# castorini/dhr

Hardware: AMD Instinct MI355X
Metric: queries/sec (exact top-1000, brute-force dense-hybrid GIP retrieval) (higher is better)
Workload: dtype i8 (bound GEMM: gated AND ungated columns int8 x int8 -> int32 on the matrix cores, every gated rounding upward, the ungated quantisation error paid by the filter margin) + f64-accumulated f16 x f32 exact rescoring of the survivors -- the returned scores are the exact scores rounded once, identical

## Files before the change

dhr_amd/_build.py:

```python
from __future__ import annotations

import concurrent.futures
import fcntl
import os
import shutil
import subprocess

CSRC = os.path.join(os.path.dirname(os.path.abspath(__file__)), "csrc")
LIB = os.path.join(CSRC, "libdhr_hip.so")
OBJDIR = os.path.join(CSRC, "build")
SOURCES = ["abi.cpp", "kernels.hip", "gemm_w4.hip", "gemm_g8.hip", "index_build.hip", "search_core.hip", "api.hip", "sharded.hip", "pq_adc.hip", "select_global.hip", "host_io.hip", "lexical.hip", "gip_train.hip", "lexical_train.hip", "maxsim.hip", "aggretriever_train.hip", "lexical_proj.hip", "lexical_proj_train.hip", "train_loss.hip", "densify_sparse.hip"]
HEADERS = ["dhr_internal.h", "dhr_state.h", "search_plan.h", "index_layout.h", "sharded_plan.h", "host_stage.h", "op_dispatch.h", "abi_guard.h", "libdhr.map", "gemm_common.h", "gemm_g8.h", "lexical_common.h", "lexical_proj_common.h", "lexical_proj_layout.h", os.path.join("..", "..", "include", "dhr_hip.h")]
FLAGS = ["--offload-arch=gfx950", "-O3", "-std=c++17", "-fPIC", "-Wno-unused-value", "-Wno-unused-result"]
if os.environ.get("DHR_AB_VARIANTS") == "1":
    SOURCES = SOURCES + [os.path.join("..", "..", "tools", "ab", "gemm_g8p.hip")]
    FLAGS = FLAGS + ["-DDHR_AB_VARIANTS", "-I" + CSRC]


def _mtime(path: str) -> float:
    return os.path.getmtime(path) if os.path.exists(path) else 0.0


def _stale() -> bool:
    t = _mtime(LIB)
    return t == 0.0 or any(_mtime(os.path.join(CSRC, f)) > t for f in SOURCES + HEADERS)


def _compile(hipcc: str, src: str, newest_header: float, force: bool, verbose: bool) -> str:
    obj = os.path.join(OBJDIR, os.path.splitext(os.path.basename(src))[0] + ".o")
    if not force and _mtime(obj) > max(_mtime(os.path.join(CSRC, src)), newest_header):
        return obj
    tmp = obj + ".tmp.%d" % os.getpid()
    cmd = [hipcc] + FLAGS + ["-c", src, "-o", tmp]
    if verbose:
        print(" ".join(cmd), flush=True)
    subprocess.run(cmd, cwd=CSRC, check=True)
    os.replace(tmp, obj)
    return obj


def build(force: bool = False, verbose: bool = False) -> str:
    if not force and not _stale():
        return LIB
    os.makedirs(OBJDIR, exist_ok=True)
    with open(os.path.join(OBJDIR, ".lock"), "w") as lock:
        fcntl.flock(lock, fcntl.LOCK_EX)
        try:
            if not force and not _stale():
                return LIB
            hipcc = shutil.which("hipcc") or "/opt/rocm/bin/hipcc"
            newest_header = max(_mtime(os.path.join(CSRC, h)) for h in HEADERS)
            with concurrent.futures.ThreadPoolExecutor(max_workers=min(len(SOURCES), os.cpu_count() or 1, 16)) as ex:
                objs = list(ex.map(lambda s: _compile(hipcc, s, newest_header, force, verbose), SOURCES))
            tmp = LIB + ".tmp.%d" % os.getpid()
            cmd = [hipcc, "--offload-arch=gfx950", "-shared", "-fPIC", "-Wl,--version-script=" + os.path.join(CSRC, "libdhr.map"), "-o", tmp] + objs + ["-L/opt/rocm/lib", "-lrccl"]
            if verbose:
                print(" ".join(cmd), flush=True)
            subprocess.run(cmd, cwd=CSRC, check=True)
            os.replace(tmp, LIB)
        finally:
            fcntl.flock(lock, fcntl.LOCK_UN)
    return LIB


if __name__ == "__main__":
# ... 3 lines not shown
```

dhr_amd/_lib.py:

```python
from __future__ import annotations

import ctypes as C
import os

import numpy as np

from . import _build

DHR_OK = 0
ERR_INVALID, ERR_UNSUPPORTED, ERR_HIP, ERR_INTERNAL, ERR_NOMEM, ERR_PEER = -1, -2, -3, -4, -5, -6
ABI_INDEX_DESC, ABI_QUERY_BATCH, ABI_SEARCH_STATS, ABI_FILE_INFO, ABI_HOST_SHARD = 0, 1, 2, 3, 4
IDX_NONE, IDX_U8, IDX_I8, IDX_I16 = 0, 1, 2, 3
VAL_F16, VAL_F32, VAL_BF16 = 0, 1, 2
MEM_HOST, MEM_DEVICE = 0, 1
LEX_RAW, LEX_DENSIFY, LEX_AGG_FULL, LEX_AGG_SEMI = 0, 1, 2, 3
PARAM_CAND_CAP, PARAM_FIRST_ROWS, PARAM_PROFILE, PARAM_MAX_GROWTH, PARAM_SAMPLE_PERIOD, PARAM_GEMM_VARIANT, PARAM_MAIN_CHUNKS, PARAM_PROGRESSIVE_THR, PARAM_AUX_CUS, PARAM_GEMM_EXCLUSIVE, PARAM_OVERLAP_AUX, PARAM_SAMPLE_SHARE, PARAM_ASYNC_CONTROLLER, PARAM_LIST_STRIDE = 1, 2, 3, 4, 5, 6, 7, 8, 9, 10, 11, 12, 13, 14
OPT_DENSE_I8, OPT_GATED_I8 = 1, 2
COMM_TRANSPORT, COMM_WORLD, COMM_RANK, COMM_DEVICE = 0, 1, 2, 3
INFO_DENSE_I8, INFO_I8_SCALE, INFO_I8_ROW_ERR, INFO_I8_ROW_NORM, INFO_ROW_NORM_MAX, INFO_TILE_BYTES, INFO_GATED_I8, INFO_GEMM_KERNEL = 1, 2, 3, 4, 5, 6, 7, 8

EXPORTS = ["dhr_version", "dhr_abi_sizes", "dhr_abi_size", "dhr_debug_fail_alloc", "dhr_set_option", "dhr_index_get_info", "dhr_last_error", "dhr_index_create", "dhr_index_destroy", "dhr_index_set_param",
           "dhr_index_device_bytes", "dhr_search", "dhr_score_rows", "dhr_merge_topk", "dhr_merge_topk_host", "dhr_merge_topk_lists", "dhr_merge_topk_lists_host",
           "dhr_get_stats", "dhr_debug_bound_scores", "dhr_debug_query_margins", "dhr_debug_gemm_time", "dhr_debug_seq_to_tile", "dhr_debug_sharded_repairs", "dhr_search_sample_rank", "dhr_search_union_rank", "dhr_search_begin",
           "dhr_search_finish", "dhr_search_mid_ranks", "dhr_search_mid", "dhr_search_pre_ranks", "dhr_search_pre", "dhr_search_begin_rest", "dhr_search_rerank", "dhr_comm_unique_id", "dhr_comm_create", "dhr_comm_wrap", "dhr_comm_create_callback", "dhr_comm_destroy", "dhr_comm_info", "dhr_comm_abort", "dhr_search_sharded", "dhr_search_sharded_local", "dhr_search_sharded_host", "dhr_pq_create", "dhr_pq_destroy", "dhr_pq_device_bytes", "dhr_pq_search", "dhr_pq_adc_scores", "dhr_pq_last_scan", "dhr_index_save", "dhr_index_file_info", "dhr_index_load", "dhr_densify", "dhr_pq_train", "dhr_pq_encode", "dhr_pq_decode", "dhr_pq_train_nbits", "dhr_pq_encode_nbits", "dhr_pq_decode_nbits", "dhr_write_trec", "dhr_format_float", "dhr_lexical_head", "dhr_aggregate", "dhr_gip_scores_workspace", "dhr_gip_scores", "dhr_gip_scores_backward", "dhr_densify_backward", "dhr_lexical_head_train_workspace", "dhr_lexical_head_train", "dhr_lexical_head_backward", "dhr_maxsim_scores", "dhr_maxsim_scores_backward", "dhr_aggregate_train", "dhr_aggregate_backward", "dhr_term_weight_head",
           "dhr_term_weight_head_backward", "dhr_lexical_proj_workspace", "dhr_lexical_proj_head", "dhr_lexical_proj_train_workspace",
           "dhr_lexical_proj_train", "dhr_lexical_proj_backward", "dhr_train_loss_workspace", "dhr_train_loss", "dhr_densify_sparse"]


class DhrError(RuntimeError):

    def __init__(self, msg, status=None):
        super().__init__(msg)
        self.status = status


class IndexDesc(C.Structure):
    _fields_ = [("device", C.c_int32), ("mem_kind", C.c_int32), ("n_rows", C.c_int64), ("d_dlr", C.c_int32),
                ("d_cls", C.c_int32), ("value", C.c_void_p), ("ld_value", C.c_int64), ("index", C.c_void_p),
                ("index_dtype", C.c_int32), ("idx_buckets", C.c_int32), ("ld_index", C.c_int64),
                ("row_offset", C.c_int64)]


class QueryBatch(C.Structure):
    _fields_ = [("n_queries", C.c_int32), ("mem_kind", C.c_int32), ("value", C.c_void_p), ("value_dtype", C.c_int32),
                ("index_dtype", C.c_int32), ("ld_value", C.c_int64), ("index", C.c_void_p), ("ld_index", C.c_int64)]


class SearchStats(C.Structure):
    _fields_ = [("n_rows", C.c_int64), ("n_queries", C.c_int64), ("k", C.c_int64), ("phases", C.c_int32),
                ("overflow_retries", C.c_int32), ("candidates_bound", C.c_int64), ("candidates_exact", C.c_int64),
                ("gemm_rows", C.c_int64), ("sample_fallback_queries", C.c_int64), ("gemm_ms", C.c_double), ("refine_ms", C.c_double),
                ("rescore_ms", C.c_double), ("select_ms", C.c_double), ("prep_ms", C.c_double),
                ("total_ms", C.c_double), ("gemm_flops", C.c_double), ("gemm_flops_alg", C.c_double)]

    def as_dict(self):
        return {f: getattr(self, f) for f, _ in self._fields_}


class FileInfo(C.Structure):
    _fields_ = [("n_rows", C.c_int64), ("row_offset", C.c_int64), ("d_dlr", C.c_int32), ("d_cls", C.c_int32),
                ("index_dtype", C.c_int32), ("idx_buckets", C.c_int32), ("file_version", C.c_uint32), ("reserved", C.c_uint32),
                ("payload_bytes", C.c_int64), ("blob_offset", C.c_int64), ("blob_bytes", C.c_int64)]


FILE_MAGIC = b"DHRIDX1\x00"

ALLGATHER_FN = C.CFUNCTYPE(C.c_int, C.c_void_p, C.c_void_p, C.c_void_p, C.c_int64)
HS_SAMPLE_RANK = C.CFUNCTYPE(C.c_int32, C.c_void_p, C.c_int32, C.c_int32)
HS_UNION_RANK = C.CFUNCTYPE(C.c_int32, C.c_void_p, C.c_int32)
HS_BEGIN = C.CFUNCTYPE(C.c_int32, C.c_void_p, C.POINTER(QueryBatch), C.c_int32, C.c_int32, C.c_void_p)
HS_FINISH = C.CFUNCTYPE(C.c_int32, C.c_void_p, C.c_void_p, C.c_void_p, C.c_void_p, C.c_void_p)
HS_SEARCH = C.CFUNCTYPE(C.c_int32, C.c_void_p, C.POINTER(QueryBatch), C.c_int32, C.c_void_p, C.c_void_p)
HS_MID_RANKS = C.CFUNCTYPE(C.c_int32, C.c_void_p, C.c_int32, C.c_int32, C.POINTER(C.c_int32), C.POINTER(C.c_int32))
HS_MID = C.CFUNCTYPE(C.c_int32, C.c_void_p, C.c_void_p, C.c_int32, C.c_void_p)
HS_PRE_RANKS = C.CFUNCTYPE(C.c_int32, C.c_void_p, C.c_int32, C.c_int32, C.POINTER(C.c_int32), C.POINTER(C.c_int32))
HS_PRE = C.CFUNCTYPE(C.c_int32, C.c_void_p, C.POINTER(QueryBatch), C.c_int32, C.c_int32, C.c_int32, C.c_void_p)
# ... 103 lines not shown
    lib.dhr_aggregate_train.argtypes = lib.dhr_aggregate.argtypes[:-1] + [C.c_void_p, C.c_int64, C.c_void_p]
    lib.dhr_aggregate_backward.argtypes = [C.c_int32, C.c_int32, C.c_void_p, C.c_int32, C.c_int64, C.c_void_p, C.c_int64, C.c_int64, C.c_int32, C.c_int32,
                                           C.c_int32, C.c_int32, C.c_void_p, C.c_int64, C.c_void_p]
    ids = [C.c_int32, C.c_int32, C.c_void_p, C.c_int32, C.c_int64]
    lib.dhr_term_weight_head.argtypes = ids + [C.c_void_p, C.c_int32, C.c_int64, C.c_int64, C.c_int32, C.c_int32, C.c_int32, C.c_void_p, C.c_int64,
                                               C.c_void_p, C.c_int64, C.c_void_p]
    lib.dhr_term_weight_head_backward.argtypes = ids + [C.c_int64, C.c_int32, C.c_int32, C.c_int32, C.c_void_p, C.c_int64, C.c_void_p, C.c_int64,
                                                        C.c_void_p, C.c_int32, C.c_int64, C.c_void_p]
    lib.dhr_pq_train.argtypes = [C.c_int32, C.c_int32, C.c_void_p, C.c_int64, C.c_int64, C.c_int32, C.c_int32, C.c_int32, C.c_int64, C.c_void_p,
                                 C.POINTER(C.c_double), C.c_void_p]
    lib.dhr_pq_encode.argtypes = [C.c_int32, C.c_int32, C.c_void_p, C.c_int64, C.c_int64, C.c_int32, C.c_int32, C.c_void_p, C.c_void_p, C.c_void_p]
    lib.dhr_pq_train_nbits.argtypes = [C.c_int32, C.c_int32, C.c_void_p, C.c_int64, C.c_int64, C.c_int32, C.c_int32, C.c_int32, C.c_int32, C.c_int64, C.c_void_p,
                                       C.POINTER(C.c_double), C.c_void_p]
    lib.dhr_pq_encode_nbits.argtypes = [C.c_int32, C.c_int32, C.c_void_p, C.c_int64, C.c_int64, C.c_int32, C.c_int32, C.c_int32, C.c_void_p, C.c_void_p, C.c_void_p]
    lib.dhr_pq_decode_nbits.argtypes = [C.c_int32, C.c_int32, C.c_void_p, C.c_int64, C.c_int32, C.c_int32, C.c_int32, C.c_void_p, C.c_void_p, C.c_int64, C.c_void_p]
    lib.dhr_write_trec.argtypes = [C.c_char_p, C.c_int32, C.c_int64, C.c_int64, C.c_void_p, C.c_void_p, C.c_void_p, C.c_void_p, C.c_int64, C.c_void_p,
                                   C.c_int64, C.c_void_p, C.c_char_p, C.c_int32, C.c_int32, C.POINTER(C.c_int64)]
    lib.dhr_format_float.argtypes = [C.c_double, C.c_char_p, C.c_int32]
    lib.dhr_pq_decode.argtypes = [C.c_int32, C.c_int32, C.c_void_p, C.c_int64, C.c_int32, C.c_int32, C.c_void_p, C.c_void_p, C.c_int64, C.c_void_p]
    lib.dhr_score_rows.argtypes = [C.c_void_p, C.POINTER(QueryBatch), C.c_int32, C.c_void_p, C.c_void_p, C.c_int32, C.c_void_p]
    lib.dhr_merge_topk.argtypes = [C.c_int32, C.c_int32, C.c_int32, C.c_void_p, C.c_void_p, C.c_int32, C.c_void_p,
                                   C.c_void_p, C.c_void_p]
    lib.dhr_merge_topk_host.argtypes = [C.c_int32, C.c_int32, C.c_void_p, C.c_void_p, C.c_int32, C.c_void_p, C.c_void_p]
    lib.dhr_merge_topk_lists.argtypes = [C.c_int32, C.c_int32, C.c_int32, C.c_int32, C.c_void_p, C.c_void_p, C.c_int32,
                                         C.c_void_p, C.c_void_p, C.c_void_p]
    lib.dhr_merge_topk_lists_host.argtypes = [C.c_int32, C.c_int32, C.c_int32, C.c_void_p, C.c_void_p, C.c_int32, C.c_void_p,
                                              C.c_void_p]
    lib.dhr_comm_unique_id.argtypes = [C.c_void_p, C.c_int32]
    lib.dhr_comm_create.argtypes = [C.c_void_p, C.c_int32, C.c_int32, C.c_int32, C.POINTER(C.c_void_p)]
    lib.dhr_comm_wrap.argtypes = [C.c_void_p, C.c_int32, C.c_int32, C.c_int32, C.POINTER(C.c_void_p)]
    lib.dhr_comm_create_callback.argtypes = [C.c_int32, C.c_int32, C.c_int32, ALLGATHER_FN, C.c_void_p, C.POINTER(C.c_void_p)]
    lib.dhr_search_sharded_host.argtypes = [C.POINTER(HostShard), C.c_int32, C.c_int32, ALLGATHER_FN, C.c_void_p, C.POINTER(QueryBatch), C.c_int32,
                                            C.c_void_p, C.c_void_p]
    lib.dhr_comm_destroy.argtypes = [C.c_void_p]
    lib.dhr_comm_destroy.restype = None
    lib.dhr_comm_abort.argtypes = [C.c_void_p]
    lib.dhr_comm_abort.restype = None
    lib.dhr_comm_info.argtypes = [C.c_void_p, C.c_int32]
    lib.dhr_search_sharded.argtypes = [C.c_void_p, C.c_void_p, C.POINTER(QueryBatch), C.c_int32, C.c_void_p, C.c_void_p, C.c_int32, C.c_void_p]
    lib.dhr_search_sharded_local.argtypes = [C.POINTER(C.c_void_p), C.c_int32, C.POINTER(QueryBatch), C.c_int32, C.c_void_p, C.c_void_p, C.c_int32, C.c_void_p]
    lib.dhr_pq_create.argtypes = [C.c_int32, C.c_int32, C.c_int64, C.c_int32, C.c_int32, C.c_int32, C.c_void_p, C.c_void_p, C.c_int64, C.POINTER(C.c_void_p)]
    lib.dhr_pq_destroy.argtypes = [C.c_void_p]
    lib.dhr_pq_destroy.restype = None
    lib.dhr_pq_device_bytes.argtypes = [C.c_void_p]
    lib.dhr_pq_device_bytes.restype = C.c_int64
    lib.dhr_pq_search.argtypes = [C.c_void_p, C.POINTER(QueryBatch), C.c_int32, C.c_void_p, C.c_void_p, C.c_int32, C.c_void_p]
    lib.dhr_pq_adc_scores.argtypes = [C.c_void_p, C.POINTER(QueryBatch), C.c_int64, C.c_int64, C.c_void_p, C.c_void_p]
    lib.dhr_pq_last_scan.argtypes = [C.c_void_p, C.POINTER(C.c_double), C.POINTER(C.c_double)]
    lib.dhr_get_stats.argtypes = [C.c_void_p, C.POINTER(SearchStats)]
    lib.dhr_set_option.argtypes = [C.c_int32, C.c_int64]
    lib.dhr_index_get_info.argtypes = [C.c_void_p, C.c_int32, C.POINTER(C.c_double)]
    lib.dhr_debug_bound_scores.argtypes = [C.c_void_p, C.POINTER(QueryBatch), C.c_int64, C.c_int64, C.c_void_p, C.c_void_p]
    lib.dhr_debug_query_margins.argtypes = [C.c_void_p, C.POINTER(QueryBatch), C.c_void_p, C.c_void_p]
    lib.dhr_debug_gemm_time.argtypes = [C.c_void_p, C.POINTER(QueryBatch), C.c_int32, C.POINTER(C.c_double),
                                        C.POINTER(C.c_double), C.c_void_p]
    if hasattr(lib, "dhr_debug_seq_to_tile"):
        lib.dhr_debug_seq_to_tile.argtypes = [C.c_int64, C.c_int32, C.c_int32, C.c_int64, C.c_int64, C.c_int64, C.POINTER(C.c_int64)]
        lib.dhr_debug_seq_to_tile.restype = None
    lib.dhr_search_sample_rank.argtypes = [C.c_void_p, C.c_int32]
    lib.dhr_search_sample_rank.restype = C.c_int32
    lib.dhr_search_union_rank.argtypes = [C.c_void_p, C.c_int32]
    lib.dhr_search_union_rank.restype = C.c_int32
    lib.dhr_search_begin.argtypes = [C.c_void_p, C.POINTER(QueryBatch), C.c_int32, C.c_void_p, C.c_void_p]
    lib.dhr_search_finish.argtypes = [C.c_void_p, C.c_void_p, C.c_void_p, C.c_void_p, C.c_void_p, C.c_int32, C.c_void_p]
    lib.dhr_search_mid_ranks.argtypes = [C.c_void_p, C.c_int32, C.POINTER(C.c_int32), C.POINTER(C.c_int32)]
    lib.dhr_search_mid_ranks.restype = C.c_int32
    lib.dhr_search_mid.argtypes = [C.c_void_p, C.c_void_p, C.c_int32, C.c_void_p, C.c_void_p]
    lib.dhr_search_pre_ranks.argtypes = [C.c_void_p, C.c_int32, C.POINTER(C.c_int32), C.POINTER(C.c_int32)]
    lib.dhr_search_pre_ranks.restype = C.c_int32
    lib.dhr_search_pre.argtypes = [C.c_void_p, C.POINTER(QueryBatch), C.c_int32, C.c_int32, C.c_void_p, C.c_void_p]
    lib.dhr_search_begin_rest.argtypes = [C.c_void_p, C.c_void_p, C.c_void_p, C.c_void_p]
    _lib = lib
    return lib


def check(rc: int, what: str):
    if rc != DHR_OK:
        raise DhrError(f"{what} failed ({rc}): {load().dhr_last_error().decode()}", status=rc)


_NP_IDX = {np.dtype(np.uint8): IDX_U8, np.dtype(np.int8): IDX_I8, np.dtype(np.int16): IDX_I16}


def idx_code(dtype) -> int:
    name = str(dtype).replace("torch.", "")
    try:
        return _NP_IDX[np.dtype(name)]
    except (KeyError, TypeError):
        raise DhrError(f"unsupported index dtype {dtype} (uint8 / int8 / int16)") from None


def _ptr_ld(a):
    if isinstance(a, np.ndarray):
        if a.ndim != 2 or a.strides[1] != a.itemsize or a.strides[0] % a.itemsize:
            raise DhrError("arrays must be 2-D with a contiguous last dimension")
        return a.ctypes.data, a.strides[0] // a.itemsize, MEM_HOST
    if a.dim() != 2 or a.stride(1) != 1:
        raise DhrError("tensors must be 2-D with a contiguous last dimension")
    return a.data_ptr(), a.stride(0), (MEM_DEVICE if a.is_cuda else MEM_HOST)


def _val_code(a, bf16: bool = False) -> int:
    name = str(a.dtype).replace("torch.", "")
    if name == "float16":
        return VAL_F16
    if name == "float32":
# ... 21 lines not shown
```

dhr_amd/csrc/api.hip:

```cpp
#include "host_stage.h"

namespace {
dhr_search_stats fresh_stats(const dhr_index* ix, int Q, int k) {
  dhr_search_stats st{};
  st.n_rows = ix->n_rows; st.n_queries = Q; st.k = k;
  return st;
}
int emit_results(dhr_index* ix, Workspace& w, int Q, int k, float* out_scores, int64_t* out_rows, int out_mem_kind, hipStream_t s) {
  if (out_mem_kind == DHR_MEM_HOST) {
    const int rc = grow(w.out_stage, w.out_stage_bytes, (size_t)Q * k * 12, w.bytes);
    if (rc != DHR_OK) return rc;
  }
  return emit_topk(w.topk_keys, w.kp, Q, k, ix->row_offset, out_scores, out_rows, out_mem_kind, w.out_stage, s);
}
void collect_timers(Timer& tm, dhr_search_stats& st) {
  double ms[5] = {0, 0, 0, 0, 0};
  tm.collect(ms);
  st.gemm_ms += ms[T_GEMM]; st.refine_ms += ms[T_REFINE]; st.rescore_ms += ms[T_RESCORE]; st.select_ms += ms[T_SELECT]; st.prep_ms += ms[T_PREP];
}
template <typename Body>
int timed_search(dhr_index* ix, int Q, int k, hipStream_t s, Body&& body) {
  Events evs;
  hipEvent_t ev0, ev1;
  HIP_TRY(evs.add(&ev0)); HIP_TRY(evs.add(&ev1));
// ... 431 lines not shown
  if (nbits < 1 || nbits > 8) return set_error(DHR_ERR_UNSUPPORTED, "nbits must be in [1, 8]");
  const int ksub = 1 << nbits;
  if (!out_values) return set_error(DHR_ERR_INVALID, "null pointer");
  if (n == 0) return DHR_OK;
  HIP_TRY(hipSetDevice(device));
  hipStream_t s = (hipStream_t)stream;
  const int dsub = d / M;
  const bool host = mem_kind == DHR_MEM_HOST;
  DevMem m_cb, m_cd, m_ov;
  const float* d_cb;
  const uint8_t* d_cd;
  HIP_TRY(operand_in(m_cb, mem_kind, codebooks, (size_t)M * ksub * dsub * 4, s, d_cb));
  HIP_TRY(operand_in(m_cd, mem_kind, codes, (size_t)n * M, s, d_cd));
  if (host) HIP_TRY(dev_alloc(m_ov, n * d * 2));
  HIP_TRY(launch_pq_decode(d_cd, M, n, M, dsub, d_cb, (__half*)(host ? m_ov.p : out_values), host ? d : ld_out, ksub, s));
  if (host) HIP_TRY(stage_out(out_values, ld_out, m_ov.p, n, d, 2, s));
  HIP_TRY(hipStreamSynchronize(s));
  return DHR_OK;
} DHR_CATCH_STATUS

extern "C" int dhr_debug_bound_scores(dhr_index* ix, const dhr_query_batch* qb, int64_t row_lo, int64_t row_hi,
                                      float* out_dev, void* stream) try {
  int rc = check_queries(ix, qb);
  if (rc) return rc;
  if (row_lo < 0 || row_hi > ix->n_rows || row_lo >= row_hi || !out_dev) return set_error(DHR_ERR_INVALID, "bad row range");
  HIP_TRY(hipSetDevice(ix->device));
  hipStream_t s = (hipStream_t)stream;
  Workspace& w = ix->ws;
  if ((rc = ensure_ws(ix, w, qb->n_queries, 1, 0)) != DHR_OK) return rc;
  if ((rc = prep_queries(ix, w, qb, s)) != DHR_OK) return rc;
  GemmArgs g = base_gemm_args(ix, w, qb->n_queries);
  g.seq_lo = row_lo / TILE_ROWS; g.seq_hi = (row_hi + TILE_ROWS - 1) / TILE_ROWS; g.map_mode = 0; g.period = 1; g.head = 0;
  g.thr = w.thr; g.cand = w.cand; g.cnt = w.cnt;
  g.dump = out_dev; g.dump_ld = row_hi - row_lo; g.dump_row0 = row_lo;
  HIP_TRY(launch_gemm_filter(g, s));
  HIP_TRY(hipStreamSynchronize(s));
  return DHR_OK;
} DHR_CATCH_STATUS

extern "C" int dhr_debug_query_margins(dhr_index* ix, const dhr_query_batch* qb, float* out_host, void* stream) try {
  int rc = check_queries(ix, qb);
  if (rc) return rc;
  if (!out_host) return set_error(DHR_ERR_INVALID, "null output pointer");
  HIP_TRY(hipSetDevice(ix->device));
  hipStream_t s = (hipStream_t)stream;
  Workspace& w = ix->ws;
  if ((rc = ensure_ws(ix, w, qb->n_queries, 1, 0)) != DHR_OK) return rc;
  if ((rc = prep_queries(ix, w, qb, s)) != DHR_OK) return rc;
  HIP_TRY(hipMemcpyAsync(out_host, w.margin, (size_t)qb->n_queries * 4, hipMemcpyDeviceToHost, s));
  HIP_TRY(hipStreamSynchronize(s));
  return DHR_OK;
} DHR_CATCH_STATUS

extern "C" void dhr_debug_seq_to_tile(int64_t seq, int32_t map_mode, int32_t period, int64_t head, int64_t perm_mul, int64_t perm_n, int64_t out[2]) try {
  out[0] = seq_to_tile_fast(seq, map_mode, period, head, perm_mul, perm_n, 1.0 / (double)(perm_n > 0 ? perm_n : 1), 1.0 / (double)(period > 1 ? period - 1 : 1));
  out[1] = seq_to_tile(seq, map_mode, period, head, perm_mul, perm_n);
} DHR_CATCH_VOID
extern "C" int dhr_debug_gemm_time(dhr_index* ix, const dhr_query_batch* qb, int32_t iters, double* ms_out, double* flops_out,
                                   void* stream) try {
  int rc = check_queries(ix, qb);
  if (rc) return rc;
  if (iters <= 0 || !ms_out) return set_error(DHR_ERR_INVALID, "bad iters / null pointer");
  HIP_TRY(hipSetDevice(ix->device));
  hipStream_t s = (hipStream_t)stream;
  Workspace& w = ix->ws;
  const bool open = getenv("DHR_GEMM_TIME_OPEN") && atoi(getenv("DHR_GEMM_TIME_OPEN")) != 0 && w.thr_hat && ix->stats.k > 0 && ix->stats.n_queries == qb->n_queries;
  if ((rc = ensure_ws(ix, w, qb->n_queries, open ? (int)ix->stats.k : 1, 0)) != DHR_OK) return rc;
  if ((rc = prep_queries(ix, w, qb, s)) != DHR_OK) return rc;
  if (open) {
    HIP_TRY(hipMemcpyAsync(w.thr, w.thr_hat, (size_t)w.q_pad * 4, hipMemcpyDeviceToDevice, s));
  } else {
    std::vector<float> inf((size_t)w.q_pad, INFINITY);
    HIP_TRY(hipMemcpyAsync(w.thr, inf.data(), (size_t)w.q_pad * 4, hipMemcpyHostToDevice, s));
  }
  const bool opened = open;
  HIP_TRY(hipMemsetAsync(w.cnt, 0, (size_t)w.q_pad * 4, s));
  GemmArgs g = base_gemm_args(ix, w, qb->n_queries);
  g.seq_lo = 0; g.seq_hi = ix->n_tiles; g.map_mode = 0; g.period = 1; g.head = 0;
  g.thr = w.thr; g.cand = w.cand; g.cnt = w.cnt;
  HIP_TRY(launch_gemm_filter(g, s));
  Events evs;
  hipEvent_t e0, e1;
  HIP_TRY(evs.add(&e0)); HIP_TRY(evs.add(&e1));
  HIP_TRY(hipEventRecord(e0, s));
  for (int i = 0; i < iters; ++i) {
    if (opened) HIP_TRY(hipMemsetAsync(w.cnt, 0, (size_t)w.q_pad * 4, s));
    HIP_TRY(launch_gemm_filter(g, s));
  }
  HIP_TRY(hipEventRecord(e1, s));
  HIP_TRY(hipStreamSynchronize(s));
  float ms = 0.f;
  HIP_TRY(hipEventElapsedTime(&ms, e0, e1));
  *ms_out = ms / iters;
  if (flops_out) *flops_out = 2.0 * (double)w.q_pad * (double)ix->n_tiles * TILE_ROWS * (double)ix->kt;
  return DHR_OK;
} DHR_CATCH_STATUS

extern "C" int dhr_merge_topk(int32_t device, int32_t n_queries, int32_t n_in, const float* in_scores,
                              const int64_t* in_rows, int32_t k_out, float* out_scores, int64_t* out_rows, void* stream) try {
  if (n_queries <= 0 || n_in <= 0 || k_out <= 0 || !in_scores || !in_rows || !out_scores || !out_rows)
    return set_error(DHR_ERR_INVALID, "bad argument");
  HIP_TRY(hipSetDevice(device));
  if (n_in > 16384) {
    if ((int64_t)n_queries * n_in > (int64_t)0x7fffffff) return set_error(DHR_ERR_UNSUPPORTED, "more than 2^31 entries in one device reduce");
    HIP_TRY(launch_merge_topk_global(n_queries, n_in, in_scores, in_rows, k_out, out_scores, out_rows, (hipStream_t)stream));
    return DHR_OK;
// ... 60 lines not shown
```

dhr_amd/csrc/dhr_internal.h:

```cpp
#pragma once
#include <hip/hip_runtime.h>
#include <hip/hip_fp16.h>
#include <stdint.h>

#include "../../include/dhr_hip.h"
#include "abi_guard.h"

extern "C" int dhr_set_error_message(int code, const char* msg);
extern "C" int dhr_index_device(const dhr_index* ix);
extern "C" void dhr_internal_index_arena(dhr_index* ix, void*** base, size_t** bytes);
extern "C" int dhr_internal_search_begin_async(dhr_index* ix, const dhr_query_batch* qb, int32_t k, float* out_sample_scores_dev, void* stream);
extern "C" void dhr_internal_search_abort(dhr_index* ix);
extern "C" int dhr_internal_search_pre_async(dhr_index* ix, const dhr_query_batch* qb, int32_t k, int32_t r_local, float* out_scores_dev, void* stream);
extern "C" int dhr_internal_search_begin_rest_async(dhr_index* ix, const float* tau_dev, float* out_sample_scores_dev, void* stream);
extern "C" int dhr_internal_search_mid_async(dhr_index* ix, const float* tau_hat_dev, int32_t r_local, float* out_scores_dev, void* stream);
extern "C" int dhr_internal_search_finish_async(dhr_index* ix, const float* tau_hat_dev, float* out_scores, int64_t* out_rows, int32_t* out_count_dev,
                                                int32_t out_mem_kind, void* stream);

namespace dhr {

constexpr int TILE_ROWS = 256;
constexpr int TILE_K = 64;
constexpr int CHUNK = 8;
constexpr int TILE_HALVES = TILE_ROWS * TILE_K;
// ... 46 lines not shown
__host__ __device__ inline int64_t seq_to_tile(int64_t i, int map_mode, int period, int64_t head, int64_t perm_mul = 1, int64_t perm_n = 1) {
  if (map_mode == 0) return i;
  if (map_mode == 1) return head + i * period;
  if (map_mode == 3) i = (i * perm_mul) % perm_n;
  return head + (i / (period - 1)) * period + i % (period - 1) + 1;
}
__host__ __device__ inline int64_t divmod24(int64_t x, int64_t n, double inv_n, int64_t& rem) {
  const double xd = (double)(int32_t)(x >> 24) * 16777216.0 + (double)(int32_t)(x & 0xFFFFFF);
  int64_t q = (int64_t)(int32_t)(xd * inv_n);
  int64_t r = x - q * n;
  if (r < 0) { r += n; --q; } else if (r >= n) { r -= n; ++q; }
  rem = r;
  return q;
}
__host__ __device__ inline int64_t seq_to_tile_fast(int64_t i, int map_mode, int period, int64_t head, int64_t perm_mul, int64_t perm_n,
                                                    double inv_perm_n, double inv_pm1) {
  if (map_mode == 0) return i;
  if (map_mode == 1) return head + i * period;
  if (map_mode == 3) (void)divmod24(i * perm_mul, perm_n, inv_perm_n, i);
  int64_t rem;
  const int64_t q = divmod24(i, period - 1, inv_pm1, rem);
  return head + q * period + rem + 1;
}
__host__ __device__ inline uint64_t make_key(float score, uint32_t row) {
  return ((uint64_t)f32_ordered(score) << 32) | (uint64_t)(0xFFFFFFFFu - row);
}

struct GemmArgs {
  const __half* a_tiles;
  const __half* b_tiles;
  int ksteps;
  int k_split;
  int ts, td;
  int ts_q;
  int64_t seq_lo, seq_hi;
  int map_mode, period;
  int64_t perm_mul, perm_n;
  double inv_perm_n, inv_pm1;
  int64_t head, n_tiles;
  int n_qtiles;
  int64_t n_rows;
  const float* thr;
  uint2* cand;
  uint32_t* cnt;
  uint32_t cap;
  float* dump;
  int64_t dump_ld;
  int64_t dump_row0;
  int n_queries;
  int variant;
  const int32_t* g8_shift;
  const int32_t* g8_rsum;
  int partial_wn;
  uint32_t* p_ctr;
  int64_t p_groups;
  const float* i8_mul;
  const struct ListTier* tier;
};
struct ListTier { uint2* ovf; const uint32_t* ovf_off; const uint32_t* ovf_cap; };
#if defined(__HIPCC__)
template <bool TIER = true>
__device__ __forceinline__ void cand_store(const GemmArgs& p, int q, uint32_t slot, uint2 v) {
  if (slot < p.cap) p.cand[(int64_t)q * p.cap + slot] = v;
  else if (TIER && p.tier) {
    const ListTier* t = p.tier;
    const uint32_t o = slot - p.cap;
    if (o < t->ovf_cap[q]) t->ovf[(size_t)t->ovf_off[q] + o] = v;
  }
}
#endif

__host__ __device__ inline int quant_up_i8(float x, float inv_step) {
  float r = ceilf(x * inv_step);
  r = r < 0.f ? 0.f : (r > 127.f ? 127.f : r);
  return (int)r;
}
__host__ __device__ inline int quant_up_u8(float x, float inv_step) {
  float r = ceilf(x * inv_step);
  r = r < 0.f ? 0.f : (r > 255.f ? 255.f : r);
  return (int)r;
}
__host__ __device__ inline int quant_i8(float v, float inv_scale) {
  float r = rintf(v * inv_scale);
  r = r < -127.f ? -127.f : (r > 127.f ? 127.f : r);
  return (int)r;
}

struct RescoreArgs {
  const __half* vals_rm;
  const void* c_idx;
  int c_idx_dtype;
  const float* q32;
  const int16_t* q_idx;
  const __half* q16; const uint8_t* q_idx8; const uint32_t* q_inexact;
  int d_dlr, k_rm;
  int gate;
  int64_t n_rows;
  const uint2* cand; const uint32_t* cnt; uint32_t cap;
  const uint32_t* rows32;
  int64_t ld_rows;
  int64_t row0; uint32_t count_all;
  const float* thr_exact;
  uint64_t* out_keys;
  int64_t ld_keys;
  float* out_scores;
  int64_t ld_scores;
// ... 75 lines not shown
inline int sparse_query_stages(int ts, bool gated, bool g8 = false) { return ts > 0 ? ((gated || g8) ? ts : 2 * ts) : 0; }
hipError_t launch_gemm_filter(const GemmArgs& a, hipStream_t s);
hipError_t launch_heavy_build(const __half* vals_rm, int k_rm, const void* idx, int idx_dtype, int64_t n_rows, int d_dlr,
                              const uint8_t* map, int n_buckets, uint32_t* heavy_key, __half* heavy_val,
                              const float* g8_inv_cs , int abs_mode, hipStream_t s);
#ifndef REFINE_PER_WG_N
#define REFINE_PER_WG_N 512
#endif
constexpr int REFINE_PER_WG = REFINE_PER_WG_N;
struct RefineArgs {
  const uint2* cand; const uint32_t* cnt; uint32_t cap;
  const uint2* ovf; const uint32_t* ovf_off; const uint32_t* ovf_cap;
  const uint32_t* heavy_key; const __half* heavy_val;
  const uint32_t* q_pack; int d_dlr;
  const float* thr;
  uint2* out; uint32_t* out_cnt; uint32_t out_cap;
  int n_queries; uint32_t max_count;
  const uint32_t* blk_off; uint32_t flat_blocks;
  const uint8_t* g8_q8;
  const float* g8_inv_cs;
  const float* g8_unit;
  int abs_mode;
  int ungated;
  const uint8_t* resid8; int resid_ld;
  const float* q32; int64_t q32_ld;
  const float* col_scale; int d_cls;
  const float* thr_raise;
};
hipError_t launch_resid_build(const __half* vals_rm, int k_rm, int64_t n_rows, int d_dlr, int d_cls, const float* col_scale, uint8_t* resid8, int resid_ld, hipStream_t s);
hipError_t launch_refine(const RefineArgs& a, hipStream_t s);
hipError_t launch_rescore(const RescoreArgs& a, hipStream_t s);
hipError_t launch_select(const SelectArgs& a, hipStream_t s);
hipError_t launch_select_global(const SelectArgs& a, hipStream_t s);
hipError_t launch_merge_topk_global(int n_queries, int n_in, const float* in_scores, const int64_t* in_rows, int k_out, float* out_scores,
                                    int64_t* out_rows, hipStream_t s);
hipError_t launch_emit(const uint64_t* topk_keys, int kp, int n_queries, int k, int64_t row_offset, float* out_scores,
                       int64_t* out_rows, hipStream_t s);
hipError_t launch_keys_to_rows(const uint64_t* topk_keys, int kp, int n_queries, int k, uint32_t* rows, hipStream_t s);
hipError_t launch_bound_topm(const float* bound , int n_rows, int n_queries, int m, uint32_t* rows , hipStream_t s);
hipError_t launch_densify(const void* lex, int in_is_f32, int64_t ld, int64_t batch, int remove, int dims, int n_groups, void* out_val,
                          int val_is_f32, int64_t ld_val, void* out_idx, int idx_is_i16, int64_t ld_idx, hipStream_t s);
hipError_t launch_pq_init(const __half* vals, int64_t ld, int64_t n, int64_t stride, int dsub, int M, float* cb, int ksub, hipStream_t s);
hipError_t launch_pq_assign(const __half* vals, int64_t ld, int64_t n, int64_t stride, int dsub, int M, const float* cb, uint8_t* codes,
                            int64_t ld_codes, float* sums, uint32_t* counts, float* err, int ksub, hipStream_t s);
hipError_t launch_pq_update(float* cb, const float* sums, const uint32_t* counts, int dsub, int M, int ksub, hipStream_t s);
hipError_t launch_pq_decode(const uint8_t* codes, int64_t ld_codes, int64_t n, int M, int dsub, const float* cb, __half* out, int64_t ld_out,
                            int ksub, hipStream_t s);
hipError_t launch_block_offsets(const uint32_t* cnt, uint32_t cap, int n_queries, uint32_t per, uint32_t* offs, hipStream_t s);
hipError_t launch_plan_overflow(const uint32_t* cnt_prev, double rows_ratio, uint32_t cap, uint32_t max_extra, uint32_t arena_entries, int n_queries,
                                uint32_t* ovf_off, uint32_t* ovf_cap, hipStream_t s);
hipError_t launch_max_u32(const uint32_t* v, int n, uint32_t* out_max, unsigned long long* out_sum, hipStream_t s);
hipError_t launch_lists_ready(const uint32_t* cnt, uint32_t cap, int n_queries, uint32_t per, uint32_t* offs, uint32_t* out_max, uint32_t* out_max2,
                              unsigned long long* out_sum, unsigned long long* out_sum2, uint32_t* fail_flags, uint32_t* zero, int n_zero,
                              hipStream_t s, const uint32_t* ovf_cap = nullptr);
hipError_t launch_rows_to_local(const int64_t* rows, int64_t n, int64_t row_offset, int64_t n_rows, uint32_t* out,
                                hipStream_t s);
hipError_t launch_mark_overflow(const uint32_t* cnt, uint32_t cap, int n_queries, uint32_t* fail_flags, hipStream_t s);
hipError_t launch_verify(const uint64_t* topk_keys, int kp, int k, const float* tau_hat, int n_queries, uint32_t* fail_flags,
                         uint32_t* n_fail, hipStream_t s);
hipError_t launch_gather_queries(const float* q32, const int16_t* q_idx, int k_rm, int d_dlr, const int32_t* ids, int n,
                                 float* out32, int16_t* out_idx, hipStream_t s);
hipError_t launch_scatter_keys(const uint64_t* src, uint64_t* dst, int kp, const int32_t* ids, int n, hipStream_t s);
hipError_t launch_emit_scores(const uint64_t* topk_keys, int kp, int n_queries, int r, float* out, hipStream_t s);
hipError_t launch_make_thr(const float* tau, const float* margin, int n_queries, int q_pad, float* thr, hipStream_t s);
hipError_t launch_raise_thr(float* thr_hat, const float* thr_run, int n_queries, hipStream_t s);
hipError_t launch_flag_tau_above(const float* tau_own, const float* tau_ext, int n_queries, uint32_t* fail_flags, hipStream_t s);
hipError_t launch_raise_thr_rank(float* thr_hat, float* tau_hat, const uint64_t* topk_keys, int kp, int r, const float* margin, int n_queries, hipStream_t s);
hipError_t launch_count_ge(const uint64_t* topk_keys, int kp, int k, const float* tau, const uint32_t* fail_flags, int n_queries,
                           int32_t* out, hipStream_t s);
hipError_t launch_merge_topk(int n_queries, int n_in, const float* in_scores, const int64_t* in_rows, int k_out,
                             float* out_scores, int64_t* out_rows, hipStream_t s);
hipError_t launch_merge_lists(int n_queries, int n_lists, int list_len, const float* in_scores, const int64_t* in_rows, int k_out,
                              float* out_scores, int64_t* out_rows, hipStream_t s, int64_t stride_s = 0, int64_t stride_r = 0);

extern int g_gemm_variant;
extern thread_local int g_last_gemm_kernel;
constexpr int RESCORE_CANDS_PER_WG = 32;
constexpr uint32_t FLAT_GRID_MAX = 1u << 20;
constexpr uint32_t FLAT_GRID_ASYNC = 16384;
constexpr int SELECT_THREADS = 1024;

}
```

dhr_amd/csrc/dhr_state.h:

```cpp
#pragma once
#include <algorithm>
#include <cmath>
#include <cstdio>
#include <cstring>
#include <string>
#include <vector>

#include "dhr_internal.h"
#include "search_plan.h"
#include <hip/hip_ext.h>

using namespace dhr;
static_assert(plan::TILE_ROWS == TILE_ROWS && plan::DOC_GROUP == DOC_GROUP, "search_plan.h restates the tile geometry of dhr_internal.h");
using plan::BOOT_M;
using plan::SearchPlan;
using plan::round_up;

inline int set_error(int code, const std::string& msg) { return dhr_set_error_message(code, msg.c_str()); }
#define HIP_TRY(expr)                                                                                          \
  do {                                                                                                         \
    hipError_t _e = (expr);                                                                                    \
    if (_e != hipSuccess)                                                                                      \
      return set_error(DHR_ERR_HIP, std::string(#expr) + ": " + hipGetErrorString(_e) + " (" __FILE__ ":" +    \
                                        std::to_string(__LINE__) + ")");                                       \
// ... 16 lines not shown
    v.reserve(v.size() + 1);
    hipEvent_t e = nullptr;
    const hipError_t rc = hipEventCreateWithFlags(&e, flags);
    if (rc == hipSuccess) v.push_back(e);
    *out = e;
    return rc;
  }
};
static inline int idx_esize(int dt) { return dt == DHR_IDX_I16 ? 2 : 1; }

struct Workspace {
  int q_pad = 0, kp = 0;
  int q_alloc = 0;
  int64_t cap = 0;
  int64_t cap_deep = 0;
  int64_t arena = 0;
  uint2 *ovf = nullptr, *ovf2 = nullptr;
  uint32_t *ovf_off = nullptr, *ovf_cap = nullptr;
  uint32_t* boot_rows = nullptr;
  float* boot_bound = nullptr;
  bool keys_alias = false;
  ListTier* tier_dev = nullptr;
  uint32_t* cnt_plan = nullptr;
  int64_t plan_rows = 0;
  uint32_t last_maxr = 0;
  int64_t cap_r = 0;
  int64_t keys_ld = 0, kt = 0, d_dlr = 0;
  int ts_q = 0;
  __half* q_tiles = nullptr;
  float* q32 = nullptr;
  int16_t* q_idx = nullptr;
  __half* q16 = nullptr;
  uint8_t* q_idx8 = nullptr;
  uint32_t* q_inexact = nullptr;
  float *margin = nullptr, *tau = nullptr, *thr = nullptr;
  float* i8_mul = nullptr;
  uint8_t* g8_q8 = nullptr;
  int32_t* g8_shift = nullptr;
  float* g8_unit = nullptr;
  uint32_t* cnt = nullptr;
  uint2* cand = nullptr;
  uint64_t *rs_keys = nullptr, *topk_keys = nullptr;
  uint32_t* d_max = nullptr;
  float* tau_hat = nullptr;
  float* thr_hat = nullptr;
  uint32_t* fail_flags = nullptr;
  uint32_t* q_pack = nullptr;
  float* thr_raise = nullptr;
  uint2* cand_r = nullptr;
  uint32_t* cnt_r = nullptr;
  uint32_t* blk_off = nullptr;
  uint2* cand2 = nullptr;
  uint32_t* cnt2 = nullptr;
  void* h_pinned = nullptr;
  char* h_pinned2 = nullptr;
  uint32_t* d_max2 = nullptr;
  unsigned long long* d_stats = nullptr;
  void* h_stats = nullptr;
  uint32_t* d_ref = nullptr;
  void* h_ref = nullptr;
  void* q_stage = nullptr;  size_t q_stage_bytes = 0;
  void* qi_stage = nullptr; size_t qi_stage_bytes = 0;
  void* out_stage = nullptr; size_t out_stage_bytes = 0;
  int64_t bytes = 0;
};

enum class StagedState { None, AfterPre, AfterBegin, AfterMid, Complete };
enum class Stage { Whole, Begin, Finish, Mid, Pre, BeginRest };

struct dhr_index {
  int device = 0;
  int64_t n_rows = 0, n_tiles = 0, row_offset = 0;
  int d_dlr = 0, d_cls = 0, k = 0, idx_dtype = DHR_IDX_NONE;
  int dlr_pad = 0;
  int k_rm = 0;
  int n_buckets = 1;
  int idx_buckets_req = 0;
  int kt = 0;
  int ksteps = 0;
  int ts = 0, td = 0;
  __half* tiles = nullptr;
  __half* vals_rm = nullptr;
  void* c_idx = nullptr;
  uint8_t* bucket_map = nullptr;
  uint32_t* heavy_key = nullptr;
  __half* heavy_val = nullptr;
  bool abs_mode = false;
  float dmax = 0.f;
  bool dense_i8 = false;
  float i8_scale = 0.f, i8_ec = 0.f, i8_nc = 0.f;
  uint8_t* resid8 = nullptr;
  int resid_ld = 0;
  float resid_ec2 = 0.f;
  float* i8_col_scale = nullptr;
  bool gated_i8 = false;
  float g8_sref = 0.f;
  int g8_max_shift = 0;
  float* g8_inv_cs = nullptr;
  float* g8_w = nullptr;
  int32_t* g8_rsum = nullptr;
  int64_t index_bytes = 0;
  int64_t cand_cap = 0, first_rows = 0;
  int64_t list_stride = 0;
  int profile = 0, max_growth16 = 32;
  int sample_period = 32;
  int async_ctl = 2;
  int sample_share = 1;
  int main_chunks = 2;
  int progressive_thr = 2;
  int n_cu = 256;
  int gemm_variant = 0;
  int last_gemm_kernel = 0;
  int overlap_aux = -1;
  int aux_cus = -1, gemm_exclusive = 0;
  int aux_cus_made = -1, gemm_excl_made = -1;
  hipStream_t s_gemm = nullptr;
  hipStream_t s_aux = nullptr;
  struct {
    StagedState state = StagedState::None;
    bool gate = false; int Q = 0, k = 0;
    double rate = 0.0, rate_r = 0.0;
    int64_t dev_bound = 0, dev_exact = 0;
    int64_t pre_pos = 0, pre_seen = 0, pre_last_rows = 0;
  } pend;
  Workspace ws, ws_fb[2];
  void* sh_arena = nullptr;
  size_t sh_arena_bytes = 0;
  dhr_search_stats stats{};
};

inline void free_ws(Workspace& w) {
  hipFree(w.q_tiles); hipFree(w.q32); hipFree(w.q_idx); hipFree(w.q16); hipFree(w.q_idx8); hipFree(w.q_inexact); hipFree(w.margin); hipFree(w.i8_mul); hipFree(w.g8_q8); hipFree(w.g8_shift); hipFree(w.g8_unit); hipFree(w.tau); hipFree(w.thr);
  hipFree(w.cnt); hipFree(w.cand); if (!w.keys_alias) hipFree(w.rs_keys); hipFree(w.topk_keys); hipFree(w.d_max); hipFree(w.tau_hat); hipFree(w.fail_flags); hipFree(w.thr_hat); hipFree(w.cand2); hipFree(w.cnt2); hipFree(w.q_pack); hipFree(w.cand_r); hipFree(w.cnt_r); hipFree(w.thr_raise); hipFree(w.blk_off); hipFree(w.ovf); hipFree(w.ovf2); hipFree(w.ovf_off); hipFree(w.ovf_cap); hipFree(w.cnt_plan); hipFree(w.tier_dev); hipFree(w.boot_rows); hipFree(w.boot_bound);
  if (w.h_pinned) hipHostFree(w.h_pinned);
  if (w.h_pinned2) hipHostFree(w.h_pinned2);
  hipFree(w.d_max2); hipFree(w.d_ref); hipFree(w.d_stats);
  if (w.h_ref) hipHostFree(w.h_ref);
  if (w.h_stats) hipHostFree(w.h_stats);
  hipFree(w.q_stage); hipFree(w.qi_stage); hipFree(w.out_stage);
  w = Workspace();
}


constexpr int32_t MEM_DEVICE_PADDED = 2;
#ifndef SELECT_SORT_Q
#define SELECT_SORT_Q 8
#endif
inline int select_sort_n(int kp) { return kp * SELECT_SORT_Q / 4; }
enum { T_GEMM = 0, T_REFINE = 1, T_RESCORE = 2, T_SELECT = 3, T_PREP = 4 };
struct Drain {
  dhr_index* ix; hipStream_t s; bool armed = true;
  ~Drain() {
    if (!armed) return;
    (void)hipStreamSynchronize(s);
    if (ix->s_aux) (void)hipStreamSynchronize(ix->s_aux);
    if (ix->s_gemm) (void)hipStreamSynchronize(ix->s_gemm);
    (void)hipGetLastError();
  }
};
struct Timer {
  bool on; hipStream_t s; std::vector<std::pair<hipEvent_t, hipEvent_t>> ev; std::vector<int> kind;
  ~Timer() { for (auto& e : ev) { (void)hipEventDestroy(e.first); (void)hipEventDestroy(e.second); } }
  void begin(int k) { begin_on(k, s); }
  void end() { end_on(s); }
  void begin_on(int k, hipStream_t st) { if (!on) return; ev.reserve(ev.size() + 1); kind.reserve(kind.size() + 1); hipEvent_t a, b; hipEventCreate(&a); hipEventCreate(&b); hipEventRecord(a, st); ev.push_back({a, b}); kind.push_back(k); }
  void end_on(hipStream_t st) { if (!on) return; hipEventRecord(ev.back().second, st); }
  void collect(double* ms ) {
    for (size_t i = 0; i < ev.size(); ++i) {
      float t = 0.f;
      if (hipEventElapsedTime(&t, ev[i].first, ev[i].second) == hipSuccess) ms[kind[i]] += t;
      hipEventDestroy(ev[i].first); hipEventDestroy(ev[i].second);
    }
    ev.clear(); kind.clear();
  }
};

int ensure_ws(dhr_index* ix, Workspace& w, int n_queries, int k, int64_t keys_ld_min, int64_t cap_mult = 1, bool use_refine = true, bool queries_only = false);
int check_queries(const dhr_index* ix, const dhr_query_batch* qb);
int grow(void*& p, size_t& have, size_t need, int64_t& total);
int prep_queries(dhr_index* ix, Workspace& w, const dhr_query_batch* qb, hipStream_t s);
dhr::RescoreArgs base_rescore_args(const dhr_index* ix, const Workspace& w, int n_queries, bool gate);
dhr::GemmArgs base_gemm_args(const dhr_index* ix, const Workspace& w, int n_queries);
dhr::SelectArgs rescored_select_args(const Workspace& w, int n_queries, int k);
inline SearchPlan search_plan_of(const dhr_index* ix, int k, int depth, bool staged) {
  plan::PlanInput in;
  in.n_rows = ix->n_rows; in.n_tiles = ix->n_tiles; in.k = k; in.sample_period = ix->sample_period; in.sample_share = ix->sample_share;
// ... 8 lines not shown
```

dhr_amd/csrc/gemm_g8.h:

```cpp
#pragma once
#include "gemm_common.h"
#include <climits>

namespace dhr {

typedef int intx4 __attribute__((ext_vector_type(4)));
typedef int intx8 __attribute__((ext_vector_type(8)));

constexpr int G8_QOFF = 16384;
constexpr int G8_SLOT = 32768;
constexpr int G8_META = 4 * G8_SLOT;
constexpr int G8_RING_LDS = 4 * G8_SLOT + 4096 + 64;
constexpr int G8_NT = 512;


__device__ __forceinline__ void g8_smfmac(floatx16& c, const intx4& a, const intx8& b, uint32_t idx) {
  asm("v_smfmac_i32_32x32x64_i8 %0, %1, %2, %3" : "+v"(c) : "v"(a), "v"(b), "v"(idx));
}
__device__ __forceinline__ void g8_mfma(floatx16& c, const intx4& a, const intx4& b) {
  asm("v_mfma_i32_32x32x32_i8 %0, %1, %2, %0" : "+v"(c) : "v"(a), "v"(b));
}

struct G8Frag {
  intx4 a[4];
  intx4 pw;
  union { intx8 v; intx4 h[2]; } b[2];
};

__device__ __forceinline__ int g8_thr_units(float thr, float mul) {
  const float x = thr / mul;
  if (!(x < 2.1e9f)) return INT_MAX;
  if (x < -2.1e9f) return INT_MIN;
  return (int)floorf(x - fabsf(x) * 1e-6f) - 1;
}
__device__ __forceinline__ float g8_score(int sum, float mul) {
  const float x = (float)sum * mul;
  return x + fabsf(x) * 2.4e-7f;
}


hipError_t launch_gemm_g8p(const GemmArgs& a, hipStream_t s);
bool gemm_g8p_ok(const GemmArgs& a);

}
```

dhr_amd/csrc/gemm_g8.hip:

```cpp
#include "gemm_g8.h"
#include <mutex>
#include <type_traits>

#ifndef G8_TRACE
#define G8_TRACE 0
#endif
#ifndef G8_ABL
#define G8_ABL 0
#endif
namespace dhr {

#if G8_TRACE
constexpr int G8_TRACE_SLOTS = 1 << 18;
__device__ unsigned long long g8_trace_buf[G8_TRACE_SLOTS * 8];
__device__ unsigned int g8_trace_n;
#define G8_T(i) do { if (threadIdx.x == 0 && tslot < G8_TRACE_SLOTS) g8_trace_buf[(size_t)tslot * 8 + (i)] = __builtin_readcyclecounter(); } while (0)
#else
#define G8_T(i) do { } while (0)
#endif
__device__ __forceinline__ void g8_dump_tile(const GemmArgs& p, floatx16 (&acc)[4][2], int64_t dt, int qt, int wm, int wn, int lane,
                                             const float (&mul_r)[2]) {
  const int fhalf = lane >> 5;
  const int64_t row_base = dt * TILE_ROWS + wm * 128;
#pragma unroll
  for (int ni = 0; ni < 2; ++ni) {
    const int q = qt * TILE_ROWS + wn * 64 + ni * 32 + (lane & 31);
    if (q < p.n_queries) {
#pragma unroll
      for (int mi = 0; mi < 4; ++mi)
#pragma unroll
        for (int e = 0; e < 16; ++e) {
          const int64_t row = row_base + mi * 32 + (e & 3) + 8 * (e >> 2) + 4 * fhalf;
          if (row < p.n_rows && row >= p.dump_row0 && row - p.dump_row0 < p.dump_ld)
            p.dump[(int64_t)q * p.dump_ld + (row - p.dump_row0)] = g8_score(__float_as_int(acc[mi][ni][e]), mul_r[ni]);
        }
    }
  }
}

template <bool SURPLUS, int NI_, bool CHECK_ROWS = true>
__device__ __forceinline__ void g8_scan_half(const GemmArgs& p, floatx16 (&acc)[4][2], int qt, int wm, int wn, int lane, int rows_valid, int64_t row0,
                                             uint2* stack, const int t, const float mul, uint32_t& j) {
  const int fhalf = lane >> 5;
  const int rbase = wm * 128 + 4 * fhalf;
  const int q = qt * TILE_ROWS + wn * 64 + NI_ * 32 + (lane & 31);
#pragma unroll
  for (int mi = 0; mi < 4; ++mi) {
    const floatx16& a = acc[mi][NI_];
#pragma unroll
    for (int g = 0; g < 4; ++g) {
      const int gm = max(max(__float_as_int(a[4 * g]), __float_as_int(a[4 * g + 1])), max(__float_as_int(a[4 * g + 2]), __float_as_int(a[4 * g + 3])));
      if (gm >= t) {
        asm volatile("");
        if constexpr (!SURPLUS && !CHECK_ROWS) {
#pragma unroll
          for (int e = 4 * g; e < 4 * g + 4; ++e) {
            const int v = __float_as_int(a[e]);
            const int rl = rbase + mi * 32 + (e & 3) + 8 * (e >> 2);
            const uint32_t slot = j < (uint32_t)EPI_STACK ? j : (uint32_t)EPI_STACK;
            stack[slot * G8_NT] = make_uint2((uint32_t)rl, (uint32_t)v);
            j += v >= t ? 1u : 0u;
          }
        } else
#pragma unroll
        for (int e = 4 * g; e < 4 * g + 4; ++e) {
          const int v = __float_as_int(a[e]);
          const int rl = rbase + mi * 32 + (e & 3) + 8 * (e >> 2);
          if (v >= t && (!CHECK_ROWS || rl < rows_valid)) {
            asm volatile("");
            if constexpr (SURPLUS) {
              if (j >= EPI_STACK) {
                const uint32_t slot = atomicAdd(p.cnt + q, 1u);
                cand_store(p, q, slot, make_uint2((uint32_t)(row0 + rl), __float_as_uint(g8_score(v, mul))));
              }
            } else if (j < EPI_STACK) stack[j * G8_NT] = make_uint2((uint32_t)rl, (uint32_t)v);
            ++j;
          }
        }
      }
    }
  }
}
__device__ __forceinline__ void g8_epilogue_surplus(const GemmArgs& p, floatx16 (&acc)[4][2], int qt, int wm, int wn, int lane, int rows_valid, int64_t row0,
                                                 const int (&thr_r)[2], const float (&mul_r)[2]) {
  uint32_t j = 0;
  g8_scan_half<true, 0>(p, acc, qt, wm, wn, lane, rows_valid, row0, nullptr, thr_r[0], mul_r[0], j);
  g8_scan_half<true, 1>(p, acc, qt, wm, wn, lane, rows_valid, row0, nullptr, thr_r[1], mul_r[1], j);
}
__device__ __forceinline__ void g8_epilogue(const GemmArgs& p, floatx16 (&acc)[4][2], int64_t dt, int qt, int wm, int wn, int tid, int lane,
                                            char* smem, const int (&thr_r)[2], const float (&mul_r)[2]) {
  __syncthreads();
  const int64_t row0 = dt * TILE_ROWS;
  const int rows_valid = (int)(p.n_rows - row0 < TILE_ROWS ? p.n_rows - row0 : TILE_ROWS);
  uint2* stack = (uint2*)smem + tid;
  const int q0 = qt * TILE_ROWS + wn * 64 + (lane & 31);
  const bool full = rows_valid == TILE_ROWS;
  uint32_t j = 0;
  if (full) g8_scan_half<false, 0, false>(p, acc, qt, wm, wn, lane, rows_valid, row0, stack, thr_r[0], mul_r[0], j);
  else g8_scan_half<false, 0, true>(p, acc, qt, wm, wn, lane, rows_valid, row0, stack, thr_r[0], mul_r[0], j);
  const uint32_t s0 = j < (uint32_t)EPI_STACK ? j : (uint32_t)EPI_STACK;
#if G8_ABL != 16
  uint32_t base0 = 0u, base1 = 0u;
  if (s0 > 0) base0 = atomicAdd(p.cnt + q0, s0);
#endif
  if (full) g8_scan_half<false, 1, false>(p, acc, qt, wm, wn, lane, rows_valid, row0, stack, thr_r[1], mul_r[1], j);
  else g8_scan_half<false, 1, true>(p, acc, qt, wm, wn, lane, rows_valid, row0, stack, thr_r[1], mul_r[1], j);
  const uint32_t s1 = j < (uint32_t)EPI_STACK ? j : (uint32_t)EPI_STACK;
#if G8_ABL == 16
  return;
#else
  if (s1 > s0) base1 = atomicAdd(p.cnt + q0 + 32, s1 - s0);
  if (__builtin_amdgcn_ballot_w64(j > (uint32_t)EPI_STACK) != 0) g8_epilogue_surplus(p, acc, qt, wm, wn, lane, rows_valid, row0, thr_r, mul_r);
  for (uint32_t i = 0; i < s0; ++i) {
    const uint2 en = stack[i * G8_NT];
    const uint32_t slot = base0 + i;
    cand_store(p, q0, slot, make_uint2((uint32_t)row0 + en.x, __float_as_uint(g8_score((int)en.y, mul_r[0]))));
  }
  for (uint32_t i = s0; i < s1; ++i) {
    const uint2 en = stack[i * G8_NT];
    const uint32_t slot = base1 + (i - s0);
    cand_store(p, q0 + 32, slot, make_uint2((uint32_t)row0 + en.x, __float_as_uint(g8_score((int)en.y, mul_r[1]))));
  }
#endif
}

#if G8_ABL == 2
#define G8_PAIR_SYNC() do { asm volatile("s_waitcnt lgkmcnt(0)" ::: "memory"); __builtin_amdgcn_s_barrier(); } while (0)
#elif G8_ABL == 3
#define G8_PAIR_SYNC() do { asm volatile("s_waitcnt lgkmcnt(0)" ::: "memory"); } while (0)
#else
#define G8_PAIR_SYNC() do { asm volatile("s_waitcnt vmcnt(0) lgkmcnt(0)" ::: "memory"); __builtin_amdgcn_s_barrier(); } while (0)
#endif

#ifndef G8_DMA_SCHED
#define G8_DMA_SCHED 1
#endif
#if G8_DMA_SCHED == 1
__host__ __device__ constexpr int g8_dma_piece(int ph, int g) { return ph == 0 ? g : -1; }
#elif G8_DMA_SCHED == 2
__host__ __device__ constexpr int g8_dma_piece(int ph, int g) { return ph == 0 ? (g >= 2 ? g - 2 : -1) : (ph == 1 && g < 2) ? 6 + g : -1; }
#else
__host__ __device__ constexpr int g8_dma_piece(int ph, int g) { return (ph <= 1 && (g & 1)) ? ph * 4 + (g >> 1) : -1; }
#endif

template <bool DUMP, bool PARTIAL>
__device__ __forceinline__ void g8_tile(const GemmArgs& p, char* smem, const int64_t dt, const int qt, const unsigned tslot = 0) {
  const int lane = threadIdx.x & 63;
  const int wave = __builtin_amdgcn_readfirstlane(threadIdx.x >> 6);
  const int ts = p.ts, td = p.td;
  const int nsp = ts >> 1, npairs = (ts + td) >> 1;
  const char* a_src = (const char*)p.a_tiles + dt * ((int64_t)ts * S8_STAGE_A + (int64_t)td * SP_DENSE);
  const char* b_src = (const char*)p.b_tiles + (int64_t)qt * ((int64_t)ts * SP_STAGE_B + (int64_t)td * SP_DENSE);
  const int wm = PARTIAL ? (wave & 1) : (wave >> 2), wn = PARTIAL ? (wave >> 1) : (wave & 3);
  const bool active = !PARTIAL || wn < p.partial_wn;

  const bool dma_b = ((wave >> 1) & 1) != 0;
  const int dma_s = wave >> 2;
  const int dma_h = wave & 1;
  const uint32_t lane_off = (uint32_t)lane * 16u;
  const uint32_t smem_u = (uint32_t)(uintptr_t)LDS_PTR(smem);
  const __amdgpu_buffer_rsrc_t role_rsrc = __builtin_amdgcn_make_buffer_rsrc((void*)(dma_b ? b_src : a_src), (short)0, 0x7fffffff, 0x00020000);
  int dma_soff = 0, dma_n = 0, nx_soff = 0, nx_n = 0;
  uint32_t dma_lds = 0, nx_lds = 0;
  auto dma_prepare = [&](int g) __attribute__((always_inline)) {
    const int u = 2 * g + dma_s;
    const bool sp = u < ts;
    const int half_bytes = dma_h * ((!dma_b && sp) ? S8_STAGE_A / 2 : 8192);
    if (dma_b) nx_soff = (sp ? u * SP_STAGE_B : ts * SP_STAGE_B + (u - ts) * SP_DENSE) + half_bytes;
    else nx_soff = (sp ? u * S8_STAGE_A : ts * S8_STAGE_A + (u - ts) * SP_DENSE) + half_bytes;
    nx_lds = smem_u + (uint32_t)((u & 3) * G8_SLOT + (dma_b ? G8_QOFF : 0) + half_bytes);
    nx_n = g < npairs ? ((!dma_b && sp) ? 5 : 8) : 0;
    if ((G8_ABL == 4 || G8_ABL == 8) && g >= 2) nx_n = 0;
  };
  auto dma_commit = [&]() __attribute__((always_inline)) { dma_soff = nx_soff; dma_lds = nx_lds; dma_n = nx_n; };
// ... 23 lines not shown
  const int c0 = (fhalf ^ swz4) << 4, c1 = ((2 + fhalf) ^ swz4) << 4;
  const int a8_off = ((wm * 8 + fhalf) * 32 + frow) * 16;
  const int p8_off = S8_A_BYTES + ((wm * 2 + fhalf) * 32 + frow) * 16;
  const int ad_row = (wm * 128 + frow) * 64;
  const int q_row = G8_QOFF + (wn * 64 + frow) * 64;

  auto read_s8 = [&](G8Frag& f, const char* sl, int g) __attribute__((always_inline)) {
    if (g < 4) f.b[g >> 1].h[g & 1] = *(const intx4*)(sl + q_row + (g >> 1) * 2048 + ((g & 1) ? c1 : c0));
    else if (g < 8) f.a[g - 4] = *(const intx4*)(sl + a8_off + (g - 4) * 1024);
    else if (g == 8) f.pw = *(const intx4*)(sl + p8_off);
  };
  auto read_dn = [&](G8Frag& f, const char* sl, int cc, int g) __attribute__((always_inline)) {
    if (g < 2) f.b[g].h[0] = *(const intx4*)(sl + q_row + g * 2048 + cc);
    else if (g < 6) f.a[g - 2] = *(const intx4*)(sl + ad_row + (g - 2) * 2048 + cc);
  };
  auto blk_s8 = [&](const G8Frag& fc, G8Frag& fn, int un, bool do_load, auto ph_c) __attribute__((always_inline)) {
    constexpr int PH = decltype(ph_c)::value;
    const char* sl = smem + (un & 3) * G8_SLOT;
#pragma unroll
    for (int g = 0; g < 8; ++g) {
      const int ni = g >> 2, mi = g & 3;
      if (!PARTIAL || active) {
        if (do_load && G8_ABL != 8) {
          read_s8(fn, sl, g);
          if (g == 0) read_s8(fn, sl, 8);
        }
        g8_smfmac(acc[mi][ni], fc.a[mi], fc.b[ni].v, (uint32_t)fc.pw[mi]);
      }
      if (g8_dma_piece(PH, g) >= 0) dma_piece(g8_dma_piece(PH, g));
      __builtin_amdgcn_sched_barrier(0);
    }
  };
  auto blk_dn = [&](const G8Frag& fc, G8Frag& fn, int tn, bool do_load, auto ph_c) __attribute__((always_inline)) {
    constexpr int PH = decltype(ph_c)::value;
    const char* sl = smem + ((ts + (tn >> 1)) & 3) * G8_SLOT;
    const int cc = (tn & 1) ? c1 : c0;
#pragma unroll
    for (int g = 0; g < 8; ++g) {
      const int ni = g >> 2, mi = g & 3;
      if (!PARTIAL || active) {
        if (do_load && G8_ABL != 8) read_dn(fn, sl, cc, g);
        g8_mfma(acc[mi][ni], fc.a[mi], fc.b[ni].h[0]);
      }
      if (g8_dma_piece(PH, g) >= 0) dma_piece(g8_dma_piece(PH, g));
      __builtin_amdgcn_sched_barrier(0);
    }
  };

  if (wave < 4 && (ts > 0 || wave == 1 || wave == 2)) {
    const char* src = wave == 0 ? (const char*)(p.g8_rsum + dt * TILE_ROWS) : wave == 1 ? (const char*)(p.i8_mul + qt * TILE_ROWS)
                    : wave == 2 ? (const char*)(p.thr + qt * TILE_ROWS) : (const char*)(p.g8_shift + qt * TILE_ROWS);
    __builtin_amdgcn_global_load_lds(GLOBAL_PTR(src + lane_off), LDS_PTR(smem + G8_META + wave * 1024), 16, 0, 0);
  }
  issue_pair(0);
  if (npairs > 1) {
    issue_pair(1);
    if (dma_n == 5) asm volatile("s_waitcnt vmcnt(5)" ::: "memory"); else asm volatile("s_waitcnt vmcnt(8)" ::: "memory");
  } else asm volatile("s_waitcnt vmcnt(0)" ::: "memory");
  __builtin_amdgcn_s_barrier();
  G8_T(2);
  if (ts > 0) {
    const int32_t* rs = (const int32_t*)(smem + G8_META) + wm * 128 + 4 * (lane >> 5);
#pragma unroll
    for (int mi = 0; mi < 4; ++mi)
#pragma unroll
      for (int g4 = 0; g4 < 4; ++g4) {
        const intx4 v = *(const intx4*)(rs + mi * 32 + 8 * g4);
#pragma unroll
        for (int i4 = 0; i4 < 4; ++i4) acc[mi][0][4 * g4 + i4] = acc[mi][1][4 * g4 + i4] = __int_as_float(v[i4]);
      }
  } else {
#pragma unroll
    for (int mi = 0; mi < 4; ++mi)
#pragma unroll
      for (int e = 0; e < 16; ++e) acc[mi][0][e] = acc[mi][1][e] = 0.f;
  }
  int sh_r[2];
  float mul_r[2], thr_f[2];
#pragma unroll
  for (int ni = 0; ni < 2; ++ni) {
    const int ql = wn * 64 + ni * 32 + (lane & 31);
    mul_r[ni] = ((const float*)(smem + G8_META + 1024))[ql];
    thr_f[ni] = ((const float*)(smem + G8_META + 2048))[ql];
    sh_r[ni] = ts > 0 ? ((const int*)(smem + G8_META + 3072))[ql] : 0;
    asm volatile("" : "+v"(mul_r[ni]), "+v"(thr_f[ni]), "+v"(sh_r[ni]));
  }
  G8Frag f0, f1;
  if (ts > 0) {
#pragma unroll
    for (int g = 0; g < 9; ++g) read_s8(f0, smem, g);
  }
  if (G8_ABL == 8) f1 = f0;
  constexpr std::integral_constant<int, 0> PH0{};
  constexpr std::integral_constant<int, 1> PH1{};
  constexpr std::integral_constant<int, 2> PH2{};
  dma_n = 0;
#pragma unroll 1
  for (int g = 0; g + 1 < nsp; ++g) {
    blk_s8(f0, f1, 2 * g + 1, true, PH1);
    dma_prepare(g + 2);
    __builtin_amdgcn_sched_barrier(0);
    G8_PAIR_SYNC();
    dma_commit();
    blk_s8(f1, f0, 2 * g + 2, true, PH0);
  }
  if (nsp > 0) {
// ... 140 lines not shown
```

dhr_amd/csrc/index_build.hip:

```cpp
#include <fcntl.h>
#include <sys/mman.h>
#include <sys/stat.h>
#include <unistd.h>

#include "dhr_state.h"
#include "index_layout.h"
static_assert(layout::TILE_ROWS == TILE_ROWS && layout::TILE_K == TILE_K && layout::SP_STAGE_A == SP_STAGE_A && layout::S8_STAGE_A == S8_STAGE_A && layout::SP_DENSE == SP_DENSE && layout::HEAVY_KEY_STRIDE == HEAVY_KEY_STRIDE, "index_layout.h restates the tile geometry of dhr_internal.h");

extern "C" void dhr_index_destroy(dhr_index* ix) try {
  if (!ix) return;
  hipSetDevice(ix->device);
  free_ws(ix->ws);
  free_ws(ix->ws_fb[0]);
  free_ws(ix->ws_fb[1]);
  if (ix->s_aux) hipStreamDestroy(ix->s_aux);
  if (ix->s_gemm) hipStreamDestroy(ix->s_gemm);
  hipFree(ix->sh_arena);
  hipFree(ix->resid8); hipFree(ix->i8_col_scale); hipFree(ix->g8_inv_cs); hipFree(ix->g8_w); hipFree(ix->g8_rsum); hipFree(ix->tiles); hipFree(ix->c_idx); hipFree(ix->vals_rm); hipFree(ix->bucket_map); hipFree(ix->heavy_key);
  delete ix;
} DHR_CATCH_VOID

static int g_opt_dense_i8 = -1;
static int g_opt_gated_i8 = -1;
extern "C" int dhr_set_option(int32_t option, int64_t value) try {
  if (option == DHR_OPT_DENSE_I8) { g_opt_dense_i8 = value < 0 ? -1 : (value != 0); return DHR_OK; }
  if (option == DHR_OPT_GATED_I8) { g_opt_gated_i8 = value < 0 ? -1 : (value != 0); return DHR_OK; }
  return set_error(DHR_ERR_INVALID, "unknown option");
} DHR_CATCH_STATUS
extern "C" int dhr_index_get_info(const dhr_index* ix, int32_t what, double* out) try {
  if (!ix || !out) return set_error(DHR_ERR_INVALID, "null argument");
  switch (what) {
    case DHR_INFO_DENSE_I8: *out = ix->dense_i8 ? 1.0 : 0.0; return DHR_OK;
    case DHR_INFO_I8_SCALE: *out = ix->i8_scale; return DHR_OK;
    case DHR_INFO_I8_ROW_ERR: *out = ix->i8_ec; return DHR_OK;
    case DHR_INFO_I8_ROW_NORM: *out = ix->i8_nc; return DHR_OK;
    case DHR_INFO_ROW_NORM_MAX: *out = ix->dmax; return DHR_OK;
    case DHR_INFO_GATED_I8: *out = ix->gated_i8 ? 1.0 : 0.0; return DHR_OK;
    case DHR_INFO_GEMM_KERNEL: *out = (double)ix->last_gemm_kernel; return DHR_OK;
    case DHR_INFO_TILE_BYTES: *out = (double)layout::tile_bytes(ix->n_tiles, ix->ts, ix->td, ix->gated_i8); return DHR_OK;
  }
  return set_error(DHR_ERR_INVALID, "unknown info id");
} DHR_CATCH_STATUS

extern "C" int dhr_index_set_param(dhr_index* ix, int32_t param, int64_t value) try {
  if (!ix) return set_error(DHR_ERR_INVALID, "null index");
  switch (param) {
    case DHR_PARAM_CAND_CAP:
      if (value < DOC_GROUP * TILE_ROWS || value > (1 << 22)) return set_error(DHR_ERR_INVALID, "cand_cap must be in [1024, 4194304]");
      ix->cand_cap = value; return DHR_OK;
    case DHR_PARAM_FIRST_ROWS:
      if (value < 0) return set_error(DHR_ERR_INVALID, "first_rows must be >= 0");
      ix->first_rows = value; return DHR_OK;
    case DHR_PARAM_PROFILE: ix->profile = value != 0; return DHR_OK;
    case DHR_PARAM_SAMPLE_PERIOD:
      if (value < 0 || value > 256) return set_error(DHR_ERR_INVALID, "sample_period must be in [0,256] (0/1 = off)");
      ix->sample_period = (int)value; return DHR_OK;
    case DHR_PARAM_ASYNC_CONTROLLER: ix->async_ctl = value < 0 ? 0 : (value > 2 ? 2 : (int)value); return DHR_OK;
    case DHR_PARAM_LIST_STRIDE:
      if (value != 0 && (value < DOC_GROUP * TILE_ROWS || value > (1 << 22) || value % 256))
        return set_error(DHR_ERR_INVALID, "list_stride must be 0 (default) or a multiple of 256 in [1024, 4194304]");
      ix->list_stride = value; return DHR_OK;
    case DHR_PARAM_SAMPLE_SHARE:
      if (value < 1 || value > 4096) return set_error(DHR_ERR_INVALID, "sample_share must be in [1,4096]");
      ix->sample_share = (int)value; return DHR_OK;
    case DHR_PARAM_MAIN_CHUNKS:
      if (value < 1 || value > 64) return set_error(DHR_ERR_INVALID, "main_chunks must be in [1,64]");
      ix->main_chunks = (int)value; return DHR_OK;
    case DHR_PARAM_PROGRESSIVE_THR: ix->progressive_thr = value < 0 ? 0 : (value > 2 ? 2 : (int)value); return DHR_OK;
    case DHR_PARAM_AUX_CUS:
      if (value < 0 || value > 192 || value % 8) return set_error(DHR_ERR_INVALID, "aux_cus must be a multiple of 8 in [0,192]");
      ix->aux_cus = (int)value; return DHR_OK;
    case DHR_PARAM_GEMM_EXCLUSIVE: ix->gemm_exclusive = value != 0; return DHR_OK;
    case DHR_PARAM_OVERLAP_AUX: ix->overlap_aux = value < 0 ? -1 : value != 0; return DHR_OK;
    case DHR_PARAM_GEMM_VARIANT:
#ifdef DHR_AB_VARIANTS
      if (value == 6) { ix->gemm_variant = 6; return DHR_OK; }
#endif
      if (value != 4 && value != 5) return set_error(DHR_ERR_INVALID, "gemm_variant: 4 (4 waves, 128 x 128 wave tiles) or 5 (8 waves, 128 x 64 wave tiles; default) -- the fp16-gated kernel; integer (gated_i8) indexes have one kernel");
      ix->gemm_variant = (int)value; return DHR_OK;
    case DHR_PARAM_MAX_GROWTH:
      if (value < 1 || value > 1024) return set_error(DHR_ERR_INVALID, "max_growth must be in [1,1024] sixteenths");
      ix->max_growth16 = (int)value; return DHR_OK;
  }
  return set_error(DHR_ERR_INVALID, "unknown parameter");
} DHR_CATCH_STATUS

extern "C" int dhr_index_device(const dhr_index* ix) try { return ix ? ix->device : -1; } DHR_CATCH_VALUE(-1)
extern "C" void dhr_internal_index_arena(dhr_index* ix, void*** base, size_t** bytes) try { *base = &ix->sh_arena; *bytes = &ix->sh_arena_bytes; } DHR_CATCH_VOID
extern "C" int64_t dhr_index_device_bytes(const dhr_index* ix) try { return ix ? ix->index_bytes + ix->ws.bytes + ix->ws_fb[0].bytes + ix->ws_fb[1].bytes + (int64_t)ix->sh_arena_bytes : 0; } DHR_CATCH_VALUE(0)
extern "C" int dhr_get_stats(const dhr_index* ix, dhr_search_stats* out) try {
  if (!ix || !out) return set_error(DHR_ERR_INVALID, "null argument");
  *out = ix->stats;
  return DHR_OK;
} DHR_CATCH_STATUS

static int ingest(dhr_index* ix, const dhr_index_desc* d, uint32_t* d_flags , void* stage, int64_t block_rows,
                  hipStream_t s) {
  const int64_t n = ix->n_rows;
  for (int64_t lo = 0; lo < n; lo += block_rows) {
    const int64_t rows = std::min(block_rows, n - lo);
    const __half* src;
    int64_t ld;
    if (ix->dlr_pad > 0) {
      const hipMemcpyKind kind = d->mem_kind == DHR_MEM_HOST ? hipMemcpyHostToDevice : hipMemcpyDeviceToDevice;
      const int d_in = ix->d_dlr - ix->dlr_pad;
      const char* base = (const char*)d->value + lo * d->ld_value * 2;
      HIP_TRY(hipMemcpy2DAsync(stage, (size_t)ix->k * 2, base, (size_t)d->ld_value * 2, (size_t)d_in * 2, (size_t)rows, kind, s));
      if (ix->d_cls > 0)
        HIP_TRY(hipMemcpy2DAsync((char*)stage + (size_t)ix->d_dlr * 2, (size_t)ix->k * 2, base + (size_t)d_in * 2, (size_t)d->ld_value * 2,
                                 (size_t)ix->d_cls * 2, (size_t)rows, kind, s));
      src = (const __half*)stage;
      ld = ix->k;
    } else if (d->mem_kind == DHR_MEM_HOST) {
      HIP_TRY(hipMemcpy2DAsync(stage, (size_t)ix->k * 2, (const char*)d->value + lo * d->ld_value * 2,
                               (size_t)d->ld_value * 2, (size_t)ix->k * 2, (size_t)rows, hipMemcpyHostToDevice, s));
      src = (const __half*)stage;
      ld = ix->k;
    } else {
      src = (const __half*)d->value + lo * d->ld_value;
      ld = d->ld_value;
    }
    HIP_TRY(launch_scan_rows(src, ld, rows, ix->d_dlr, ix->k, d_flags, d_flags + 1, s));
    HIP_TRY(launch_copy_rows(src, ld, rows, ix->k, ix->k_rm, ix->vals_rm + lo * ix->k_rm, s));
    if (d->mem_kind == DHR_MEM_HOST || ix->dlr_pad > 0) HIP_TRY(hipStreamSynchronize(s));
  }
  return DHR_OK;
// ... 299 lines not shown
```

dhr_amd/csrc/kernels.hip:

```cpp
#include <algorithm>
#include <cstdlib>
#include <mutex>

#include "dhr_internal.h"
#include "gemm_common.h"
#include <type_traits>

namespace dhr {

typedef short short8 __attribute__((ext_vector_type(8)));

static hipError_t ensure_lds_attr(const void* fn, int bytes, int (&have)[64]) {
  static std::mutex mu;
  int dev = 0;
  (void)hipGetDevice(&dev);
  std::lock_guard<std::mutex> lock(mu);
  if (bytes <= have[dev & 63]) return hipSuccess;
  const hipError_t e = hipFuncSetAttribute(fn, hipFuncAttributeMaxDynamicSharedMemorySize, bytes);
  if (e == hipSuccess) have[dev & 63] = bytes;
  return e;
}

__device__ __forceinline__ float wave_sum(float v) {
#pragma unroll
  for (int o = 32; o > 0; o >>= 1) v += __shfl_xor(v, o, 64);
  return v;
}
__device__ __forceinline__ double wave_sum_f64(double v) {
#pragma unroll
  for (int o = 32; o > 0; o >>= 1) v += __shfl_xor(v, o, 64);
  return v;
}

__global__ void __launch_bounds__(256) scan_rows_kernel(const __half* __restrict__ src, int64_t ld, int64_t n_rows,
                                                        int d_dlr, int k, uint32_t* max_sq_bits, uint32_t* neg_flag) {
  const int lane = threadIdx.x & 63;
  const int64_t wave0 = (int64_t)blockIdx.x * 4 + (threadIdx.x >> 6);
  const int64_t nwaves = (int64_t)gridDim.x * 4;
  const bool vec = ((k & 7) == 0) && ((ld & 7) == 0) && ((((uintptr_t)src) & 15) == 0);
  float best = 0.f, amax = 0.f, gmax = 0.f;
  bool neg = false;
  for (int64_t row = wave0; row < n_rows; row += nwaves) {
    const __half* r = src + row * ld;
    float s = 0.f;
    if (vec) {
      for (int c = lane; c * 8 < k; c += 64) {
        const half8 v = *(const half8*)(r + c * 8);
#pragma unroll
        for (int e = 0; e < 8; ++e) {
          const float f = (float)v[e];
          s += f * f;
          neg |= (c * 8 + e < d_dlr) && (f < 0.f);
          if (fabsf(f) <= 65504.f) { if (c * 8 + e >= d_dlr) amax = fmaxf(amax, fabsf(f)); else gmax = fmaxf(gmax, fabsf(f)); }
        }
      }
    } else {
      for (int j = lane; j < k; j += 64) {
        const float f = __half2float(r[j]);
// ... 474 lines not shown
  }
}

hipError_t launch_query_prep(const void* src, int src_is_f32, int64_t ld, const void* idx, int idx_dtype, int64_t ld_idx,
                             int n_queries, int q_pad, int d_dlr, int d_cls, int k_rm, int n_buckets, int kt,
                             const uint8_t* map, bool abs_dlr, float dmax, __half* q_tiles, float* q32, int16_t* q_idx,
                             float* margin, float* tau, float* thr, int ts, int td, uint32_t* q_pack, __half* q16, uint8_t* q_idx8,
                             uint32_t* q_inexact, int c_idx_dtype, float i8_scale, float i8_ec, float i8_nc, float* i8_mul,
                             const float* col_scale, const G8Prep& g8, hipStream_t s) {
  hipLaunchKernelGGL(query_prep_kernel, dim3((q_pad + 3) / 4), dim3(256), 0, s, src, src_is_f32, ld, idx, idx_dtype,
                     ld_idx, n_queries, q_pad, d_dlr, d_cls, k_rm, n_buckets, kt, map, abs_dlr ? 1 : 0, dmax, q_tiles, q32,
                     q_idx, margin, tau, thr, ts, td, q_pack, q16, q_idx8, q_inexact, c_idx_dtype, i8_scale, i8_ec, i8_nc, i8_mul, col_scale, g8);
  return hipGetLastError();
}


int g_gemm_variant = 5;

thread_local int g_last_gemm_kernel = 0;
static hipError_t launch_gemm_filter_grid(const GemmArgs& a, dim3 grid, hipStream_t s);
hipError_t launch_gemm_filter(const GemmArgs& a_in, hipStream_t s) {
  static bool env_read = false;
  if (!env_read) {
    if (const char* e = getenv("DHR_GEMM_VARIANT")) g_gemm_variant = atoi(e) == 4 ? 4 : 5;
    env_read = true;
  }
  const int64_t n_tiles = a_in.seq_hi - a_in.seq_lo;
  if (n_tiles <= 0) return hipSuccess;
  const int64_t groups = (n_tiles + DOC_GROUP - 1) / DOC_GROUP;
  const int64_t groups_per_xcd = (groups + 7) / 8;
  if ((int64_t)DOC_GROUP * a_in.n_qtiles > 65535 || a_in.perm_n >= (1 << 24) || a_in.period > (1 << 20)) return hipErrorInvalidValue;
  if (a_in.map_mode >= 2 && a_in.period < 2) return hipErrorInvalidValue;
#ifdef DHR_AB_VARIANTS
  static const int g8_persist = getenv("DHR_G8_PERSIST") ? atoi(getenv("DHR_G8_PERSIST")) : 0;
  if (a_in.g8_shift && (g8_persist || a_in.variant == 6) && gemm_g8p_ok(a_in)) { g_last_gemm_kernel = 6; return launch_gemm_g8p(a_in, s); }
#endif
  GemmArgs a = a_in;
  a.inv_perm_n = 1.0 / (double)(a.perm_n > 0 ? a.perm_n : 1);
  a.inv_pm1 = 1.0 / (double)(a.period > 1 ? a.period - 1 : 1);
  if (groups < 8) {
    a.map_mode |= MAP_SPREAD_Q;
    const dim3 grid(8u, (unsigned)(DOC_GROUP * ((a.n_qtiles + 7) / 8)), (unsigned)groups);
    return launch_gemm_filter_grid(a, grid, s);
  }
  for (int64_t z0 = 0; z0 < groups_per_xcd; z0 += 65535) {
    GemmArgs c = a;
    c.seq_lo = a.seq_lo + z0 * 8 * DOC_GROUP;
    const dim3 grid(8u, (unsigned)(DOC_GROUP * a.n_qtiles), (unsigned)std::min<int64_t>(65535, groups_per_xcd - z0));
    const hipError_t e = launch_gemm_filter_grid(c, grid, s);
    if (e != hipSuccess) return e;
  }
  return hipSuccess;
}
static hipError_t launch_gemm_filter_grid(const GemmArgs& a, dim3 grid, hipStream_t s) {
  const int variant = a.variant == 4 ? 4 : a.variant ? 5 : g_gemm_variant;
  if (a.ts + a.td <= 0 || (a.ts & 1) || (a.td & 1) || (a.ts_q & 1)) return hipErrorInvalidValue;
  if (a.g8_shift) { g_last_gemm_kernel = 5; return (a.ts > 0 && a.ts_q == a.ts) ? launch_gemm_g8(a, grid, s) : hipErrorInvalidValue; }
  static const int dense_g8 = getenv("DHR_DENSE_G8") ? atoi(getenv("DHR_DENSE_G8")) : 1;
  if (a.i8_mul && dense_g8 && a.ts == 0 && a.ts_q == 0 && a.td > 0) { g_last_gemm_kernel = 5; return launch_gemm_g8(a, grid, s); }
  g_last_gemm_kernel = variant == 4 ? 4 : 3;
  return launch_gemm_wx(a, grid, variant, s);
}

__global__ void __launch_bounds__(1024) block_offsets_kernel(const uint32_t* __restrict__ cnt, uint32_t cap, int n_queries, uint32_t per,
                                                             uint32_t* __restrict__ offs) {
  __shared__ uint32_t part[1024];
  const int tid = threadIdx.x;
  const int chunk = (n_queries + 1023) / 1024;
  const int lo = tid * chunk, hi = min(lo + chunk, n_queries);
  uint32_t s = 0;
  for (int q = lo; q < hi; ++q) { uint32_t c = cnt[q]; if (c > cap) c = cap; s += (c + per - 1) / per; }
  part[tid] = s;
  __syncthreads();
  for (int d = 1; d < 1024; d <<= 1) {
    const uint32_t v = tid >= d ? part[tid - d] : 0u;
    __syncthreads();
    part[tid] += v;
    __syncthreads();
  }
  uint32_t run = tid ? part[tid - 1] : 0u;
  for (int q = lo; q < hi; ++q) { offs[q] = run; uint32_t c = cnt[q]; if (c > cap) c = cap; run += (c + per - 1) / per; }
  if (tid == 1023) offs[n_queries] = part[1023];
}
hipError_t launch_block_offsets(const uint32_t* cnt, uint32_t cap, int n_queries, uint32_t per, uint32_t* offs, hipStream_t s) {
  hipLaunchKernelGGL(block_offsets_kernel, dim3(1), dim3(1024), 0, s, cnt, cap, n_queries, per, offs);
  return hipGetLastError();
}
__global__ void __launch_bounds__(1024) lists_ready_kernel(const uint32_t* __restrict__ cnt, uint32_t cap, int n_queries, uint32_t per,
                                                           uint32_t* __restrict__ offs, uint32_t* __restrict__ out_max, uint32_t* __restrict__ out_max2,
                                                           unsigned long long* __restrict__ out_sum, unsigned long long* __restrict__ out_sum2,
                                                           uint32_t* __restrict__ fail_flags, uint32_t* __restrict__ zero, int n_zero,
                                                           const uint32_t* __restrict__ ovf_cap) {
  __shared__ uint32_t part[1024];
  __shared__ uint32_t wmax[16];
  __shared__ unsigned long long wsum[16];
  const int tid = threadIdx.x;
  const int chunk = (n_queries + 1023) / 1024;
  const int lo = tid * chunk, hi = min(lo + chunk, n_queries);
  uint32_t s = 0, m = 0;
  unsigned long long tot = 0;
  for (int q = lo; q < hi; ++q) {
    uint32_t c = cnt[q];
    m = c > m ? c : m;
    tot += c;
    const uint32_t cq = ovf_cap ? cap + ovf_cap[q] : cap;
    if (c > cq) { c = cq; if (fail_flags) fail_flags[q] = 1u; }
    s += (c + per - 1) / per;
  }
  part[tid] = s;
#pragma unroll
  for (int o = 32; o > 0; o >>= 1) {
    const uint32_t om = __shfl_xor(m, o, 64);
    m = om > m ? om : m;
    tot += __shfl_xor(tot, o, 64);
  }
  if ((tid & 63) == 0) { wmax[tid >> 6] = m; wsum[tid >> 6] = tot; }
  __syncthreads();
  for (int d = 1; d < 1024; d <<= 1) {
    const uint32_t v = tid >= d ? part[tid - d] : 0u;
    __syncthreads();
    part[tid] += v;
    __syncthreads();
  }
  uint32_t run = tid ? part[tid - 1] : 0u;
  for (int q = lo; q < hi; ++q) { offs[q] = run; uint32_t c = cnt[q]; const uint32_t cq = ovf_cap ? cap + ovf_cap[q] : cap; if (c > cq) c = cq; run += (c + per - 1) / per; }
  if (tid == 1023) offs[n_queries] = part[1023];
  if (tid == 0) {
    for (int i = 1; i < 16; ++i) { m = wmax[i] > m ? wmax[i] : m; tot += wsum[i]; }
    if (out_max) *out_max = m;
    if (out_max2) *out_max2 = m;
    if (out_sum) atomicAdd(out_sum, tot);
    if (out_sum2) atomicAdd(out_sum2, tot);
  }
  for (int j = tid; j < n_zero; j += 1024) zero[j] = 0u;
}
hipError_t launch_lists_ready(const uint32_t* cnt, uint32_t cap, int n_queries, uint32_t per, uint32_t* offs, uint32_t* out_max, uint32_t* out_max2,
                              unsigned long long* out_sum, unsigned long long* out_sum2, uint32_t* fail_flags, uint32_t* zero, int n_zero,
                              hipStream_t s, const uint32_t* ovf_cap) {
  hipLaunchKernelGGL(lists_ready_kernel, dim3(1), dim3(1024), 0, s, cnt, cap, n_queries, per, offs, out_max, out_max2, out_sum, out_sum2, fail_flags,
                     zero, n_zero, ovf_cap);
  return hipGetLastError();
}
__global__ void __launch_bounds__(1024) plan_overflow_kernel(const uint32_t* __restrict__ cnt_prev, double rows_ratio, uint32_t cap, uint32_t max_extra,
                                                             uint32_t arena_entries, int n_queries, uint32_t* __restrict__ ovf_off,
                                                             uint32_t* __restrict__ ovf_cap) {
  __shared__ unsigned long long part[1024];
  __shared__ double scale_s;
  const int tid = threadIdx.x;
  const int chunk = (n_queries + 1023) / 1024;
  const int lo = tid * chunk, hi = min(lo + chunk, n_queries);
  auto want = [&](int q) -> uint32_t {
    if (!cnt_prev) return 0u;
    const double need = 2.0 * (double)cnt_prev[q] * rows_ratio + 2048.0;
    if (!(need > (double)cap)) return 0u;
    const double extra = need - (double)cap;
    return extra >= (double)max_extra ? max_extra : (uint32_t)extra;
  };
  unsigned long long s = 0;
  for (int q = lo; q < hi; ++q) s += want(q);
  part[tid] = s;
  __syncthreads();
  for (int d = 512; d > 0; d >>= 1) {
    if (tid < d) part[tid] += part[tid + d];
    __syncthreads();
  }
  if (tid == 0) {
    const unsigned long long total = part[0] + 256ull * (unsigned long long)n_queries;
    scale_s = total > arena_entries ? (double)arena_entries / (double)total : 1.0;
  }
  __syncthreads();
  const double scale = scale_s;
  auto seg = [&](int q) -> uint32_t {
    const uint32_t w = want(q);
    if (w == 0u) return 0u;
    const uint32_t v = scale < 1.0 ? (uint32_t)((double)w * scale) : w;
    return (v + 255u) & ~255u;
  };
  __syncthreads();
  s = 0;
  for (int q = lo; q < hi; ++q) s += seg(q);
  part[tid] = s;
  __syncthreads();
  for (int d = 1; d < 1024; d <<= 1) {
    const unsigned long long v = tid >= d ? part[tid - d] : 0ull;
    __syncthreads();
    part[tid] += v;
    __syncthreads();
  }
  unsigned long long run = tid ? part[tid - 1] : 0ull;
  for (int q = lo; q < hi; ++q) {
    uint32_t w = seg(q);
    if (run >= arena_entries) w = 0u;
    else if (run + w > arena_entries) w = (uint32_t)(arena_entries - run);
// ... 1406 lines not shown
__global__ void emit_scores_kernel(const uint64_t* __restrict__ topk_keys, int kp, int n_queries, int r, float* __restrict__ out) {
  const int64_t g = (int64_t)blockIdx.x * blockDim.x + threadIdx.x;
  if (g >= (int64_t)n_queries * r) return;
  const int q = (int)(g / r), j = (int)(g - (int64_t)q * r);
  const uint64_t key = topk_keys[(int64_t)q * kp + j];
  out[g] = key ? ordered_f32((uint32_t)(key >> 32)) : -INFINITY;
}
hipError_t launch_emit_scores(const uint64_t* topk_keys, int kp, int n_queries, int r, float* out, hipStream_t s) {
  const int64_t total = (int64_t)n_queries * r;
  if (total <= 0) return hipSuccess;
  hipLaunchKernelGGL(emit_scores_kernel, dim3((unsigned)((total + 255) / 256)), dim3(256), 0, s, topk_keys, kp, n_queries, r, out);
  return hipGetLastError();
}
__global__ void make_thr_kernel(const float* __restrict__ tau, const float* __restrict__ margin, int n_queries, int q_pad,
                                float* __restrict__ thr) {
  const int q = blockIdx.x * blockDim.x + threadIdx.x;
  if (q < q_pad) thr[q] = q < n_queries ? tau[q] - margin[q] : INFINITY;
}
hipError_t launch_make_thr(const float* tau, const float* margin, int n_queries, int q_pad, float* thr, hipStream_t s) {
  hipLaunchKernelGGL(make_thr_kernel, dim3((q_pad + 255) / 256), dim3(256), 0, s, tau, margin, n_queries, q_pad, thr);
  return hipGetLastError();
}
__global__ void raise_thr_kernel(float* __restrict__ thr_hat, const float* __restrict__ thr_run, int n_queries) {
  const int q = blockIdx.x * blockDim.x + threadIdx.x;
  if (q < n_queries) thr_hat[q] = fmaxf(thr_hat[q], thr_run[q]);
}
hipError_t launch_raise_thr(float* thr_hat, const float* thr_run, int n_queries, hipStream_t s) {
  hipLaunchKernelGGL(raise_thr_kernel, dim3((n_queries + 255) / 256), dim3(256), 0, s, thr_hat, thr_run, n_queries);
  return hipGetLastError();
}
__global__ void flag_tau_above_kernel(const float* __restrict__ tau_own, const float* __restrict__ tau_ext, int n_queries, uint32_t* __restrict__ fail_flags) {
  const int q = blockIdx.x * blockDim.x + threadIdx.x;
  if (q < n_queries && tau_own[q] > tau_ext[q]) fail_flags[q] = 1u;
}
hipError_t launch_flag_tau_above(const float* tau_own, const float* tau_ext, int n_queries, uint32_t* fail_flags, hipStream_t s) {
  hipLaunchKernelGGL(flag_tau_above_kernel, dim3((n_queries + 255) / 256), dim3(256), 0, s, tau_own, tau_ext, n_queries, fail_flags);
  return hipGetLastError();
}
__global__ void raise_thr_rank_kernel(float* __restrict__ thr_hat, float* __restrict__ tau_hat, const uint64_t* __restrict__ topk_keys, int kp, int r,
                                      const float* __restrict__ margin, int n_queries) {
  const int q = blockIdx.x * blockDim.x + threadIdx.x;
  if (q >= n_queries) return;
  const uint64_t key = topk_keys[(int64_t)q * kp + (r - 1)];
  if (key == 0ull) return;
  const float t = ordered_f32((uint32_t)(key >> 32));
  if (!(t > tau_hat[q])) return;
  tau_hat[q] = t;
  thr_hat[q] = fmaxf(thr_hat[q], t - margin[q]);
}
hipError_t launch_raise_thr_rank(float* thr_hat, float* tau_hat, const uint64_t* topk_keys, int kp, int r, const float* margin, int n_queries, hipStream_t s) {
  hipLaunchKernelGGL(raise_thr_rank_kernel, dim3((n_queries + 255) / 256), dim3(256), 0, s, thr_hat, tau_hat, topk_keys, kp, r, margin, n_queries);
  return hipGetLastError();
}
__global__ void count_ge_kernel(const uint64_t* __restrict__ topk_keys, int kp, int k, const float* __restrict__ tau,
                                const uint32_t* __restrict__ fail_flags, int n_queries, int32_t* __restrict__ out) {
  const int q = blockIdx.x;
  if (q >= n_queries) return;
  __shared__ int cnt;
  if (threadIdx.x == 0) cnt = 0;
  __syncthreads();
  const float t = tau ? tau[q] : -INFINITY;
  int c = 0;
  for (int j = threadIdx.x; j < k; j += blockDim.x) {
    const uint64_t key = topk_keys[(int64_t)q * kp + j];
    if (key && ordered_f32((uint32_t)(key >> 32)) >= t) ++c;
  }
  atomicAdd(&cnt, c);
  __syncthreads();
  if (threadIdx.x == 0) out[q] = (fail_flags && fail_flags[q]) ? -1 : cnt;
}
hipError_t launch_count_ge(const uint64_t* topk_keys, int kp, int k, const float* tau, const uint32_t* fail_flags, int n_queries,
                           int32_t* out, hipStream_t s) {
  if (n_queries <= 0) return hipSuccess;
  hipLaunchKernelGGL(count_ge_kernel, dim3((unsigned)n_queries), dim3(256), 0, s, topk_keys, kp, k, tau, fail_flags, n_queries, out);
  return hipGetLastError();
}

__global__ void __launch_bounds__(1024) merge_topk_kernel(int n_in, int n_pad, const float* __restrict__ in_scores,
                                                          const int64_t* __restrict__ in_rows, int k_out,
                                                          float* __restrict__ out_scores, int64_t* __restrict__ out_rows) {
  extern __shared__ __attribute__((aligned(16))) char smem[];
  uint32_t* sk = (uint32_t*)smem;
  uint32_t* pos = sk + n_pad;
  const int q = blockIdx.x, tid = threadIdx.x;
  const float* s = in_scores + (int64_t)q * n_in;
  const int64_t* r = in_rows + (int64_t)q * n_in;
  for (int j = tid; j < n_pad; j += 1024) {
    const bool ok = j < n_in && r[j] >= 0;
    sk[j] = ok ? f32_ordered(s[j]) : 0u;
    pos[j] = ok ? (uint32_t)j : 0xFFFFFFFFu;
  }
  __syncthreads();
  auto before = [&](uint32_t ka, uint32_t pa, uint32_t kb, uint32_t pb) -> bool {
    if (pa == 0xFFFFFFFFu) return false;
    if (pb == 0xFFFFFFFFu) return true;
    if (ka != kb) return ka > kb;
    return r[pa] < r[pb];
  };
  for (int size = 2; size <= n_pad; size <<= 1)
    for (int stride = size >> 1; stride > 0; stride >>= 1) {
      for (int t = tid; t < (n_pad >> 1); t += 1024) {
        const int p0 = 2 * t - (t & (stride - 1)), p1 = p0 + stride;
        const uint32_t ka = sk[p0], pa = pos[p0], kb = sk[p1], pb = pos[p1];
        const bool desc = (p0 & size) == 0;
        const bool swap = desc ? before(kb, pb, ka, pa) : before(ka, pa, kb, pb);
        if (swap) { sk[p0] = kb; pos[p0] = pb; sk[p1] = ka; pos[p1] = pa; }
// ... 168 lines not shown
```

dhr_amd/csrc/search_core.hip:

```cpp
#include "dhr_state.h"

template <typename T>
static hipError_t re_malloc(T*& p, size_t bytes, int64_t& total) {
  if (p) hipFree(p);
  p = nullptr;
  total += (int64_t)bytes;
  return hipMalloc((void**)&p, bytes ? bytes : 16);
}

int ensure_ws(dhr_index* ix, Workspace& w, int n_queries, int k, int64_t keys_ld_min, int64_t cap_mult, bool use_refine, bool queries_only) {
  const int q_pad = (int)round_up(n_queries, TILE_ROWS);
  if (queries_only && w.q_alloc >= q_pad && w.kt == ix->kt && w.q32 != nullptr) { w.q_pad = q_pad; return DHR_OK; }
  int kp = 1;
  while (kp < k) kp <<= 1;
  if (kp < 64) kp = 64;
  const bool refine = (ix->heavy_key != nullptr || ix->resid8 != nullptr) && use_refine;
  int64_t cap = 0, cap_r = 0, keys_ld = 0, cap_deep = 0, arena = 0;
  auto plan_depths = [&](int q_for_cap) {
    int64_t base_cap = refine ? 262144 : 65536;
    const int64_t by_rows = ix->gated_i8 ? std::min<int64_t>(std::max<int64_t>(ix->n_rows / 8, 32768), 262144)
                                         : std::max<int64_t>(ix->n_rows / 128, refine ? 32768 : 16384);
    while (base_cap > by_rows && base_cap > 4096) base_cap >>= 1;
    while (base_cap > 4096 && (int64_t)q_for_cap * base_cap * 16 > ((int64_t)32 << 30)) base_cap >>= 1;
    if (ix->cand_cap > 0) base_cap = ix->cand_cap;
    cap = std::min<int64_t>(base_cap * cap_mult, (int64_t)1 << 22);
    cap_deep = cap;
    const int64_t stride = ix->list_stride > 0 ? ix->list_stride : 32768;
    arena = 0;
    const int variant = ix->gemm_variant ? ix->gemm_variant : g_gemm_variant;
    const bool kernel_writes_tier = ix->gated_i8 || variant != 4;
    if (refine && cap_mult == 1 && ix->cand_cap <= 0 && cap > stride && kernel_writes_tier) {
      cap = stride;
      arena = std::max<int64_t>((int64_t)4 << 20, std::min<int64_t>((int64_t)q_for_cap * 8192, (int64_t)128 << 20));
      arena = std::max(arena, 2 * (cap_deep - cap));
    }
    cap_r = refine ? std::min<int64_t>(cap_deep, std::max<int64_t>(32768, 4 * (int64_t)kp) * cap_mult) : cap;
    keys_ld = std::max<int64_t>(cap_r, keys_ld_min);
  };
  if (w.q_alloc >= q_pad && w.kt == ix->kt) {
    plan_depths(w.q_alloc);
    if (w.kp == kp && w.cap == cap && w.cap_deep == cap_deep && w.arena == arena && w.cap_r == cap_r && w.keys_ld >= keys_ld) { w.q_pad = q_pad; return DHR_OK; }
  }
  plan_depths(q_pad);
  free_ws(w);
  int64_t tot = 0;
  HIP_TRY(re_malloc(w.q_tiles, (size_t)q_pad * ix->kt * 2, tot));
  HIP_TRY(re_malloc(w.q32, (size_t)q_pad * ix->k_rm * 4, tot));
  HIP_TRY(re_malloc(w.q_idx, (size_t)q_pad * std::max(ix->d_dlr, 8) * 2, tot));
  HIP_TRY(re_malloc(w.q16, (size_t)q_pad * ix->k_rm * 2, tot));
  HIP_TRY(re_malloc(w.q_idx8, (size_t)q_pad * std::max(ix->d_dlr, 8), tot));
  HIP_TRY(re_malloc(w.q_inexact, 16, tot));
  HIP_TRY(re_malloc(w.margin, (size_t)q_pad * 4, tot));
  HIP_TRY(re_malloc(w.i8_mul, (size_t)q_pad * 4, tot));
// ... 116 lines not shown
  G8Prep g8{};
  if (ix->gated_i8) { g8.inv_cs = ix->g8_inv_cs; g8.w = ix->g8_w; g8.s_ref = ix->g8_sref; g8.max_shift = ix->g8_max_shift; g8.q8 = w.g8_q8; g8.shift = w.g8_shift; g8.unit = w.g8_unit; }
  if (ix->resid8) { g8.thr_raise = w.thr_raise; g8.resid_ec2 = ix->resid_ec2; }
  HIP_TRY(hipMemsetAsync(w.q_inexact, 0, 8, s));
  HIP_TRY(launch_query_prep(v, qb->value_dtype == DHR_VAL_F32, ldv, (ix->d_dlr > 0 && qb->index) ? qi : nullptr, qb->index_dtype, ldi,
                            qb->n_queries, w.q_pad, ix->d_dlr, ix->d_cls, ix->k_rm, ix->n_buckets, ix->kt, ix->bucket_map,
                            ix->abs_mode, ix->dmax, w.q_tiles, w.q32,
                            w.q_idx, w.margin, w.tau, w.thr, ix->ts, ix->td, w.q_pack, w.q16, w.q_idx8, w.q_inexact, ix->idx_dtype,
                            ix->dense_i8 ? ix->i8_scale : 0.f, ix->i8_ec, ix->i8_nc, w.i8_mul, ix->i8_col_scale, g8, s));
  return DHR_OK;
}

static inline bool uses_refine(const dhr_index* ix, bool gate) { return (ix->heavy_key != nullptr && (gate || ix->gated_i8)) || ix->resid8 != nullptr; }
RescoreArgs base_rescore_args(const dhr_index* ix, const Workspace& w, int n_queries, bool gate) {
  RescoreArgs r{};
  r.vals_rm = ix->vals_rm; r.c_idx = ix->c_idx; r.c_idx_dtype = ix->idx_dtype;
  r.q32 = w.q32; r.q_idx = w.q_idx; r.d_dlr = ix->d_dlr; r.k_rm = ix->k_rm;
  r.q16 = w.q16; r.q_idx8 = w.q_idx8; r.q_inexact = w.q_inexact;
  r.n_rows = ix->n_rows; r.n_queries = n_queries; r.gate = gate ? 1 : 0;
  return r;
}
GemmArgs base_gemm_args(const dhr_index* ix, const Workspace& w, int Q) {
  GemmArgs g{};
  g.a_tiles = ix->tiles; g.b_tiles = w.q_tiles; g.ksteps = ix->ksteps; g.k_split = ix->d_dlr / TILE_K; g.ts = ix->ts; g.td = ix->td; g.ts_q = w.ts_q; g.variant = ix->gemm_variant;
  g.i8_mul = (ix->dense_i8 || ix->gated_i8) ? w.i8_mul : nullptr; g.g8_shift = ix->gated_i8 ? w.g8_shift : nullptr; g.g8_rsum = ix->g8_rsum;
  g.n_tiles = ix->n_tiles; g.n_qtiles = w.q_pad / TILE_ROWS; g.n_rows = ix->n_rows; g.cap = (uint32_t)w.cap; g.n_queries = Q;
  return g;
}
SelectArgs rescored_select_args(const Workspace& w, int Q, int k) {
  SelectArgs sel{};
  sel.topk_keys = w.topk_keys; sel.in_keys = w.rs_keys; sel.ld_keys = w.keys_ld; sel.cap = (uint32_t)w.cap;
  sel.k = k; sel.kp = w.kp; sel.sort_n = select_sort_n(w.kp);
  sel.kps = 64; while (sel.kps < k) sel.kps <<= 1;
  sel.margin = w.margin; sel.tau = w.tau; sel.thr = w.thr; sel.n_queries = Q;
  return sel;
}
static RefineArgs base_refine_args(const dhr_index* ix, const Workspace& w, int Q, bool gate, const float* thr) {
  RefineArgs f{};
  f.cap = (uint32_t)w.cap; f.heavy_key = ix->heavy_key; f.heavy_val = ix->heavy_val;
  f.q_pack = w.q_pack; f.d_dlr = ix->d_dlr; f.thr = thr; f.out = w.cand_r; f.out_cnt = w.cnt_r; f.out_cap = (uint32_t)w.cap_r;
  f.n_queries = Q;
  if (ix->gated_i8) { f.g8_q8 = w.g8_q8; f.g8_inv_cs = ix->g8_inv_cs; f.g8_unit = w.g8_unit; f.abs_mode = ix->abs_mode ? 1 : 0; f.ungated = gate ? 0 : 1; }
  if (ix->resid8) { f.resid8 = ix->resid8; f.resid_ld = ix->resid_ld; f.q32 = w.q32; f.q32_ld = ix->k_rm; f.col_scale = ix->i8_col_scale; f.d_cls = ix->d_cls; f.thr_raise = w.thr_raise; }
  return f;
}

struct Search {
  dhr_index* ix; Workspace& w; Timer& tm; dhr_search_stats& st; hipStream_t s;
  Stage stage; int depth, k; const float* tau_ext;
  int Q = 0;
  bool gate = false;
  bool after_mid = false;
  bool async_ctl = false;
  SearchPlan p;
  SelectArgs sel{};
  double rate = 0.0, rate_r = 0.0;
  bool whole() const { return stage == Stage::Whole; }
  bool fresh() const { return whole() || stage == Stage::Begin || stage == Stage::Pre; }
};

static void count_gemm(const Search& c, int64_t tiles) {
  const double rows = (double)tiles * TILE_ROWS;
  c.st.phases++;
  c.st.gemm_rows += (int64_t)rows;
  c.st.gemm_flops += 2.0 * (double)c.w.q_pad * rows * (double)c.ix->kt;
  c.st.gemm_flops_alg += 2.0 * (double)c.Q * rows * (double)c.ix->k;
}

static int gemm_phase(Search& c, int64_t lo, int64_t hi, int period, bool enqueue_only, uint32_t* maxc, unsigned long long* sumc) {
  dhr_index* ix = c.ix; Workspace& w = c.w; hipStream_t s = c.s;
  GemmArgs g = base_gemm_args(ix, w, c.Q);
  if (enqueue_only && w.arena > 0) g.tier = w.tier_dev;
  g.seq_lo = lo; g.seq_hi = hi; g.map_mode = 1; g.period = period; g.head = c.p.head;
  g.thr = w.thr; g.cand = w.cand; g.cnt = w.cnt;
  HIP_TRY(hipMemsetAsync(w.cnt, 0, (size_t)w.q_pad * 4, s));
  if (!enqueue_only) HIP_TRY(hipMemsetAsync(w.d_max, 0, 16, s));
  c.tm.begin(T_GEMM); HIP_TRY(launch_gemm_filter(g, s)); c.tm.end();
  ix->last_gemm_kernel = g_last_gemm_kernel;
  if (!enqueue_only) {
    HIP_TRY(launch_max_u32(w.cnt, c.Q, w.d_max, (unsigned long long*)(w.d_max + 2), s));
    HIP_TRY(hipMemcpyAsync(w.h_pinned, w.d_max, 16, hipMemcpyDeviceToHost, s));
    HIP_TRY(hipStreamSynchronize(s));
    *maxc = ((uint32_t*)w.h_pinned)[0];
    memcpy(sumc, (uint32_t*)w.h_pinned + 2, 8);
  }
  count_gemm(c, hi - lo);
  return DHR_OK;
}
static int rescore_and_select(Search& c, const uint2* cand, const uint32_t* cnt, uint32_t list_cap, uint32_t max_count, uint32_t flat_blocks, hipStream_t s) {
  Workspace& w = c.w;
  RescoreArgs r = base_rescore_args(c.ix, w, c.Q, c.gate);
  r.cand = cand; r.cnt = cnt; r.cap = list_cap; r.max_count = max_count;
  r.out_keys = w.rs_keys; r.ld_keys = w.keys_ld;
  r.blk_off = w.blk_off + w.q_pad + 1; r.flat_blocks = flat_blocks;
  c.tm.begin_on(T_RESCORE, s); HIP_TRY(launch_rescore(r, s)); c.tm.end_on(s);
  c.sel.cnt = cnt; c.sel.count_all = 0; c.sel.cap = list_cap;
  c.tm.begin_on(T_SELECT, s); HIP_TRY(launch_select(c.sel, s)); c.tm.end_on(s);
  return DHR_OK;
}
static int rescore_select_async(Search& c, const uint2* cand, const uint32_t* cnt, const float* thr, hipStream_t s, uint32_t* d_fullest_bound = nullptr,
                                uint32_t* d_fullest = nullptr, const uint2* ovf = nullptr) {
  dhr_index* ix = c.ix; Workspace& w = c.w; Timer& tm = c.tm; const int Q = c.Q;
  uint32_t list_cap = (uint32_t)w.cap;
  const bool refine = uses_refine(ix, c.gate);
  if (!refine) ovf = nullptr;
  const uint32_t* ovf_cap = ovf ? w.ovf_cap : nullptr;
  HIP_TRY(launch_lists_ready(cnt, (uint32_t)w.cap, Q, refine ? (uint32_t)REFINE_PER_WG : (uint32_t)RESCORE_CANDS_PER_WG, refine ? w.blk_off : w.blk_off + w.q_pad + 1,
                             d_fullest_bound, refine ? nullptr : d_fullest, w.d_stats + 0, refine ? nullptr : w.d_stats + 1, w.fail_flags,
                             refine ? w.cnt_r : nullptr, refine ? (int)w.q_pad : 0, s, ovf_cap));
  if (refine) {
    RefineArgs f = base_refine_args(ix, w, Q, c.gate, thr);
    f.ovf = ovf; f.ovf_off = ovf ? w.ovf_off : nullptr; f.ovf_cap = ovf_cap;
    f.cand = cand; f.cnt = cnt; f.max_count = 1;
    f.blk_off = w.blk_off; f.flat_blocks = FLAT_GRID_ASYNC;
    tm.begin_on(T_REFINE, s); HIP_TRY(launch_refine(f, s)); tm.end_on(s);
    list_cap = (uint32_t)w.cap_r;
    cand = w.cand_r; cnt = w.cnt_r;
    HIP_TRY(launch_lists_ready(cnt, list_cap, Q, (uint32_t)RESCORE_CANDS_PER_WG, w.blk_off + w.q_pad + 1, d_fullest, nullptr, w.d_stats + 1,
                               nullptr, w.fail_flags, nullptr, 0, s));
  }
  return rescore_and_select(c, cand, cnt, list_cap, 1, FLAT_GRID_ASYNC, s);
}
static int rescore_select(Search& c, const uint2* cand, const uint32_t* cnt, const float* thr, uint32_t maxc, hipStream_t s, int64_t bound_sum,
                          uint32_t* fail_flags) {
  dhr_index* ix = c.ix; Workspace& w = c.w; Timer& tm = c.tm; const int Q = c.Q;
  uint32_t maxr = std::min<uint32_t>(maxc, (uint32_t)w.cap);
  if (maxr == 0) return DHR_OK;
  int64_t exact = bound_sum;
  uint32_t list_cap = (uint32_t)w.cap;
  if (uses_refine(ix, c.gate)) {
    RefineArgs f = base_refine_args(ix, w, Q, c.gate, thr);
    f.cand = cand; f.cnt = cnt; f.max_count = maxr;
    HIP_TRY(launch_block_offsets(cnt, (uint32_t)w.cap, Q, REFINE_PER_WG, w.blk_off, s));
    f.blk_off = w.blk_off; f.flat_blocks = (uint32_t)std::min<int64_t>(bound_sum / REFINE_PER_WG + Q, (int64_t)0x7fffffff);
    HIP_TRY(hipMemsetAsync(w.cnt_r, 0, (size_t)w.q_pad * 4, s));
    HIP_TRY(hipMemsetAsync(w.d_ref, 0, 16, s));
    tm.begin_on(T_REFINE, s); HIP_TRY(launch_refine(f, s)); tm.end_on(s);
    HIP_TRY(launch_max_u32(w.cnt_r, Q, w.d_ref, (unsigned long long*)(w.d_ref + 2), s));
    HIP_TRY(hipMemcpyAsync(w.h_ref, w.d_ref, 16, hipMemcpyDeviceToHost, s));
    HIP_TRY(hipStreamSynchronize(s));
    w.last_maxr = ((uint32_t*)w.h_ref)[0];
    maxr = std::min<uint32_t>(((uint32_t*)w.h_ref)[0], (uint32_t)w.cap_r);
    if (((uint32_t*)w.h_ref)[0] > (uint32_t)w.cap_r) {
      if (fail_flags) HIP_TRY(launch_mark_overflow(w.cnt_r, (uint32_t)w.cap_r, Q, fail_flags, s));
      else return 1;
    }
    list_cap = (uint32_t)w.cap_r;
    unsigned long long sum;
    memcpy(&sum, (uint32_t*)w.h_ref + 2, 8);
    exact = (int64_t)sum;
    cand = w.cand_r; cnt = w.cnt_r;
  }
  c.st.candidates_exact += exact;
  if (getenv("DHR_DEBUG_PLAN"))
    fprintf(stderr, "[dhr]   lists: bound %.0f per query (fullest %u) -> exact %.0f per query (fullest %u)\n", (double)bound_sum / Q, maxc, (double)exact / Q, maxr);
  if (maxr == 0) return DHR_OK;
  HIP_TRY(launch_block_offsets(cnt, list_cap, Q, RESCORE_CANDS_PER_WG, w.blk_off + w.q_pad + 1, s));
  return rescore_and_select(c, cand, cnt, list_cap, maxr, (uint32_t)std::min<int64_t>(exact / RESCORE_CANDS_PER_WG + Q, (int64_t)0x7fffffff), s);
}

struct StreamOpts {
  bool async_ctl = false;
// ... 54 lines not shown
    if (rc != DHR_OK) return rc < 0 ? rc : set_error(DHR_ERR_INTERNAL, "survivor list overflow at the minimum chunk size");
    if (o.last_rate_r) *o.last_rate_r = (uses_refine(ix, c.gate) && maxc > 0) ? (double)w.last_maxr / (double)chunk_rows : 0.0;
    pos = hi;
    seen_rows += chunk_rows;
    const double target = (double)w.cap / 2.0;
    double next_rows = (maxc == 0) ? (double)chunk_rows * 4.0 : (double)chunk_rows * target / (double)maxc;
    next_rows = std::min(next_rows, (double)seen_rows * ix->max_growth16 / 16.0);
    chunk = std::max<int64_t>(DOC_GROUP, (int64_t)(next_rows / (DOC_GROUP * TILE_ROWS)) * DOC_GROUP);
  }
  return DHR_OK;
}

static int prepare_and_phase0(Search& c, const dhr_query_batch* qb) {
  dhr_index* ix = c.ix; Workspace& w = c.w; Timer& tm = c.tm; hipStream_t s = c.s; const SearchPlan& p = c.p; const int Q = c.Q;
  int rc;
  tm.begin(T_PREP);
  if ((rc = prep_queries(ix, w, qb, s)) != DHR_OK) return rc;
  HIP_TRY(hipMemsetAsync(w.topk_keys, 0, (size_t)w.q_pad * w.kp * 8, s));
  HIP_TRY(hipMemsetAsync(w.fail_flags, 0, (size_t)w.q_pad * 4, s));
  HIP_TRY(hipMemsetAsync(w.d_stats, 0, 32, s));
  tm.end();
  RescoreArgs r = base_rescore_args(ix, w, Q, c.gate);
  r.out_keys = w.rs_keys; r.ld_keys = w.keys_ld;
  c.sel.cnt = nullptr;
  if (p.bootstrap) {
    const int m = p.boot_m;
    {
      GemmArgs g = base_gemm_args(ix, w, Q);
      g.seq_lo = 0; g.seq_hi = 1; g.map_mode = 0; g.period = 1; g.head = 0;
      g.thr = w.thr; g.cand = w.cand; g.cnt = w.cnt;
      g.dump = w.boot_bound; g.dump_ld = TILE_ROWS; g.dump_row0 = 0;
      tm.begin(T_GEMM); HIP_TRY(launch_gemm_filter(g, s)); tm.end();
      c.st.phases++;
    }
    HIP_TRY(launch_bound_topm(w.boot_bound, (int)std::min<int64_t>(TILE_ROWS, ix->n_rows), Q, m, w.boot_rows, s));
    r.rows32 = w.boot_rows; r.ld_rows = m; r.count_all = (uint32_t)m; r.max_count = (uint32_t)m;
    tm.begin(T_RESCORE); HIP_TRY(launch_rescore(r, s)); tm.end();
    c.sel.count_all = (uint32_t)m;
    c.sel.k = std::min(p.boot_r0, m); c.sel.monotone = 1;
    tm.begin(T_SELECT); HIP_TRY(launch_select(c.sel, s)); tm.end();
    HIP_TRY(hipMemsetAsync(w.topk_keys, 0, (size_t)w.q_pad * w.kp * 8, s));
    c.st.candidates_exact += (int64_t)m * Q;
    return DHR_OK;
  }
  r.row0 = 0; r.count_all = (uint32_t)p.first_valid; r.max_count = (uint32_t)p.first_valid;
  tm.begin(T_RESCORE); HIP_TRY(launch_rescore(r, s)); tm.end();
  c.sel.count_all = (uint32_t)p.first_valid;
  if (p.sampled) { c.sel.k = p.head_rank; c.sel.monotone = 1; }
  tm.begin(T_SELECT); HIP_TRY(launch_select(c.sel, s)); tm.end();
  c.st.candidates_exact += (int64_t)p.first_valid * Q;
  return DHR_OK;
}

static int sampled_run(Search& c) {
  dhr_index* ix = c.ix; Workspace& w = c.w; hipStream_t s = c.s; const SearchPlan& p = c.p; const int Q = c.Q;
  int64_t last_rows = 0;
  int64_t seen0 = p.first_valid, n_hi = p.n_sample, chunk0 = std::max<int64_t>(p.head, DOC_GROUP);
  StreamOpts o;
  o.async_ctl = c.async_ctl; o.last_rate = &c.rate; o.last_rate_r = &c.rate_r; o.last_rows = &last_rows;
  o.rank_target = p.r_eff; o.rank_rows = p.sample_rows;
  const bool pre = c.stage == Stage::Pre;
  if (pre) {
    n_hi = p.pre_positions;
    if (n_hi <= 0) return set_error(DHR_ERR_INVALID, "the sample of this index is too small for a pre step");
    constexpr int pre_growth = 64;
    o.growth16 = std::max(ix->max_growth16, pre_growth);
  }
  if (c.stage == Stage::BeginRest) {
    o.pos0 = ix->pend.pre_pos; seen0 = ix->pend.pre_seen;
    o.prev_rows0 = ix->pend.pre_last_rows;
    HIP_TRY(launch_raise_thr(w.tau, c.tau_ext, Q, s));
    HIP_TRY(launch_make_thr(w.tau, w.margin, Q, w.q_pad, w.thr, s));
    chunk0 = round_up(p.n_sample - o.pos0, DOC_GROUP);
  }
  int rc = stream_phases(c, n_hi, p.S, chunk0, seen0, o);
  if (rc != DHR_OK) return rc;
  if (pre) {
    staged_open(ix, StagedState::AfterPre, c.gate, Q, c.k);
    ix->pend.pre_pos = n_hi; ix->pend.pre_seen = p.first_valid + n_hi * TILE_ROWS; ix->pend.pre_last_rows = last_rows;
    return DHR_OK;
  }
  HIP_TRY(hipMemcpyAsync(w.tau_hat, w.tau, (size_t)w.q_pad * 4, hipMemcpyDeviceToDevice, s));
  if (c.async_ctl && w.arena > 0) {
    HIP_TRY(hipMemcpyAsync(w.cnt_plan, w.cnt, (size_t)w.q_pad * 4, hipMemcpyDeviceToDevice, s));
    w.plan_rows = last_rows;
  } else w.plan_rows = 0;
  if (c.async_ctl && ix->async_ctl >= 2 && c.whole() && last_rows > 0) {
    HIP_TRY(hipMemcpyAsync(w.h_pinned2, w.d_max2, 32, hipMemcpyDeviceToHost, s));
    HIP_TRY(hipStreamSynchronize(s));
    const uint32_t* hp = (const uint32_t*)w.h_pinned2;
    c.rate = (double)hp[0] / (double)last_rows;
    c.rate_r = uses_refine(ix, c.gate) ? (double)hp[4] / (double)last_rows : 0.0;
  }
  if (!c.whole()) {
    staged_open(ix, StagedState::AfterBegin, c.gate, Q, c.k);
    ix->pend.rate = c.rate; ix->pend.rate_r = c.rate_r;
  }
  return DHR_OK;
}

static int adopt_thresholds(Search& c) {
  Workspace& w = c.w; hipStream_t s = c.s; const int Q = c.Q;
  c.rate = c.ix->pend.rate; c.rate_r = c.ix->pend.rate_r;
  if (c.after_mid) {
    HIP_TRY(launch_raise_thr(w.tau_hat, c.tau_ext, Q, s));
    HIP_TRY(launch_make_thr(w.tau_hat, w.margin, Q, w.q_pad, w.thr, s));
    HIP_TRY(launch_raise_thr(w.thr_hat, w.thr, Q, s));
  } else {
    HIP_TRY(hipMemcpyAsync(w.tau_hat, c.tau_ext, (size_t)Q * 4, hipMemcpyDeviceToDevice, s));
    HIP_TRY(launch_flag_tau_above(w.tau, w.tau_hat, Q, w.fail_flags, s));
    HIP_TRY(launch_make_thr(w.tau_hat, w.margin, Q, w.q_pad, w.thr, s));
  }
  return DHR_OK;
}
struct MainPass {
  hipStream_t sg = nullptr, sb = nullptr;
  bool extrapolate = false, scatter = false, two_tier = false;
  int M = 0, c_lo = 0, c_hi = 0;
  std::vector<int64_t> bound;
  std::vector<hipEvent_t> ev_gemm, ev_done;
  Events evs;
};
static int main_streams(Search& c, MainPass& mp) {
  dhr_index* ix = c.ix;
  const int aux_cus = ix->aux_cus >= 0 ? ix->aux_cus : (ix->d_dlr == 0 ? 128 : 0);
  if (ix->aux_cus_made != aux_cus || ix->gemm_excl_made != ix->gemm_exclusive) {
    if (ix->s_aux) { hipStreamDestroy(ix->s_aux); ix->s_aux = nullptr; }
    if (ix->s_gemm) { hipStreamDestroy(ix->s_gemm); ix->s_gemm = nullptr; }
// ... 3 lines not shown
        const int lo = i * 32;
        const int n = std::max(0, std::min(32, aux_cus - lo));
        m_aux[i] = n >= 32 ? 0xffffffffu : ((1u << n) - 1u);
        m_gemm[i] = ix->gemm_exclusive ? ~m_aux[i] : 0xffffffffu;
      }
      if (hipExtStreamCreateWithCUMask(&ix->s_aux, 8, m_aux) != hipSuccess ||
          hipExtStreamCreateWithCUMask(&ix->s_gemm, 8, m_gemm) != hipSuccess) {
        (void)hipGetLastError();
        if (ix->s_aux) { hipStreamDestroy(ix->s_aux); ix->s_aux = nullptr; }
        if (ix->s_gemm) { hipStreamDestroy(ix->s_gemm); ix->s_gemm = nullptr; }
      }
    }
    if (!ix->s_aux) {
      HIP_TRY(hipStreamCreateWithFlags(&ix->s_aux, hipStreamNonBlocking));
    }
    ix->aux_cus_made = aux_cus; ix->gemm_excl_made = ix->gemm_exclusive;
  }
  mp.sg = ix->s_gemm ? ix->s_gemm : c.s;
  const bool overlap = ix->overlap_aux < 0 ? true : ix->overlap_aux != 0;
  mp.sb = overlap ? ix->s_aux : mp.sg;
  return DHR_OK;
}
static int main_chunk_count(const Search& c, const MainPass& mp, bool mid_proto) {
  const dhr_index* ix = c.ix; const Workspace& w = c.w; const int64_t n_main = c.p.n_main; const double rate = c.rate, rate_r = c.rate_r;
  const bool plan_read = ix->async_ctl >= 2 && c.whole();
  const int64_t plan_cap = mp.two_tier ? w.cap_deep : w.cap;
  const int64_t need = std::max((int64_t)std::ceil(1.5 * rate * (double)n_main * TILE_ROWS / (double)plan_cap),
                                (int64_t)std::ceil(1.5 * rate_r * (double)n_main * TILE_ROWS / (double)w.cap_r));
  int64_t by_size = std::min<int64_t>(8, std::max<int64_t>(2, (n_main + 4199) / 4200));
  const int64_t no_overflow = (3 * n_main * TILE_ROWS + 2 * std::min(plan_cap, w.cap_r) - 1) / (2 * std::min(plan_cap, w.cap_r));
  if (no_overflow <= 12) by_size = std::max(by_size, no_overflow);
  {
    const double k_eff = (double)c.k / (double)std::max(1, c.whole() ? 1 : ix->sample_share);
    const int64_t by_hot = (int64_t)std::ceil(300.0 * k_eff / (double)plan_cap);
    const int64_t by_hot_r = (int64_t)std::ceil(65.0 * k_eff / (double)w.cap_r);
    by_size = std::max(by_size, std::min<int64_t>(24, std::max(by_hot, by_hot_r)));
  }
  if (mp.extrapolate) by_size = std::max(by_size, std::min<int64_t>(12, (n_main + 2799) / 2800));
  const int64_t want = c.async_ctl ? std::max<int64_t>(std::max<int64_t>(ix->main_chunks, by_size), plan_read ? need : 0) : std::max<int64_t>(ix->main_chunks, need);
  const int M_plain = (int)std::max<int64_t>(1, std::min<int64_t>(std::min<int64_t>(want, 64), n_main / (16 * DOC_GROUP)));
  if (getenv("DHR_DEBUG_PLAN"))
    fprintf(stderr, "[dhr] main pass: rate %.3e (x n_main rows = %.0f of cap %lld), rate_r %.3e (%.0f of cap_r %lld), need %lld, chunks %d, n_main %lld tiles\n", rate,
            rate * (double)n_main * TILE_ROWS, (long long)w.cap, rate_r, rate_r * (double)n_main * TILE_ROWS, (long long)w.cap_r, (long long)need, M_plain + (mid_proto ? 1 : 0), (long long)n_main);
  return M_plain;
}
static int main_gemm(Search& c, MainPass& mp, int i) {
  dhr_index* ix = c.ix; Workspace& w = c.w; hipStream_t sg = mp.sg;
  uint32_t* cnt = (i & 1) ? w.cnt2 : w.cnt;
  if (i >= mp.c_lo + 2) HIP_TRY(hipStreamWaitEvent(sg, mp.ev_done[i - 2], 0));
  GemmArgs g = base_gemm_args(ix, w, c.Q);
  g.seq_lo = mp.bound[i]; g.seq_hi = mp.bound[i + 1]; g.map_mode = mp.scatter ? 3 : 2; g.period = c.p.S; g.head = c.p.head;
  g.perm_mul = mp.scatter ? c.p.perm_mul : 1; g.perm_n = c.p.n_main;
  g.thr = w.thr_hat; g.cand = (i & 1) ? w.cand2 : w.cand; g.cnt = cnt;
  if (mp.two_tier) g.tier = w.tier_dev + (i & 1);
  HIP_TRY(hipMemsetAsync(cnt, 0, (size_t)w.q_pad * 4, sg));
  if (!c.async_ctl) HIP_TRY(hipMemsetAsync(w.d_max2 + 4 * (i & 1), 0, 16, sg));
  c.tm.begin_on(T_GEMM, sg); HIP_TRY(launch_gemm_filter(g, sg)); c.tm.end_on(sg);
  ix->last_gemm_kernel = g_last_gemm_kernel;
  if (!c.async_ctl) {
    HIP_TRY(launch_max_u32(cnt, c.Q, w.d_max2 + 4 * (i & 1), (unsigned long long*)(w.d_max2 + 4 * (i & 1) + 2), sg));
    HIP_TRY(hipMemcpyAsync(w.h_pinned2 + 16 * (i & 1), w.d_max2 + 4 * (i & 1), 16, hipMemcpyDeviceToHost, sg));
  }
  HIP_TRY(hipEventRecord(mp.ev_gemm[i], sg));
  count_gemm(c, mp.bound[i + 1] - mp.bound[i]);
  return DHR_OK;
}
static int main_chunks(Search& c, MainPass& mp) {
  dhr_index* ix = c.ix; Workspace& w = c.w; const SearchPlan& p = c.p; const int Q = c.Q;
  hipStream_t sb = mp.sb;
  int rc;
  if ((rc = main_gemm(c, mp, mp.c_lo)) != DHR_OK) return rc;
  for (int i = mp.c_lo; i < mp.c_hi; ++i) {
    if (i + 1 < mp.c_hi && (rc = main_gemm(c, mp, i + 1)) != DHR_OK) return rc;
    uint2* cand = (i & 1) ? w.cand2 : w.cand;
    uint32_t* cnt = (i & 1) ? w.cnt2 : w.cnt;
    if (c.async_ctl) {
      if (sb != mp.sg) HIP_TRY(hipStreamWaitEvent(sb, mp.ev_gemm[i], 0));
      if ((rc = rescore_select_async(c, cand, cnt, w.thr_hat, sb, nullptr, nullptr, mp.two_tier ? ((i & 1) ? w.ovf2 : w.ovf) : nullptr)) != DHR_OK) return rc;
    } else {
      HIP_TRY(hipEventSynchronize(mp.ev_gemm[i]));
      const uint32_t maxc = *(const uint32_t*)(w.h_pinned2 + 16 * (i & 1));
      unsigned long long sumc;
      memcpy(&sumc, w.h_pinned2 + 16 * (i & 1) + 8, 8);
      c.st.candidates_bound += (int64_t)sumc;
      if (getenv("DHR_DEBUG_PLAN")) fprintf(stderr, "[dhr] main chunk %d: tiles [%lld, %lld)\n", i, (long long)mp.bound[i], (long long)mp.bound[i + 1]);
      HIP_TRY(launch_mark_overflow(cnt, (uint32_t)w.cap, Q, w.fail_flags, sb));
      if ((rc = rescore_select(c, cand, cnt, w.thr_hat, maxc, sb, (int64_t)sumc, w.fail_flags)) != DHR_OK) return rc;
    }
    if (ix->progressive_thr) HIP_TRY(launch_raise_thr(w.thr_hat, c.sel.thr, Q, sb));
    if (mp.extrapolate && i + 1 < mp.M) {
      const int r = plan::extrapolated_rank(c.k, (double)(p.head + p.n_sample + mp.bound[i + 1]) / (double)ix->n_tiles);
      if (r < c.k) HIP_TRY(launch_raise_thr_rank(w.thr_hat, w.tau_hat, w.topk_keys, w.kp, r, w.margin, Q, sb));
    }
    HIP_TRY(hipEventRecord(mp.ev_done[i], sb));
  }
  return DHR_OK;
}
static int main_pass(Search& c) {
  dhr_index* ix = c.ix; Workspace& w = c.w; hipStream_t s = c.s; const SearchPlan& p = c.p;
  MainPass mp;
  c.sel.k = c.k; c.sel.kps = w.kp; c.sel.monotone = 0;
  mp.extrapolate = ix->progressive_thr >= 2 && c.whole() && c.depth == 0 && p.n_main >= 64 && c.k >= 16;
  const bool mid = c.stage == Stage::Mid;
  const bool mid_proto = mid || c.after_mid;
  mp.scatter = mp.extrapolate || (mid_proto && p.n_main >= 64);
  if (!c.after_mid) HIP_TRY(hipMemcpyAsync(w.thr_hat, w.thr, (size_t)w.q_pad * 4, hipMemcpyDeviceToDevice, s));
  if (!w.cand2) {
    int64_t tot = 0;
    HIP_TRY(re_malloc(w.cand2, (size_t)w.q_alloc * w.cap * 8, tot));
    HIP_TRY(re_malloc(w.cnt2, (size_t)w.q_alloc * 4, tot));
    if (w.arena > 0) {
      HIP_TRY(re_malloc(w.ovf2, (size_t)w.arena * 8, tot));
      const ListTier t1{w.ovf2, w.ovf_off, w.ovf_cap};
      HIP_TRY(hipMemcpy(w.tier_dev + 1, &t1, sizeof t1, hipMemcpyHostToDevice));
    }
    w.bytes += tot;
  }
  int rc;
  if ((rc = main_streams(c, mp)) != DHR_OK) return rc;
  hipStream_t sg = mp.sg, sb = mp.sb;
  mp.two_tier = c.async_ctl && w.arena > 0;
  mp.bound = plan::main_chunk_bounds(p.n_main, main_chunk_count(c, mp, mid_proto), mid_proto ? p.mid_offset : 0);
  if (mid_proto) mp.bound.insert(mp.bound.begin(), 0);
  mp.M = (int)mp.bound.size() - 1;
  mp.c_lo = c.after_mid ? 1 : 0; mp.c_hi = mid ? 1 : mp.M;
  if (mp.two_tier) {
    int64_t big = 0;
    for (int i = 0; i < mp.M; ++i) big = std::max(big, mp.bound[i + 1] - mp.bound[i]);
    HIP_TRY(launch_plan_overflow(w.plan_rows > 0 ? w.cnt_plan : nullptr, w.plan_rows > 0 ? (double)(big * TILE_ROWS) / (double)w.plan_rows : 0.0, (uint32_t)w.cap,
                                 (uint32_t)(w.cap_deep - w.cap), (uint32_t)w.arena, c.Q, w.ovf_off, w.ovf_cap, s));
  }
  if (sg != s || sb != s) {
    hipEvent_t ev_enter = nullptr;
    HIP_TRY(mp.evs.add(&ev_enter, hipEventDisableTiming));
    HIP_TRY(hipEventRecord(ev_enter, s));
    if (sg != s) HIP_TRY(hipStreamWaitEvent(sg, ev_enter, 0));
    if (sb != s) HIP_TRY(hipStreamWaitEvent(sb, ev_enter, 0));
  }
  mp.ev_gemm.resize(mp.M); mp.ev_done.resize(mp.M);
  for (int i = 0; i < mp.M; ++i) {
    HIP_TRY(mp.evs.add(&mp.ev_gemm[i], hipEventDisableTiming));
    HIP_TRY(mp.evs.add(&mp.ev_done[i], hipEventDisableTiming));
  }
  if ((rc = main_chunks(c, mp)) != DHR_OK) return rc;
  HIP_TRY(hipStreamWaitEvent(s, mp.ev_done[mp.c_hi - 1], 0));
  return DHR_OK;
}

static void debug_report_failures(const Search& c) {
  const Workspace& w = c.w; const int Q = c.Q;
  std::vector<uint32_t> ff(Q); std::vector<float> th(Q);
  (void)hipStreamSynchronize(c.s);
  (void)hipMemcpy(ff.data(), w.fail_flags, (size_t)Q * 4, hipMemcpyDeviceToHost);
  (void)hipMemcpy(th.data(), w.tau_hat, (size_t)Q * 4, hipMemcpyDeviceToHost);
  for (int q = 0; q < Q; ++q) {
    uint64_t key = 0;
    (void)hipMemcpy(&key, w.topk_keys + (size_t)q * w.kp + (c.k - 1), 8, hipMemcpyDeviceToHost);
    const float kth = key ? ordered_f32((uint32_t)(key >> 32)) : -INFINITY;
    if (ff[q] || !(kth >= th[q])) fprintf(stderr, "[dhr] depth %d query %d will be redone: list overflow %u, k-th best %.6f, threshold %.6f\n", c.depth, q, ff[q], kth, th[q]);
// ... 22 lines not shown
  std::vector<int32_t> ids;
  for (int q = 0; q < Q; ++q)
    if (flags[q]) ids.push_back(q);
  int next_depth = c.depth + 1;
  if (c.depth == 0 && (int)n_overflow == 0) next_depth = 2;
  const int nf = (int)ids.size();
  DevMem tmp_mem;
  void*& tmp = tmp_mem.p;
  const size_t b32 = (size_t)nf * ix->k_rm * 4, bidx = (size_t)nf * std::max(ix->d_dlr, 8) * 2, bids = (size_t)nf * 4;
  HIP_TRY(hipMalloc(&tmp, b32 + bidx + bids + 64));
  float* f32 = (float*)tmp;
  int16_t* fidx = (int16_t*)((char*)tmp + b32);
  int32_t* d_ids = (int32_t*)((char*)tmp + b32 + bidx);
  if (hipMemcpyAsync(d_ids, ids.data(), bids, hipMemcpyHostToDevice, s) != hipSuccess) return set_error(DHR_ERR_HIP, "H2D failed");
  if (launch_gather_queries(w.q32, w.q_idx, ix->k_rm, ix->d_dlr, d_ids, nf, f32, fidx, s) != hipSuccess)
    return set_error(DHR_ERR_HIP, "gather_queries launch failed");
  dhr_query_batch sub{};
  sub.n_queries = nf; sub.mem_kind = ix->dlr_pad > 0 ? MEM_DEVICE_PADDED : DHR_MEM_DEVICE; sub.value = f32; sub.value_dtype = DHR_VAL_F32; sub.ld_value = ix->k_rm;
  sub.index = c.gate ? fidx : nullptr; sub.index_dtype = c.gate ? DHR_IDX_I16 : DHR_IDX_NONE; sub.ld_index = ix->d_dlr;
  Workspace& w2 = ix->ws_fb[next_depth - 1];
  int rc;
  if ((rc = search_core(ix, w2, &sub, k, next_depth, c.tm, st, s)) != DHR_OK) return rc;
  if (w2.kp != w.kp) return set_error(DHR_ERR_INTERNAL, "fallback workspace mismatch");
  if (launch_scatter_keys(w2.topk_keys, w.topk_keys, w.kp, d_ids, nf, s) != hipSuccess)
    return set_error(DHR_ERR_HIP, "scatter_keys launch failed");
  if (hipStreamSynchronize(s) != hipSuccess) return set_error(DHR_ERR_HIP, "fallback search failed on the device");
  return DHR_OK;
}

int search_core(dhr_index* ix, Workspace& w, const dhr_query_batch* qb, int k, int depth, Timer& tm, dhr_search_stats& st, hipStream_t s,
                Stage stage, const float* tau_ext) {
  Search c{ix, w, tm, st, s, stage, depth, k, tau_ext};
  const bool fresh = c.fresh();
  c.Q = fresh ? qb->n_queries : ix->pend.Q;
  c.gate = fresh ? (ix->d_dlr > 0 && qb->index != nullptr && qb->index_dtype != DHR_IDX_NONE) : ix->pend.gate;
  c.after_mid = stage == Stage::Finish && ix->pend.state == StagedState::AfterMid;
  c.p = search_plan_of(ix, k, depth, !c.whole());
  const SearchPlan& p = c.p;
  int rc;
  if ((rc = ensure_ws(ix, w, c.Q, k, p.first_valid, depth == 0 ? 1 : 16, c.gate || ix->gated_i8 || ix->resid8 != nullptr)) != DHR_OK) return rc;
  c.async_ctl = depth == 0 && p.S >= 2 && ix->async_ctl != 0 && !getenv("DHR_DEBUG_PLAN");
  c.sel = rescored_select_args(w, c.Q, k);
  c.sel.k = p.r_eff; c.sel.k_keep = k;

  if (fresh && (rc = prepare_and_phase0(c, qb)) != DHR_OK) return rc;
  if (!fresh && ix->pend.state == StagedState::Complete) return DHR_OK;
  if (!p.sampled) {
    if (p.rest > 0 && (rc = stream_phases(c, p.rest, 1, p.head, p.first_valid)) != DHR_OK) return rc;
    if (fresh && !c.whole()) staged_open(ix, StagedState::Complete, c.gate, c.Q, k);
    return DHR_OK;
  }
  switch (stage) {
    case Stage::Whole:
      if ((rc = sampled_run(c)) != DHR_OK || (rc = main_pass(c)) != DHR_OK) return rc;
      return verify_and_redo(c);
    case Stage::Begin: case Stage::Pre: case Stage::BeginRest:
      return sampled_run(c);
    case Stage::Mid: case Stage::Finish:
      if ((rc = adopt_thresholds(c)) != DHR_OK || (rc = main_pass(c)) != DHR_OK) return rc;
      if (stage == Stage::Mid) staged_set(ix, StagedState::AfterMid);
      return DHR_OK;
  }
  return set_error(DHR_ERR_INTERNAL, "unknown search stage");
}
```

include/dhr_hip.h:

```cpp
#ifndef DHR_HIP_H
#define DHR_HIP_H

#include <stdint.h>

#ifdef __cplusplus
extern "C" {
#endif

#define DHR_VERSION 105

typedef enum dhr_status {
  DHR_OK = 0,
  DHR_ERR_INVALID = -1,
  DHR_ERR_UNSUPPORTED = -2,
  DHR_ERR_HIP = -3,
  DHR_ERR_INTERNAL = -4,
  DHR_ERR_NOMEM = -5,
  DHR_ERR_PEER = -6
} dhr_status;

typedef enum dhr_idx_dtype { DHR_IDX_NONE = 0, DHR_IDX_U8 = 1, DHR_IDX_I8 = 2, DHR_IDX_I16 = 3 } dhr_idx_dtype;
typedef enum dhr_val_dtype { DHR_VAL_F16 = 0, DHR_VAL_F32 = 1, DHR_VAL_BF16 = 2 } dhr_val_dtype;
typedef enum dhr_mem_kind { DHR_MEM_HOST = 0, DHR_MEM_DEVICE = 1 } dhr_mem_kind;

// ... 2 lines not shown
typedef struct dhr_index_desc {
  int32_t device;
  int32_t mem_kind;
  int64_t n_rows;
  int32_t d_dlr;
  int32_t d_cls;
  const void* value;
  int64_t ld_value;
  const void* index;
  int32_t index_dtype;
  int32_t idx_buckets;
  int64_t ld_index;
  int64_t row_offset;
} dhr_index_desc;

typedef struct dhr_query_batch {
  int32_t n_queries;
  int32_t mem_kind;
  const void* value;
  int32_t value_dtype;
  int32_t index_dtype;
  int64_t ld_value;
  const void* index;
  int64_t ld_index;
} dhr_query_batch;

typedef struct dhr_search_stats {
  int64_t n_rows, n_queries, k;
  int32_t phases;
  int32_t overflow_retries;
  int64_t candidates_bound;
  int64_t candidates_exact;
  int64_t gemm_rows;
  int64_t sample_fallback_queries;
  double gemm_ms, refine_ms, rescore_ms, select_ms, prep_ms, total_ms;
  double gemm_flops;
  double gemm_flops_alg;
} dhr_search_stats;

typedef enum dhr_param {
  DHR_PARAM_CAND_CAP = 1,
  DHR_PARAM_FIRST_ROWS = 2,
  DHR_PARAM_PROFILE = 3,
  DHR_PARAM_MAX_GROWTH = 4,
  DHR_PARAM_MAIN_CHUNKS = 7,
  DHR_PARAM_AUX_CUS = 9,
  DHR_PARAM_GEMM_EXCLUSIVE = 10,
  DHR_PARAM_OVERLAP_AUX = 11,
  DHR_PARAM_PROGRESSIVE_THR = 8,
  DHR_PARAM_GEMM_VARIANT = 6,
  DHR_PARAM_ASYNC_CONTROLLER = 13,
  DHR_PARAM_SAMPLE_SHARE = 12,
  DHR_PARAM_LIST_STRIDE = 14,
  DHR_PARAM_SAMPLE_PERIOD = 5
} dhr_param;

typedef enum dhr_option {
  DHR_OPT_DENSE_I8 = 1,
  DHR_OPT_GATED_I8 = 2
} dhr_option;
int dhr_set_option(int32_t option, int64_t value);
typedef enum dhr_info {
  DHR_INFO_DENSE_I8 = 1,
  DHR_INFO_I8_SCALE = 2,
  DHR_INFO_I8_ROW_ERR = 3,
  DHR_INFO_I8_ROW_NORM = 4,
  DHR_INFO_ROW_NORM_MAX = 5,
  DHR_INFO_TILE_BYTES = 6,
  DHR_INFO_GATED_I8 = 7,
  DHR_INFO_GEMM_KERNEL = 8
} dhr_info;
int dhr_index_get_info(const dhr_index* index, int32_t what, double* out);

int dhr_version(void);
void dhr_abi_sizes(int32_t out[4]);
enum { DHR_ABI_INDEX_DESC = 0, DHR_ABI_QUERY_BATCH = 1, DHR_ABI_SEARCH_STATS = 2, DHR_ABI_FILE_INFO = 3, DHR_ABI_HOST_SHARD = 4 };
int32_t dhr_abi_size(int32_t which);
const char* dhr_last_error(void);

int dhr_index_create(const dhr_index_desc* desc, dhr_index** out);
void dhr_index_destroy(dhr_index* index);
int dhr_index_set_param(dhr_index* index, int32_t param, int64_t value);
int64_t dhr_index_device_bytes(const dhr_index* index);

typedef struct dhr_file_info {
  int64_t n_rows, row_offset;
  int32_t d_dlr, d_cls, index_dtype, idx_buckets;
  uint32_t file_version, reserved;
  int64_t payload_bytes;
  int64_t blob_offset, blob_bytes;
} dhr_file_info;
int dhr_index_save(const dhr_index* index, const char* path, const void* blob, int64_t blob_bytes);
int dhr_index_file_info(const char* path, dhr_file_info* out);
int dhr_index_load(const char* path, int32_t device, int64_t row_offset, dhr_index** out);

int dhr_search(dhr_index* index, const dhr_query_batch* queries, int32_t k, float* out_scores,
               int64_t* out_rows, int32_t out_mem_kind, void* stream);

int dhr_search_rerank(dhr_index* index, const dhr_query_batch* stage1, const dhr_query_batch* full, int32_t k1, int32_t k,
                      float* out_scores, int64_t* out_rows, int32_t out_mem_kind, void* stream);

int32_t dhr_search_sample_rank(const dhr_index* index, int32_t k);
int32_t dhr_search_union_rank(const dhr_index* index, int32_t k);
int dhr_search_begin(dhr_index* index, const dhr_query_batch* queries, int32_t k, float* out_sample_scores_dev, void* stream);
int dhr_search_finish(dhr_index* index, const float* tau_hat_dev, float* out_scores, int64_t* out_rows,
                      int32_t* out_count_dev, int32_t out_mem_kind, void* stream);
// ... 80 lines not shown
int dhr_aggregate_train(int32_t device, int32_t mem_kind, const void* lexical, int32_t value_dtype, int64_t ld, int64_t batch, int32_t vocab,
                        int32_t dims, int32_t remove_dims, int32_t full, void* out, int32_t out_dtype, int64_t ld_out, int16_t* route,
                        int64_t ld_route, void* stream);
int dhr_aggregate_backward(int32_t device, int32_t mem_kind, const void* grad_out, int32_t grad_dtype, int64_t ld_grad_out, const int16_t* route,
                           int64_t ld_route, int64_t batch, int32_t vocab, int32_t dims, int32_t remove_dims, int32_t full, void* grad_lexical,
                           int64_t ld_grad, void* stream);
int dhr_term_weight_head(int32_t device, int32_t mem_kind, const void* input_ids, int32_t id_bytes, int64_t ld_ids, const void* term_weights,
                         int32_t value_dtype, int64_t ld_weights, int64_t batch, int32_t n_tokens, int32_t skip_tokens, int32_t vocab,
                         float* out_reps, int64_t ld_reps, int16_t* out_tokens, int64_t ld_tokens, void* stream);
int dhr_term_weight_head_backward(int32_t device, int32_t mem_kind, const void* input_ids, int32_t id_bytes, int64_t ld_ids, int64_t batch,
                                  int32_t n_tokens, int32_t skip_tokens, int32_t vocab, const float* grad_reps, int64_t ld_grad_reps,
                                  const int16_t* tokens, int64_t ld_tokens, void* grad_weights, int32_t grad_dtype, int64_t ld_grad_weights,
                                  void* stream);

int dhr_maxsim_scores(int32_t device, int32_t mem_kind, const void* q, int64_t ld_q_tok, int64_t ld_q_batch, int64_t A, int64_t Lq, const void* p,
                      int64_t ld_p_tok, int64_t ld_p_batch, int64_t B, int64_t Lp, int32_t D, int32_t value_dtype, int32_t group, float* out,
                      int64_t ld_out, int16_t* arg, void* stream);
int dhr_maxsim_scores_backward(int32_t device, int32_t mem_kind, const void* q, int64_t ld_q_tok, int64_t ld_q_batch, int64_t A, int64_t Lq,
                               const void* p, int64_t ld_p_tok, int64_t ld_p_batch, int64_t B, int64_t Lp, int32_t D, int32_t value_dtype,
                               int32_t group, const int16_t* arg, const float* grad_out, int64_t ld_grad, void* dq, void* dp, int32_t grad_dtype,
                               void* stream);

int64_t dhr_train_loss_workspace(int64_t rows);
int dhr_train_loss(int32_t device, int32_t mem_kind, const void* lexical, int32_t lexical_dtype, int64_t ld_lexical, const void* semantic,
                   int32_t semantic_dtype, int64_t ld_semantic, const void* teacher, int32_t teacher_dtype, int64_t ld_teacher, int64_t rows,
                   int64_t cols, int64_t label_stride, float lamb, float temperature, const float* weights, const float* teacher_split, float* loss,
                   float* scores_out, int64_t ld_scores, void* grad_lexical, int64_t ld_grad_lexical, void* grad_semantic,
                   int64_t ld_grad_semantic, void* workspace, int64_t workspace_bytes, void* stream);

int dhr_pq_train(int32_t device, int32_t mem_kind, const void* values_f16, int64_t ld, int64_t n, int32_t d, int32_t M, int32_t iters,
                 int64_t max_points, float* codebooks, double* out_error, void* stream);
int dhr_pq_encode(int32_t device, int32_t mem_kind, const void* values_f16, int64_t ld, int64_t n, int32_t d, int32_t M,
                  const float* codebooks, uint8_t* codes, void* stream);
int dhr_pq_decode(int32_t device, int32_t mem_kind, const uint8_t* codes, int64_t n, int32_t d, int32_t M, const float* codebooks,
                  void* out_values_f16, int64_t ld_out, void* stream);
int dhr_pq_train_nbits(int32_t device, int32_t mem_kind, const void* values_f16, int64_t ld, int64_t n, int32_t d, int32_t M, int32_t nbits,
                       int32_t iters, int64_t max_points, float* codebooks, double* out_error, void* stream);
int dhr_pq_encode_nbits(int32_t device, int32_t mem_kind, const void* values_f16, int64_t ld, int64_t n, int32_t d, int32_t M, int32_t nbits,
                        const float* codebooks, uint8_t* codes, void* stream);
int dhr_pq_decode_nbits(int32_t device, int32_t mem_kind, const uint8_t* codes, int64_t n, int32_t d, int32_t M, int32_t nbits,
                        const float* codebooks, void* out_values_f16, int64_t ld_out, void* stream);

int dhr_write_trec(const char* path, int32_t append, int64_t n_queries, int64_t k, const char* qid_blob, const int64_t* qid_off,
                   const char* docid_blob, const int64_t* docid_off, int64_t n_docs, const int64_t* rows, int64_t row_base,
                   const float* scores, const char* run_name, int32_t id_sep_bytes, int32_t n_threads, int64_t* lines_out);
int dhr_format_float(double x, char* out, int32_t cap);

int dhr_get_stats(const dhr_index* index, dhr_search_stats* out);

int dhr_debug_bound_scores(dhr_index* index, const dhr_query_batch* queries, int64_t row_lo, int64_t row_hi,
                           float* out_dev, void* stream);

int dhr_debug_query_margins(dhr_index* index, const dhr_query_batch* queries, float* out_host, void* stream);

void dhr_debug_seq_to_tile(int64_t seq, int32_t map_mode, int32_t period, int64_t head, int64_t perm_mul, int64_t perm_n, int64_t out[2]);
int64_t dhr_debug_fail_alloc(int64_t n);
int32_t dhr_debug_sharded_repairs(void);

int dhr_debug_gemm_time(dhr_index* index, const dhr_query_batch* queries, int32_t iters, double* ms_out,
                        double* flops_out, void* stream);

typedef struct dhr_pq dhr_pq;
int dhr_pq_create(int32_t device, int32_t mem_kind, int64_t n, int32_t d, int32_t M, int32_t nbits, const float* codebooks,
                  const uint8_t* codes, int64_t row_offset, dhr_pq** out);
void dhr_pq_destroy(dhr_pq* pq);
int64_t dhr_pq_device_bytes(const dhr_pq* pq);
int dhr_pq_search(dhr_pq* pq, const dhr_query_batch* queries, int32_t k, float* out_scores, int64_t* out_rows, int32_t out_mem_kind,
                  void* stream);
int dhr_pq_adc_scores(dhr_pq* pq, const dhr_query_batch* queries, int64_t row_lo, int64_t row_hi, float* out_dev, void* stream);
int dhr_pq_last_scan(const dhr_pq* pq, double* ms, double* code_bytes);

typedef struct dhr_comm dhr_comm;
int dhr_comm_unique_id(void* out128, int32_t out_bytes);
int dhr_comm_create(const void* unique_id128, int32_t world, int32_t rank, int32_t device, dhr_comm** out);
int dhr_comm_wrap(void* nccl_comm, int32_t world, int32_t rank, int32_t device, dhr_comm** out);
typedef int (*dhr_allgather_fn)(void* user, const void* send, void* recv, int64_t bytes);
int dhr_comm_create_callback(int32_t world, int32_t rank, int32_t device, dhr_allgather_fn allgather, void* user, dhr_comm** out);
void dhr_comm_destroy(dhr_comm* comm);
enum { DHR_COMM_TRANSPORT = 0, DHR_COMM_WORLD = 1, DHR_COMM_RANK = 2, DHR_COMM_DEVICE = 3 };
int dhr_comm_info(const dhr_comm* comm, int32_t what);
void dhr_comm_abort(dhr_comm* comm);
typedef struct dhr_host_shard {
  uint32_t struct_size;
  uint32_t reserved;
  void* user;
  int32_t (*sample_rank)(void* user, int32_t k, int32_t share);
  int32_t (*union_rank)(void* user, int32_t k);
  int32_t (*begin)(void* user, const dhr_query_batch* queries, int32_t k, int32_t share, float* out_sample);
  int32_t (*finish)(void* user, const float* tau, float* out_scores, int64_t* out_rows, int32_t* out_count);
  int32_t (*search)(void* user, const dhr_query_batch* queries, int32_t k, float* out_scores, int64_t* out_rows);
  int32_t (*mid_ranks)(void* user, int32_t k, int32_t share, int32_t* out_local, int32_t* out_union);
  int32_t (*mid)(void* user, const float* tau, int32_t r_local, float* out_scores);
  int32_t (*pre_ranks)(void* user, int32_t k, int32_t share, int32_t* out_local, int32_t* out_union);
  int32_t (*pre)(void* user, const dhr_query_batch* queries, int32_t k, int32_t share, int32_t r_local, float* out_scores);
  int32_t (*begin_rest)(void* user, const float* tau, float* out_sample);
} dhr_host_shard;
int dhr_search_sharded_host(const dhr_host_shard* shard, int32_t world, int32_t rank, dhr_allgather_fn allgather, void* user,
                            const dhr_query_batch* queries, int32_t k, float* out_scores, int64_t* out_rows);
int dhr_search_sharded(dhr_index* shard, dhr_comm* comm, const dhr_query_batch* queries, int32_t k, float* out_scores,
                       int64_t* out_rows, int32_t out_mem_kind, void* stream);
int dhr_search_sharded_local(dhr_index** shards, int32_t n_shards, const dhr_query_batch* queries, int32_t k, float* out_scores,
                             int64_t* out_rows, int32_t out_mem_kind, void* stream);

#ifdef __cplusplus
}
#endif
// ... 2 lines not shown
```

Before: 60460.

## Seat queries into GEMM tiles ordered by sampled candidate-list length

After the sampled pass, queries are ranked by how many candidates they collected, and the query tiles, thresholds, scales and shifts are permuted into that order. The main-pass int8 GEMM then reads a per-tile slot-to-query map from LDS so candidate writes land on the original query's list. The aim is to group heavy-candidate queries in the same tiles, so epilogue divergence and atomic traffic concentrate and light tiles finish faster. The cost is extra seating kernels (an O(q_pad^2) rank computation plus a tile copy), more LDS, and an indirection in the epilogue.

Result: faster. 61660, median of 6 (+2.0%).

```diff
diff --git a/dhr_amd/_build.py b/dhr_amd/_build.py
--- a/dhr_amd/_build.py
+++ b/dhr_amd/_build.py
@@ -10,7 +10,7 @@
 LIB = os.path.join(CSRC, "libdhr_hip.so")
 OBJDIR = os.path.join(CSRC, "build")
 SOURCES = ["abi.cpp", "kernels.hip", "gemm_w4.hip", "gemm_g8.hip", "index_build.hip", "search_core.hip", "api.hip", "sharded.hip", "pq_adc.hip", "select_global.hip", "host_io.hip", "lexical.hip", "gip_train.hip", "lexical_train.hip", "maxsim.hip", "aggretriever_train.hip", "lexical_proj.hip", "lexical_proj_train.hip", "train_loss.hip", "densify_sparse.hip"]
-HEADERS = ["dhr_internal.h", "dhr_state.h", "search_plan.h", "index_layout.h", "sharded_plan.h", "host_stage.h", "op_dispatch.h", "abi_guard.h", "libdhr.map", "gemm_common.h", "gemm_g8.h", "lexical_common.h", "lexical_proj_common.h", "lexical_proj_layout.h", os.path.join("..", "..", "include", "dhr_hip.h")]
+HEADERS = ["dhr_internal.h", "dhr_state.h", "search_plan.h", "seating.h", "index_layout.h", "sharded_plan.h", "host_stage.h", "op_dispatch.h", "abi_guard.h", "libdhr.map", "gemm_common.h", "gemm_g8.h", "lexical_common.h", "lexical_proj_common.h", "lexical_proj_layout.h", os.path.join("..", "..", "include", "dhr_hip.h")]
 FLAGS = ["--offload-arch=gfx950", "-O3", "-std=c++17", "-fPIC", "-Wno-unused-value", "-Wno-unused-result"]
 if os.environ.get("DHR_AB_VARIANTS") == "1":
     SOURCES = SOURCES + [os.path.join("..", "..", "tools", "ab", "gemm_g8p.hip")]
diff --git a/dhr_amd/_lib.py b/dhr_amd/_lib.py
--- a/dhr_amd/_lib.py
+++ b/dhr_amd/_lib.py
@@ -14,14 +14,14 @@
 VAL_F16, VAL_F32, VAL_BF16 = 0, 1, 2
 MEM_HOST, MEM_DEVICE = 0, 1
 LEX_RAW, LEX_DENSIFY, LEX_AGG_FULL, LEX_AGG_SEMI = 0, 1, 2, 3
-PARAM_CAND_CAP, PARAM_FIRST_ROWS, PARAM_PROFILE, PARAM_MAX_GROWTH, PARAM_SAMPLE_PERIOD, PARAM_GEMM_VARIANT, PARAM_MAIN_CHUNKS, PARAM_PROGRESSIVE_THR, PARAM_AUX_CUS, PARAM_GEMM_EXCLUSIVE, PARAM_OVERLAP_AUX, PARAM_SAMPLE_SHARE, PARAM_ASYNC_CONTROLLER, PARAM_LIST_STRIDE = 1, 2, 3, 4, 5, 6, 7, 8, 9, 10, 11, 12, 13, 14
+PARAM_CAND_CAP, PARAM_FIRST_ROWS, PARAM_PROFILE, PARAM_MAX_GROWTH, PARAM_SAMPLE_PERIOD, PARAM_GEMM_VARIANT, PARAM_MAIN_CHUNKS, PARAM_PROGRESSIVE_THR, PARAM_AUX_CUS, PARAM_GEMM_EXCLUSIVE, PARAM_OVERLAP_AUX, PARAM_SAMPLE_SHARE, PARAM_ASYNC_CONTROLLER, PARAM_LIST_STRIDE, PARAM_SEAT_QUERIES = 1, 2, 3, 4, 5, 6, 7, 8, 9, 10, 11, 12, 13, 14, 15
 OPT_DENSE_I8, OPT_GATED_I8 = 1, 2
 COMM_TRANSPORT, COMM_WORLD, COMM_RANK, COMM_DEVICE = 0, 1, 2, 3
 INFO_DENSE_I8, INFO_I8_SCALE, INFO_I8_ROW_ERR, INFO_I8_ROW_NORM, INFO_ROW_NORM_MAX, INFO_TILE_BYTES, INFO_GATED_I8, INFO_GEMM_KERNEL = 1, 2, 3, 4, 5, 6, 7, 8
 
 EXPORTS = ["dhr_version", "dhr_abi_sizes", "dhr_abi_size", "dhr_debug_fail_alloc", "dhr_set_option", "dhr_index_get_info", "dhr_last_error", "dhr_index_create", "dhr_index_destroy", "dhr_index_set_param",
            "dhr_index_device_bytes", "dhr_search", "dhr_score_rows", "dhr_merge_topk", "dhr_merge_topk_host", "dhr_merge_topk_lists", "dhr_merge_topk_lists_host",
-           "dhr_get_stats", "dhr_debug_bound_scores", "dhr_debug_query_margins", "dhr_debug_gemm_time", "dhr_debug_seq_to_tile", "dhr_debug_sharded_repairs", "dhr_search_sample_rank", "dhr_search_union_rank", "dhr_search_begin",
+           "dhr_get_stats", "dhr_debug_bound_scores", "dhr_debug_query_margins", "dhr_debug_query_seating", "dhr_debug_gemm_time", "dhr_debug_seq_to_tile", "dhr_debug_sharded_repairs", "dhr_search_sample_rank", "dhr_search_union_rank", "dhr_search_begin",
            "dhr_search_finish", "dhr_search_mid_ranks", "dhr_search_mid", "dhr_search_pre_ranks", "dhr_search_pre", "dhr_search_begin_rest", "dhr_search_rerank", "dhr_comm_unique_id", "dhr_comm_create", "dhr_comm_wrap", "dhr_comm_create_callback", "dhr_comm_destroy", "dhr_comm_info", "dhr_comm_abort", "dhr_search_sharded", "dhr_search_sharded_local", "dhr_search_sharded_host", "dhr_pq_create", "dhr_pq_destroy", "dhr_pq_device_bytes", "dhr_pq_search", "dhr_pq_adc_scores", "dhr_pq_last_scan", "dhr_index_save", "dhr_index_file_info", "dhr_index_load", "dhr_densify", "dhr_pq_train", "dhr_pq_encode", "dhr_pq_decode", "dhr_pq_train_nbits", "dhr_pq_encode_nbits", "dhr_pq_decode_nbits", "dhr_write_trec", "dhr_format_float", "dhr_lexical_head", "dhr_aggregate", "dhr_gip_scores_workspace", "dhr_gip_scores", "dhr_gip_scores_backward", "dhr_densify_backward", "dhr_lexical_head_train_workspace", "dhr_lexical_head_train", "dhr_lexical_head_backward", "dhr_maxsim_scores", "dhr_maxsim_scores_backward", "dhr_aggregate_train", "dhr_aggregate_backward", "dhr_term_weight_head",
            "dhr_term_weight_head_backward", "dhr_lexical_proj_workspace", "dhr_lexical_proj_head", "dhr_lexical_proj_train_workspace",
            "dhr_lexical_proj_train", "dhr_lexical_proj_backward", "dhr_train_loss_workspace", "dhr_train_loss", "dhr_densify_sparse"]
@@ -231,6 +231,8 @@
     lib.dhr_index_get_info.argtypes = [C.c_void_p, C.c_int32, C.POINTER(C.c_double)]
     lib.dhr_debug_bound_scores.argtypes = [C.c_void_p, C.POINTER(QueryBatch), C.c_int64, C.c_int64, C.c_void_p, C.c_void_p]
     lib.dhr_debug_query_margins.argtypes = [C.c_void_p, C.POINTER(QueryBatch), C.c_void_p, C.c_void_p]
+    if hasattr(lib, "dhr_debug_query_seating"):
+        lib.dhr_debug_query_seating.argtypes = [C.c_void_p, C.c_int32, C.c_void_p, C.c_void_p, C.c_void_p, C.c_void_p, C.c_void_p]
     lib.dhr_debug_gemm_time.argtypes = [C.c_void_p, C.POINTER(QueryBatch), C.c_int32, C.POINTER(C.c_double),
                                         C.POINTER(C.c_double), C.c_void_p]
     if hasattr(lib, "dhr_debug_seq_to_tile"):
diff --git a/dhr_amd/csrc/api.hip b/dhr_amd/csrc/api.hip
--- a/dhr_amd/csrc/api.hip
+++ b/dhr_amd/csrc/api.hip
@@ -507,6 +507,22 @@
   return DHR_OK;
 } DHR_CATCH_STATUS
 
+extern "C" int dhr_debug_query_seating(dhr_index* ix, int32_t n_slots, int32_t* slot_q, int32_t* q_slot, uint32_t* lengths, float* thr_seat, float* thr_hat) try {
+  if (!ix) return set_error(DHR_ERR_INVALID, "null index");
+  HIP_TRY(hipSetDevice(ix->device));
+  const Workspace& w = ix->ws;
+  if (!w.seated || !w.seat_rec) return 0;
+  if (n_slots != w.q_pad) return set_error(DHR_ERR_INVALID, "n_slots must be the padded query count of the latest search");
+  HIP_TRY(hipDeviceSynchronize());
+  const size_t b = (size_t)n_slots * 4;
+  if (slot_q) HIP_TRY(hipMemcpy(slot_q, w.slot_q(), b, hipMemcpyDeviceToHost));
+  if (q_slot) HIP_TRY(hipMemcpy(q_slot, w.q_slot(), b, hipMemcpyDeviceToHost));
+  if (lengths) HIP_TRY(hipMemcpy(lengths, w.seat_len, b, hipMemcpyDeviceToHost));
+  if (thr_seat) HIP_TRY(hipMemcpy(thr_seat, w.thr_seat(), b, hipMemcpyDeviceToHost));
+  if (thr_hat) HIP_TRY(hipMemcpy(thr_hat, w.thr_hat, b, hipMemcpyDeviceToHost));
+  return 1;
+} DHR_CATCH_STATUS
+
 extern "C" void dhr_debug_seq_to_tile(int64_t seq, int32_t map_mode, int32_t period, int64_t head, int64_t perm_mul, int64_t perm_n, int64_t out[2]) try {
   out[0] = seq_to_tile_fast(seq, map_mode, period, head, perm_mul, perm_n, 1.0 / (double)(perm_n > 0 ? perm_n : 1), 1.0 / (double)(period > 1 ? period - 1 : 1));
   out[1] = seq_to_tile(seq, map_mode, period, head, perm_mul, perm_n);
diff --git a/dhr_amd/csrc/dhr_internal.h b/dhr_amd/csrc/dhr_internal.h
--- a/dhr_amd/csrc/dhr_internal.h
+++ b/dhr_amd/csrc/dhr_internal.h
@@ -122,6 +122,7 @@
   const int32_t* g8_shift;
   const int32_t* g8_rsum;
   int partial_wn;
+  int seat;
   uint32_t* p_ctr;
   int64_t p_groups;
   const float* i8_mul;
@@ -303,7 +304,7 @@
 hipError_t launch_max_u32(const uint32_t* v, int n, uint32_t* out_max, unsigned long long* out_sum, hipStream_t s);
 hipError_t launch_lists_ready(const uint32_t* cnt, uint32_t cap, int n_queries, uint32_t per, uint32_t* offs, uint32_t* out_max, uint32_t* out_max2,
                               unsigned long long* out_sum, unsigned long long* out_sum2, uint32_t* fail_flags, uint32_t* zero, int n_zero,
-                              hipStream_t s, const uint32_t* ovf_cap = nullptr);
+                              hipStream_t s, const uint32_t* ovf_cap = nullptr, uint32_t* seat_len = nullptr );
 hipError_t launch_rows_to_local(const int64_t* rows, int64_t n, int64_t row_offset, int64_t n_rows, uint32_t* out,
                                 hipStream_t s);
 hipError_t launch_mark_overflow(const uint32_t* cnt, uint32_t cap, int n_queries, uint32_t* fail_flags, hipStream_t s);
@@ -317,6 +318,12 @@
 hipError_t launch_raise_thr(float* thr_hat, const float* thr_run, int n_queries, hipStream_t s);
 hipError_t launch_flag_tau_above(const float* tau_own, const float* tau_ext, int n_queries, uint32_t* fail_flags, hipStream_t s);
 hipError_t launch_raise_thr_rank(float* thr_hat, float* tau_hat, const uint64_t* topk_keys, int kp, int r, const float* margin, int n_queries, hipStream_t s);
+hipError_t launch_raise_thr_main(float* thr_hat, const float* thr_run, float* tau_hat, const uint64_t* topk_keys, int kp, int r, const float* margin,
+                                 int n_queries, float* thr_seat, const int32_t* q_slot, hipStream_t s);
+hipError_t launch_seat_queries(const uint32_t* len, int n_queries, int q_pad, const float* thr, const float* i8_mul, const int32_t* g8_shift, const void* q_tiles,
+                               int ts_q, int td, int32_t* slot_q, int32_t* q_slot, float* thr_seat, float* mul_seat, int32_t* shift_seat, void* tiles_seat,
+                               hipStream_t s);
+bool gemm_filter_takes_g8(const GemmArgs& a);
 hipError_t launch_count_ge(const uint64_t* topk_keys, int kp, int k, const float* tau, const uint32_t* fail_flags, int n_queries,
                            int32_t* out, hipStream_t s);
 hipError_t launch_merge_topk(int n_queries, int n_in, const float* in_scores, const int64_t* in_rows, int k_out,
diff --git a/dhr_amd/csrc/dhr_state.h b/dhr_amd/csrc/dhr_state.h
--- a/dhr_amd/csrc/dhr_state.h
+++ b/dhr_amd/csrc/dhr_state.h
@@ -92,6 +92,15 @@
   uint32_t* blk_off = nullptr;
   uint2* cand2 = nullptr;
   uint32_t* cnt2 = nullptr;
+  float* seat_rec = nullptr;
+  __half* q_tiles_seat = nullptr;
+  uint32_t* seat_len = nullptr;
+  bool seated = false;
+  float* thr_seat() const { return seat_rec; }
+  int32_t* slot_q() const { return (int32_t*)seat_rec + q_alloc; }
+  int32_t* q_slot() const { return (int32_t*)seat_rec + 2 * (size_t)q_alloc; }
+  float* mul_seat() const { return seat_rec + 3 * (size_t)q_alloc; }
+  int32_t* shift_seat() const { return (int32_t*)seat_rec + 4 * (size_t)q_alloc; }
   void* h_pinned = nullptr;
   char* h_pinned2 = nullptr;
   uint32_t* d_max2 = nullptr;
@@ -152,6 +161,7 @@
   int gemm_variant = 0;
   int last_gemm_kernel = 0;
   int overlap_aux = -1;
+  int seat_queries = -1;
   int aux_cus = -1, gemm_exclusive = 0;
   int aux_cus_made = -1, gemm_excl_made = -1;
   hipStream_t s_gemm = nullptr;
@@ -172,6 +182,7 @@
 inline void free_ws(Workspace& w) {
   hipFree(w.q_tiles); hipFree(w.q32); hipFree(w.q_idx); hipFree(w.q16); hipFree(w.q_idx8); hipFree(w.q_inexact); hipFree(w.margin); hipFree(w.i8_mul); hipFree(w.g8_q8); hipFree(w.g8_shift); hipFree(w.g8_unit); hipFree(w.tau); hipFree(w.thr);
   hipFree(w.cnt); hipFree(w.cand); if (!w.keys_alias) hipFree(w.rs_keys); hipFree(w.topk_keys); hipFree(w.d_max); hipFree(w.tau_hat); hipFree(w.fail_flags); hipFree(w.thr_hat); hipFree(w.cand2); hipFree(w.cnt2); hipFree(w.q_pack); hipFree(w.cand_r); hipFree(w.cnt_r); hipFree(w.thr_raise); hipFree(w.blk_off); hipFree(w.ovf); hipFree(w.ovf2); hipFree(w.ovf_off); hipFree(w.ovf_cap); hipFree(w.cnt_plan); hipFree(w.tier_dev); hipFree(w.boot_rows); hipFree(w.boot_bound);
+  hipFree(w.seat_rec); hipFree(w.q_tiles_seat); hipFree(w.seat_len);
   if (w.h_pinned) hipHostFree(w.h_pinned);
   if (w.h_pinned2) hipHostFree(w.h_pinned2);
   hipFree(w.d_max2); hipFree(w.d_ref); hipFree(w.d_stats);
diff --git a/dhr_amd/csrc/gemm_g8.h b/dhr_amd/csrc/gemm_g8.h
--- a/dhr_amd/csrc/gemm_g8.h
+++ b/dhr_amd/csrc/gemm_g8.h
@@ -10,7 +10,8 @@
 constexpr int G8_QOFF = 16384;
 constexpr int G8_SLOT = 32768;
 constexpr int G8_META = 4 * G8_SLOT;
-constexpr int G8_RING_LDS = 4 * G8_SLOT + 4096 + 64;
+constexpr int G8_MAP = G8_META + 4096;
+constexpr int G8_RING_LDS = 4 * G8_SLOT + 4096 + 1024 + 64;
 constexpr int G8_NT = 512;
 
 
diff --git a/dhr_amd/csrc/gemm_g8.hip b/dhr_amd/csrc/gemm_g8.hip
--- a/dhr_amd/csrc/gemm_g8.hip
+++ b/dhr_amd/csrc/gemm_g8.hip
@@ -40,10 +40,10 @@
 
 template <bool SURPLUS, int NI_, bool CHECK_ROWS = true>
 __device__ __forceinline__ void g8_scan_half(const GemmArgs& p, floatx16 (&acc)[4][2], int qt, int wm, int wn, int lane, int rows_valid, int64_t row0,
-                                             uint2* stack, const int t, const float mul, uint32_t& j) {
+                                             uint2* stack, const int t, const float mul, uint32_t& j, const int* qmap = nullptr) {
   const int fhalf = lane >> 5;
   const int rbase = wm * 128 + 4 * fhalf;
-  const int q = qt * TILE_ROWS + wn * 64 + NI_ * 32 + (lane & 31);
+  const int ql = wn * 64 + NI_ * 32 + (lane & 31);
 #pragma unroll
   for (int mi = 0; mi < 4; ++mi) {
     const floatx16& a = acc[mi][NI_];
@@ -70,6 +70,7 @@
             asm volatile("");
             if constexpr (SURPLUS) {
               if (j >= EPI_STACK) {
+                const int q = qmap ? qmap[ql] : qt * TILE_ROWS + ql;
                 const uint32_t slot = atomicAdd(p.cnt + q, 1u);
                 cand_store(p, q, slot, make_uint2((uint32_t)(row0 + rl), __float_as_uint(g8_score(v, mul))));
               }
@@ -82,10 +83,10 @@
   }
 }
 __device__ __forceinline__ void g8_epilogue_surplus(const GemmArgs& p, floatx16 (&acc)[4][2], int qt, int wm, int wn, int lane, int rows_valid, int64_t row0,
-                                                 const int (&thr_r)[2], const float (&mul_r)[2]) {
+                                                 const int (&thr_r)[2], const float (&mul_r)[2], const int* qmap) {
   uint32_t j = 0;
-  g8_scan_half<true, 0>(p, acc, qt, wm, wn, lane, rows_valid, row0, nullptr, thr_r[0], mul_r[0], j);
-  g8_scan_half<true, 1>(p, acc, qt, wm, wn, lane, rows_valid, row0, nullptr, thr_r[1], mul_r[1], j);
+  g8_scan_half<true, 0>(p, acc, qt, wm, wn, lane, rows_valid, row0, nullptr, thr_r[0], mul_r[0], j, qmap);
+  g8_scan_half<true, 1>(p, acc, qt, wm, wn, lane, rows_valid, row0, nullptr, thr_r[1], mul_r[1], j, qmap);
 }
 __device__ __forceinline__ void g8_epilogue(const GemmArgs& p, floatx16 (&acc)[4][2], int64_t dt, int qt, int wm, int wn, int tid, int lane,
                                             char* smem, const int (&thr_r)[2], const float (&mul_r)[2]) {
@@ -93,7 +94,9 @@
   const int64_t row0 = dt * TILE_ROWS;
   const int rows_valid = (int)(p.n_rows - row0 < TILE_ROWS ? p.n_rows - row0 : TILE_ROWS);
   uint2* stack = (uint2*)smem + tid;
-  const int q0 = qt * TILE_ROWS + wn * 64 + (lane & 31);
+  const int ql0 = wn * 64 + (lane & 31);
+  const int* qmap = p.seat ? (const int*)(smem + G8_MAP) : nullptr;
+  int q0 = qt * TILE_ROWS + ql0, q1 = q0 + 32;
   const bool full = rows_valid == TILE_ROWS;
   uint32_t j = 0;
   if (full) g8_scan_half<false, 0, false>(p, acc, qt, wm, wn, lane, rows_valid, row0, stack, thr_r[0], mul_r[0], j);
@@ -101,7 +104,10 @@
   const uint32_t s0 = j < (uint32_t)EPI_STACK ? j : (uint32_t)EPI_STACK;
 #if G8_ABL != 16
   uint32_t base0 = 0u, base1 = 0u;
-  if (s0 > 0) base0 = atomicAdd(p.cnt + q0, s0);
+  if (s0 > 0) {
+    if (qmap) q0 = qmap[ql0];
+    base0 = atomicAdd(p.cnt + q0, s0);
+  }
 #endif
   if (full) g8_scan_half<false, 1, false>(p, acc, qt, wm, wn, lane, rows_valid, row0, stack, thr_r[1], mul_r[1], j);
   else g8_scan_half<false, 1, true>(p, acc, qt, wm, wn, lane, rows_valid, row0, stack, thr_r[1], mul_r[1], j);
@@ -109,8 +115,11 @@
 #if G8_ABL == 16
   return;
 #else
-  if (s1 > s0) base1 = atomicAdd(p.cnt + q0 + 32, s1 - s0);
-  if (__builtin_amdgcn_ballot_w64(j > (uint32_t)EPI_STACK) != 0) g8_epilogue_surplus(p, acc, qt, wm, wn, lane, rows_valid, row0, thr_r, mul_r);
+  if (s1 > s0) {
+    if (qmap) q1 = qmap[ql0 + 32];
+    base1 = atomicAdd(p.cnt + q1, s1 - s0);
+  }
+  if (__builtin_amdgcn_ballot_w64(j > (uint32_t)EPI_STACK) != 0) g8_epilogue_surplus(p, acc, qt, wm, wn, lane, rows_valid, row0, thr_r, mul_r, qmap);
   for (uint32_t i = 0; i < s0; ++i) {
     const uint2 en = stack[i * G8_NT];
     const uint32_t slot = base0 + i;
@@ -119,7 +128,7 @@
   for (uint32_t i = s0; i < s1; ++i) {
     const uint2 en = stack[i * G8_NT];
     const uint32_t slot = base1 + (i - s0);
-    cand_store(p, q0 + 32, slot, make_uint2((uint32_t)row0 + en.x, __float_as_uint(g8_score((int)en.y, mul_r[1]))));
+    cand_store(p, q1, slot, make_uint2((uint32_t)row0 + en.x, __float_as_uint(g8_score((int)en.y, mul_r[1]))));
   }
 #endif
 }
@@ -249,6 +258,8 @@
                     : wave == 2 ? (const char*)(p.thr + qt * TILE_ROWS) : (const char*)(p.g8_shift + qt * TILE_ROWS);
     __builtin_amdgcn_global_load_lds(GLOBAL_PTR(src + lane_off), LDS_PTR(smem + G8_META + wave * 1024), 16, 0, 0);
   }
+  if (wave == 4 && p.seat != 0 && !DUMP)
+    __builtin_amdgcn_global_load_lds(GLOBAL_PTR((const char*)(p.thr + p.seat + qt * TILE_ROWS) + lane_off), LDS_PTR(smem + G8_MAP), 16, 0, 0);
   issue_pair(0);
   if (npairs > 1) {
     issue_pair(1);
diff --git a/dhr_amd/csrc/index_build.hip b/dhr_amd/csrc/index_build.hip
--- a/dhr_amd/csrc/index_build.hip
+++ b/dhr_amd/csrc/index_build.hip
@@ -72,6 +72,7 @@
       ix->aux_cus = (int)value; return DHR_OK;
     case DHR_PARAM_GEMM_EXCLUSIVE: ix->gemm_exclusive = value != 0; return DHR_OK;
     case DHR_PARAM_OVERLAP_AUX: ix->overlap_aux = value < 0 ? -1 : value != 0; return DHR_OK;
+    case DHR_PARAM_SEAT_QUERIES: ix->seat_queries = value < 0 ? -1 : 0; return DHR_OK;
     case DHR_PARAM_GEMM_VARIANT:
 #ifdef DHR_AB_VARIANTS
       if (value == 6) { ix->gemm_variant = 6; return DHR_OK; }
diff --git a/dhr_amd/csrc/kernels.hip b/dhr_amd/csrc/kernels.hip
--- a/dhr_amd/csrc/kernels.hip
+++ b/dhr_amd/csrc/kernels.hip
@@ -4,6 +4,7 @@
 
 #include "dhr_internal.h"
 #include "gemm_common.h"
+#include "seating.h"
 #include <type_traits>
 
 namespace dhr {
@@ -584,12 +585,18 @@
   }
   return hipSuccess;
 }
+bool gemm_filter_takes_g8(const GemmArgs& a) {
+  if (a.ts + a.td <= 0 || (a.ts & 1) || (a.td & 1) || (a.ts_q & 1)) return false;
+  if (a.g8_shift) return a.ts > 0 && a.ts_q == a.ts;
+  static const int dense_g8 = getenv("DHR_DENSE_G8") ? atoi(getenv("DHR_DENSE_G8")) : 1;
+  return a.i8_mul && dense_g8 && a.ts == 0 && a.ts_q == 0 && a.td > 0;
+}
 static hipError_t launch_gemm_filter_grid(const GemmArgs& a, dim3 grid, hipStream_t s) {
   const int variant = a.variant == 4 ? 4 : a.variant ? 5 : g_gemm_variant;
   if (a.ts + a.td <= 0 || (a.ts & 1) || (a.td & 1) || (a.ts_q & 1)) return hipErrorInvalidValue;
   if (a.g8_shift) { g_last_gemm_kernel = 5; return (a.ts > 0 && a.ts_q == a.ts) ? launch_gemm_g8(a, grid, s) : hipErrorInvalidValue; }
-  static const int dense_g8 = getenv("DHR_DENSE_G8") ? atoi(getenv("DHR_DENSE_G8")) : 1;
-  if (a.i8_mul && dense_g8 && a.ts == 0 && a.ts_q == 0 && a.td > 0) { g_last_gemm_kernel = 5; return launch_gemm_g8(a, grid, s); }
+  if (gemm_filter_takes_g8(a)) { g_last_gemm_kernel = 5; return launch_gemm_g8(a, grid, s); }
+  if (a.seat) return hipErrorInvalidValue;
   g_last_gemm_kernel = variant == 4 ? 4 : 3;
   return launch_gemm_wx(a, grid, variant, s);
 }
@@ -622,7 +629,7 @@
                                                            uint32_t* __restrict__ offs, uint32_t* __restrict__ out_max, uint32_t* __restrict__ out_max2,
                                                            unsigned long long* __restrict__ out_sum, unsigned long long* __restrict__ out_sum2,
                                                            uint32_t* __restrict__ fail_flags, uint32_t* __restrict__ zero, int n_zero,
-                                                           const uint32_t* __restrict__ ovf_cap) {
+                                                           const uint32_t* __restrict__ ovf_cap, uint32_t* __restrict__ seat_len) {
   __shared__ uint32_t part[1024];
   __shared__ uint32_t wmax[16];
   __shared__ unsigned long long wsum[16];
@@ -635,6 +642,7 @@
     uint32_t c = cnt[q];
     m = c > m ? c : m;
     tot += c;
+    if (seat_len) seat_len[q] += c;
     const uint32_t cq = ovf_cap ? cap + ovf_cap[q] : cap;
     if (c > cq) { c = cq; if (fail_flags) fail_flags[q] = 1u; }
     s += (c + per - 1) / per;
@@ -668,9 +676,9 @@
 }
 hipError_t launch_lists_ready(const uint32_t* cnt, uint32_t cap, int n_queries, uint32_t per, uint32_t* offs, uint32_t* out_max, uint32_t* out_max2,
                               unsigned long long* out_sum, unsigned long long* out_sum2, uint32_t* fail_flags, uint32_t* zero, int n_zero,
-                              hipStream_t s, const uint32_t* ovf_cap) {
+                              hipStream_t s, const uint32_t* ovf_cap, uint32_t* seat_len) {
   hipLaunchKernelGGL(lists_ready_kernel, dim3(1), dim3(1024), 0, s, cnt, cap, n_queries, per, offs, out_max, out_max2, out_sum, out_sum2, fail_flags,
-                     zero, n_zero, ovf_cap);
+                     zero, n_zero, ovf_cap, seat_len);
   return hipGetLastError();
 }
 __global__ void __launch_bounds__(1024) plan_overflow_kernel(const uint32_t* __restrict__ cnt_prev, double rows_ratio, uint32_t cap, uint32_t max_extra,
@@ -2183,6 +2191,79 @@
   hipLaunchKernelGGL(raise_thr_rank_kernel, dim3((n_queries + 255) / 256), dim3(256), 0, s, thr_hat, tau_hat, topk_keys, kp, r, margin, n_queries);
   return hipGetLastError();
 }
+__global__ void raise_thr_main_kernel(float* __restrict__ thr_hat, const float* __restrict__ thr_run, float* __restrict__ tau_hat,
+                                      const uint64_t* __restrict__ topk_keys, int kp, int r, const float* __restrict__ margin, int n_queries,
+                                      float* __restrict__ thr_seat, const int32_t* __restrict__ q_slot) {
+  const int q = blockIdx.x * blockDim.x + threadIdx.x;
+  if (q >= n_queries) return;
+  float t = thr_hat[q];
+  if (thr_run) t = fmaxf(t, thr_run[q]);
+  if (r > 0) {
+    const uint64_t key = topk_keys[(int64_t)q * kp + (r - 1)];
+    if (key != 0ull) {
+      const float te = ordered_f32((uint32_t)(key >> 32));
+      if (te > tau_hat[q]) {
+        tau_hat[q] = te;
+        t = fmaxf(t, te - margin[q]);
+      }
+    }
+  }
+  thr_hat[q] = t;
+  if (thr_seat) thr_seat[q_slot[q]] = t;
+}
+hipError_t launch_raise_thr_main(float* thr_hat, const float* thr_run, float* tau_hat, const uint64_t* topk_keys, int kp, int r, const float* margin,
+                                 int n_queries, float* thr_seat, const int32_t* q_slot, hipStream_t s) {
+  hipLaunchKernelGGL(raise_thr_main_kernel, dim3((n_queries + 255) / 256), dim3(256), 0, s, thr_hat, thr_run, tau_hat, topk_keys, kp, r, margin, n_queries,
+                     thr_seat, q_slot);
+  return hipGetLastError();
+}
+__global__ void __launch_bounds__(256) seat_rank_kernel(const uint32_t* __restrict__ len, int n_queries, int q_pad, const float* __restrict__ thr,
+                                                        const float* __restrict__ i8_mul, const int32_t* __restrict__ g8_shift,
+                                                        int32_t* __restrict__ slot_q, int32_t* __restrict__ q_slot, float* __restrict__ thr_seat,
+                                                        float* __restrict__ mul_seat, int32_t* __restrict__ shift_seat) {
+  __shared__ int32_t keys[seat::MAX_QUERIES];
+  for (int j = threadIdx.x; j < q_pad; j += 256) {
+    const uint32_t l = j < n_queries ? len[j] : 0u;
+    keys[j] = (int32_t)seat::key_of(l < 0x7fffffffu ? l : 0x7fffffffu, j, n_queries);
+  }
+  __syncthreads();
+  const int q = blockIdx.x * 256 + threadIdx.x;
+  if (q >= q_pad) return;
+  const int64_t kq = keys[q];
+  int slot = 0;
+  for (int j = 0; j < q_pad; ++j) slot += seat::before((int64_t)keys[j], j, kq, q) ? 1 : 0;
+  slot_q[slot] = q;
+  q_slot[q] = slot;
+  thr_seat[slot] = thr[q];
+  mul_seat[slot] = i8_mul[q];
+  if (g8_shift) shift_seat[slot] = g8_shift[q];
+}
+__global__ void __launch_bounds__(256) seat_tiles_kernel(const char* __restrict__ src, char* __restrict__ dst, const int32_t* __restrict__ slot_q, int q_pad,
+                                                         int ts_q, int td) {
+  const int cpq = (ts_q + td) * 4;
+  const int64_t i = (int64_t)blockIdx.x * 256 + threadIdx.x;
+  if (i >= (int64_t)q_pad * cpq) return;
+  const int sl = (int)(i / cpq), c = (int)(i - (int64_t)sl * cpq);
+  const int st = c >> 2, cc = c & 3;
+  const int q = slot_q[sl];
+  const int64_t tile_bytes = (int64_t)ts_q * SP_STAGE_B + (int64_t)td * SP_DENSE;
+  const int64_t st_off = st < ts_q ? (int64_t)st * SP_STAGE_B : (int64_t)ts_q * SP_STAGE_B + (int64_t)(st - ts_q) * SP_DENSE;
+  const int rq = q & 255, rs = sl & 255;
+  const uint4 v = *(const uint4*)(src + (int64_t)(q >> 8) * tile_bytes + st_off + rq * 64 + ((cc ^ ((rq >> 2) & 3)) * 16));
+  *(uint4*)(dst + (int64_t)(sl >> 8) * tile_bytes + st_off + rs * 64 + ((cc ^ ((rs >> 2) & 3)) * 16)) = v;
+}
+hipError_t launch_seat_queries(const uint32_t* len, int n_queries, int q_pad, const float* thr, const float* i8_mul, const int32_t* g8_shift, const void* q_tiles,
+                               int ts_q, int td, int32_t* slot_q, int32_t* q_slot, float* thr_seat, float* mul_seat, int32_t* shift_seat, void* tiles_seat,
+                               hipStream_t s) {
+  if (q_pad <= 0 || q_pad > seat::MAX_QUERIES || (q_pad & 255)) return hipErrorInvalidValue;
+  hipLaunchKernelGGL(seat_rank_kernel, dim3(q_pad / 256), dim3(256), 0, s, len, n_queries, q_pad, thr, i8_mul, g8_shift, slot_q, q_slot, thr_seat, mul_seat,
+                     shift_seat);
+  hipError_t e = hipGetLastError();
+  if (e != hipSuccess) return e;
+  const int64_t chunks = (int64_t)q_pad * (ts_q + td) * 4;
+  hipLaunchKernelGGL(seat_tiles_kernel, dim3((unsigned)((chunks + 255) / 256)), dim3(256), 0, s, (const char*)q_tiles, (char*)tiles_seat, slot_q, q_pad, ts_q, td);
+  return hipGetLastError();
+}
 __global__ void count_ge_kernel(const uint64_t* __restrict__ topk_keys, int kp, int k, const float* __restrict__ tau,
                                 const uint32_t* __restrict__ fail_flags, int n_queries, int32_t* __restrict__ out) {
   const int q = blockIdx.x;
diff --git a/dhr_amd/csrc/search_core.hip b/dhr_amd/csrc/search_core.hip
--- a/dhr_amd/csrc/search_core.hip
+++ b/dhr_amd/csrc/search_core.hip
@@ -1,4 +1,5 @@
 #include "dhr_state.h"
+#include "seating.h"
 
 template <typename T>
 static hipError_t re_malloc(T*& p, size_t bytes, int64_t& total) {
@@ -221,6 +222,8 @@
   bool gate = false;
   bool after_mid = false;
   bool async_ctl = false;
+  bool seat = false;
+  uint32_t* seat_acc = nullptr;
   SearchPlan p;
   SelectArgs sel{};
   double rate = 0.0, rate_r = 0.0;
@@ -276,7 +279,7 @@
   const uint32_t* ovf_cap = ovf ? w.ovf_cap : nullptr;
   HIP_TRY(launch_lists_ready(cnt, (uint32_t)w.cap, Q, refine ? (uint32_t)REFINE_PER_WG : (uint32_t)RESCORE_CANDS_PER_WG, refine ? w.blk_off : w.blk_off + w.q_pad + 1,
                              d_fullest_bound, refine ? nullptr : d_fullest, w.d_stats + 0, refine ? nullptr : w.d_stats + 1, w.fail_flags,
-                             refine ? w.cnt_r : nullptr, refine ? (int)w.q_pad : 0, s, ovf_cap));
+                             refine ? w.cnt_r : nullptr, refine ? (int)w.q_pad : 0, s, ovf_cap, c.seat_acc));
   if (refine) {
     RefineArgs f = base_refine_args(ix, w, Q, c.gate, thr);
     f.ovf = ovf; f.ovf_off = ovf ? w.ovf_off : nullptr; f.ovf_cap = ovf_cap;
@@ -437,6 +440,24 @@
   return DHR_OK;
 }
 
+static int seat_plan(Search& c) {
+  dhr_index* ix = c.ix; Workspace& w = c.w;
+  c.seat = false;
+  if (!c.whole() || c.depth != 0 || !c.async_ctl || !c.p.sampled || ix->seat_queries == 0 || ix->gemm_variant == 6 || !ix->gated_i8) return DHR_OK;
+  if (w.q_pad <= TILE_ROWS || w.q_pad > seat::MAX_QUERIES) return DHR_OK;
+  if (!gemm_filter_takes_g8(base_gemm_args(ix, w, c.Q))) return DHR_OK;
+  if (!w.seat_rec) {
+    int64_t tot = 0;
+    HIP_TRY(re_malloc(w.seat_rec, (size_t)w.q_alloc * 5 * 4, tot));
+    HIP_TRY(re_malloc(w.q_tiles_seat, (size_t)w.q_alloc * ix->kt * 2, tot));
+    HIP_TRY(re_malloc(w.seat_len, (size_t)w.q_alloc * 4, tot));
+    w.bytes += tot;
+  }
+  HIP_TRY(hipMemsetAsync(w.seat_len, 0, (size_t)w.q_pad * 4, c.s));
+  c.seat = true;
+  return DHR_OK;
+}
+
 static int sampled_run(Search& c) {
   dhr_index* ix = c.ix; Workspace& w = c.w; hipStream_t s = c.s; const SearchPlan& p = c.p; const int Q = c.Q;
   int64_t last_rows = 0;
@@ -458,7 +479,9 @@
     HIP_TRY(launch_make_thr(w.tau, w.margin, Q, w.q_pad, w.thr, s));
     chunk0 = round_up(p.n_sample - o.pos0, DOC_GROUP);
   }
+  c.seat_acc = c.seat ? w.seat_len : nullptr;
   int rc = stream_phases(c, n_hi, p.S, chunk0, seen0, o);
+  c.seat_acc = nullptr;
   if (rc != DHR_OK) return rc;
   if (pre) {
     staged_open(ix, StagedState::AfterPre, c.gate, Q, c.k);
@@ -568,6 +591,10 @@
   g.seq_lo = mp.bound[i]; g.seq_hi = mp.bound[i + 1]; g.map_mode = mp.scatter ? 3 : 2; g.period = c.p.S; g.head = c.p.head;
   g.perm_mul = mp.scatter ? c.p.perm_mul : 1; g.perm_n = c.p.n_main;
   g.thr = w.thr_hat; g.cand = (i & 1) ? w.cand2 : w.cand; g.cnt = cnt;
+  if (c.seat) {
+    g.b_tiles = w.q_tiles_seat; g.i8_mul = w.mul_seat(); g.thr = w.thr_seat(); g.seat = w.q_alloc;
+    if (g.g8_shift) g.g8_shift = w.shift_seat();
+  }
   if (mp.two_tier) g.tier = w.tier_dev + (i & 1);
   HIP_TRY(hipMemsetAsync(cnt, 0, (size_t)w.q_pad * 4, sg));
   if (!c.async_ctl) HIP_TRY(hipMemsetAsync(w.d_max2 + 4 * (i & 1), 0, 16, sg));
@@ -603,11 +630,15 @@
       HIP_TRY(launch_mark_overflow(cnt, (uint32_t)w.cap, Q, w.fail_flags, sb));
       if ((rc = rescore_select(c, cand, cnt, w.thr_hat, maxc, sb, (int64_t)sumc, w.fail_flags)) != DHR_OK) return rc;
     }
-    if (ix->progressive_thr) HIP_TRY(launch_raise_thr(w.thr_hat, c.sel.thr, Q, sb));
+    const float* thr_run = ix->progressive_thr ? c.sel.thr : nullptr;
+    int r = 0;
     if (mp.extrapolate && i + 1 < mp.M) {
-      const int r = plan::extrapolated_rank(c.k, (double)(p.head + p.n_sample + mp.bound[i + 1]) / (double)ix->n_tiles);
-      if (r < c.k) HIP_TRY(launch_raise_thr_rank(w.thr_hat, w.tau_hat, w.topk_keys, w.kp, r, w.margin, Q, sb));
-    }
+      r = plan::extrapolated_rank(c.k, (double)(p.head + p.n_sample + mp.bound[i + 1]) / (double)ix->n_tiles);
+      if (r >= c.k) r = 0;
+    }
+    if (thr_run || r > 0)
+      HIP_TRY(launch_raise_thr_main(w.thr_hat, thr_run, w.tau_hat, w.topk_keys, w.kp, r, w.margin, Q, c.seat ? w.thr_seat() : nullptr,
+                                    c.seat ? w.q_slot() : nullptr, sb));
     HIP_TRY(hipEventRecord(mp.ev_done[i], sb));
   }
   return DHR_OK;
@@ -621,6 +652,10 @@
   const bool mid_proto = mid || c.after_mid;
   mp.scatter = mp.extrapolate || (mid_proto && p.n_main >= 64);
   if (!c.after_mid) HIP_TRY(hipMemcpyAsync(w.thr_hat, w.thr, (size_t)w.q_pad * 4, hipMemcpyDeviceToDevice, s));
+  w.seated = c.seat;
+  if (c.seat)
+    HIP_TRY(launch_seat_queries(w.seat_len, c.Q, w.q_pad, w.thr, w.i8_mul, ix->gated_i8 ? w.g8_shift : nullptr, w.q_tiles, w.ts_q, ix->td, w.slot_q(), w.q_slot(),
+                                w.thr_seat(), w.mul_seat(), w.shift_seat(), w.q_tiles_seat, s));
   if (!w.cand2) {
     int64_t tot = 0;
     HIP_TRY(re_malloc(w.cand2, (size_t)w.q_alloc * w.cap * 8, tot));
@@ -749,7 +784,7 @@
   }
   switch (stage) {
     case Stage::Whole:
-      if ((rc = sampled_run(c)) != DHR_OK || (rc = main_pass(c)) != DHR_OK) return rc;
+      if ((rc = seat_plan(c)) != DHR_OK || (rc = sampled_run(c)) != DHR_OK || (rc = main_pass(c)) != DHR_OK) return rc;
       return verify_and_redo(c);
     case Stage::Begin: case Stage::Pre: case Stage::BeginRest:
       return sampled_run(c);
diff --git a/dhr_amd/csrc/seating.h b/dhr_amd/csrc/seating.h
--- /dev/null
+++ b/dhr_amd/csrc/seating.h
@@ -0,0 +1,25 @@
+#pragma once
+#include <cstdint>
+
+#if defined(__HIPCC__)
+#define DHR_SEAT_HD __host__ __device__
+#else
+#define DHR_SEAT_HD
+#endif
+
+namespace dhr {
+namespace seat {
+
+constexpr int MAX_QUERIES = 8192;
+
+DHR_SEAT_HD inline int64_t key_of(uint32_t len, int q, int n_queries) { return q < n_queries ? (int64_t)len : (int64_t)-1; }
+DHR_SEAT_HD inline bool before(int64_t ka, int a, int64_t kb, int b) { return ka > kb || (ka == kb && a < b); }
+DHR_SEAT_HD inline int slot_of(const uint32_t* len, int q, int n_queries, int q_pad) {
+  const int64_t kq = key_of(q < n_queries ? len[q] : 0u, q, n_queries);
+  int slot = 0;
+  for (int j = 0; j < q_pad; ++j) slot += before(key_of(j < n_queries ? len[j] : 0u, j, n_queries), j, kq, q) ? 1 : 0;
+  return slot;
+}
+
+}
+}
diff --git a/include/dhr_hip.h b/include/dhr_hip.h
--- a/include/dhr_hip.h
+++ b/include/dhr_hip.h
@@ -78,6 +78,7 @@
   DHR_PARAM_ASYNC_CONTROLLER = 13,
   DHR_PARAM_SAMPLE_SHARE = 12,
   DHR_PARAM_LIST_STRIDE = 14,
+  DHR_PARAM_SEAT_QUERIES = 15,
   DHR_PARAM_SAMPLE_PERIOD = 5
 } dhr_param;
 
@@ -264,6 +265,8 @@
                            float* out_dev, void* stream);
 
 int dhr_debug_query_margins(dhr_index* index, const dhr_query_batch* queries, float* out_host, void* stream);
+
+int dhr_debug_query_seating(dhr_index* index, int32_t n_slots, int32_t* slot_q, int32_t* q_slot, uint32_t* lengths, float* thr_seat, float* thr_hat);
 
 void dhr_debug_seq_to_tile(int64_t seq, int32_t map_mode, int32_t period, int64_t head, int64_t perm_mul, int64_t perm_n, int64_t out[2]);
 int64_t dhr_debug_fail_alloc(int64_t n);
```
